# initc3/HoneyBadgerMPC

Measured on AMD Instinct MI355X. Metric: shares reconstructed/sec (batch open, n=64 t=21), higher is better.
Workload: dtype u256 (integer mod p): exact int8 x int8 -> int32 byte-split GEMM on the matrix cores; the high half of every sum folded mod p on the matrix cores too, one-word Barrett quotient

## Files before the change

honeybadgermpc_amd/_capi.py:

```python
import ctypes
import os

import numpy as np

_HERE = os.path.dirname(os.path.abspath(__file__))
LIB_PATH = os.environ.get("HBMPC_HIP_LIB") or os.path.join(_HERE, "lib", "libhbmpc_hip.so")

HB_OK, HB_ERR_SINGULAR, HB_ERR_BAD_ARG, HB_ERR_UNSUPPORTED = 0, 1, 2, 3
HB_ERR_NO_DEVICE, HB_ERR_HIP, HB_ERR_MISMATCH, HB_ERR_RETRY = 4, 5, 6, 7
HB_DEC_COLLECTING, HB_DEC_DONE, HB_DEC_DISAGREE, HB_DEC_UNSUPPORTED, HB_DEC_PENDING = 0, 1, 2, 3, 4
HB_DEC_OPT_DEFER, HB_DEC_OPT_BESIDE = 1, 2
HB_EW_ADD, HB_EW_SUB, HB_EW_MUL, HB_EW_NEG = 0, 1, 2, 3
HB_EW_SELFTEST_BEAVER, HB_EW_SELFTEST_INV, HB_EW_SELFTEST_BROADCAST = 4, 5, 0x100
HB_PM_AUTO, HB_PM_DIRECT, HB_PM_NTT = 0, 1, 2
HB_PM_SELFTEST_SUMS, HB_PM_SELFTEST_POWERS, HB_PM_SELFTEST_TABLES, HB_PM_SELFTEST_MAC, HB_PM_SELFTEST_CONV = 0, 1, 2, 3, 4
HB_BF_SELFTEST_MASK, HB_BF_SELFTEST_SWITCH, HB_BF_SELFTEST_INDEX, HB_BF_SELFTEST_HALVE = 0, 1, 2, 3
HB_MIMC_SUB, HB_MIMC_PAIR = 1, 2
HB_MIMC_SELFTEST_PLAIN, HB_MIMC_SELFTEST_ROUND, HB_MIMC_SELFTEST_FIRST = 0, 1, 2
HB_JJ_SCALAR_BROADCAST, HB_JJ_POINT_BROADCAST = 1, 2
HB_JJ_SELFTEST_SCALAR_MUL, HB_JJ_SELFTEST_DOUBLE_TABLE, HB_JJ_SELFTEST_MASK, HB_JJ_SELFTEST_STAGE1 = 0, 1, 2, 3
HB_JJ_SELFTEST_STAGE2, HB_JJ_SELFTEST_STAGE3, HB_JJ_SELFTEST_SCALE = 4, 5, 6
HB_FXP_MOD, HB_FXP_TRUNC, HB_FXP_NEG_TRUNC = 0, 1, 2
HB_FXP_SELFTEST_MASK, HB_FXP_SELFTEST_TRUNC_PR, HB_FXP_SELFTEST_LEAVES = 0, 1, 2
HB_FXP_SELFTEST_CARRY_MASK, HB_FXP_SELFTEST_CARRY_COMBINE, HB_FXP_SELFTEST_FINISH = 3, 4, 5
# ... 35 lines not shown
_vp, _i, _i64, _sz = ctypes.c_void_p, ctypes.c_int, ctypes.c_int64, ctypes.c_size_t
_pp = ctypes.POINTER(ctypes.c_void_p)
SYMBOLS = {
    "hb_version": (_i, []),
    "hb_device_count": (_i, []),
    "hb_ctx_create": (_i, [_pp, _vp, _i, _i]),
    "hb_ctx_destroy": (None, [_vp]),
    "hb_last_error": (ctypes.c_char_p, [_vp]),
    "hb_ctx_cache_clear": (_i, [_vp]),
    "hb_ctx_cache_entries": (_i, [_vp]),
    "hb_elem_bytes": (_i, [_vp]),
    "hb_malloc": (_i, [_vp, _pp, _sz]),
    "hb_free": (_i, [_vp, _vp]),
    "hb_memcpy_h2d": (_i, [_vp, _vp, _vp, _sz, _vp]),
    "hb_memcpy_d2h": (_i, [_vp, _vp, _vp, _sz, _vp]),
    "hb_stream_sync": (_i, [_vp, _vp]),
    "hb_vand_matrix_create": (_i, [_vp, _vp, _i, _i, _pp, _vp]),
    "hb_vand_inverse_create": (_i, [_vp, _vp, _i, _pp, _vp]),
    "hb_matrix_from_host": (_i, [_vp, _vp, _i, _i, _pp, _vp]),
    "hb_matrix_to_host": (_i, [_vp, _vp, _vp, _vp]),
    "hb_matrix_destroy": (None, [_vp]),
    "hb_reduce": (_i, [_vp, _vp, _vp, _i64, _vp, _vp]),
    "hb_ew_op": (_i, [_vp, _i, _vp, _vp, _i, _vp, _i64, _vp]),
    "hb_ew_beaver": (_i, [_vp, _vp, _vp, _vp, _vp, _vp, _vp, _i64, _vp]),
    "hb_ew_inv": (_i, [_vp, _vp, _vp, _i64, _vp, _vp]),
    "hb_pm_power_sums": (_i, [_vp, _vp, _vp, _i64, _i, _i, _vp, _i, _vp, _vp]),
    "hb_pm_powers": (_i, [_vp, _vp, _vp, _i64, _i, _vp, _vp]),
    "hb_rf_newton": (_i, [_vp, _vp, _i, _vp, _vp]),
    "hb_rf_roots": (_i, [_vp, _vp, _i, ctypes.c_uint64, _vp, _vp, _vp]),
    "hb_bf_mask": (_i, [_vp, _vp, _vp, _vp, _vp, _i64, _i, _vp, _vp]),
    "hb_bf_switch": (_i, [_vp, _vp, _vp, _vp, _vp, _vp, _vp, _i64, _i, _vp, _vp]),
    "hb_mimc_plain": (_i, [_vp, _vp, _vp, _vp, _i, _vp, _i, _i, _vp, _i64, _vp]),
    "hb_mimc_first": (_i, [_vp, _vp, _vp, _vp, _i, _vp, _vp, _i64, _vp]),
    "hb_mimc_round": (_i, [_vp, _vp, _vp, _vp, _vp, _vp, _i, _i64, _vp, _vp, _i64, _vp]),
    "hb_jj_scalar_mul": (_i, [_vp, _vp, _i, _vp, _vp, _i, _vp, _vp, _vp, _vp, _i64, _vp]),
    "hb_jj_double_table": (_i, [_vp, _vp, _vp, _vp, _i, _vp, _vp, _vp, _i64, _vp, _vp]),
    "hb_jj_add_mask": (_i, [_vp, _vp, _vp, _vp, _vp, _vp, _vp, _i64, _vp, _i64, _vp]),
    "hb_jj_add_stage1": (_i, [_vp, _vp, _vp, _vp, _vp, _i64, _vp, _vp, _vp, _i64, _vp]),
    "hb_jj_add_stage2": (_i, [_vp, _vp, _vp, _vp, _vp, _i64, _vp, _vp, _vp, _vp, _vp, _i64, _vp]),
    "hb_jj_add_stage3": (_i, [_vp, _vp, _vp, _vp, _vp, _i64, _vp, _i64, _vp]),
    "hb_jj_add_finish": (_i, [_vp, _vp, _vp, _vp, _vp, _vp, _i64, _vp, _vp]),
    "hb_fxp_mask": (_i, [_vp, _vp, _vp, _i, _i, _i, _vp, _vp, _i64, _vp]),
    "hb_fxp_trunc_pr": (_i, [_vp, _vp, _vp, _vp, _i, _vp, _vp, _i64, _vp]),
    "hb_fxp_ltl_leaves": (_i, [_vp, _vp, _vp, _i, _vp, _vp, _i64, _vp]),
    "hb_fxp_carry_mask": (_i, [_vp, _vp, _vp, _i, _i, _vp, _vp, _vp, _i64, _vp]),
    "hb_fxp_carry_combine": (_i, [_vp, _vp, _vp, _vp, _i, _i, _vp, _vp, _vp, _vp, _vp, _i64, _vp]),
    "hb_fxp_div2m_finish": (_i, [_vp, _vp, _vp, _vp, _vp, _i, _vp, _i, _vp, _i64, _vp]),
    "hb_bd_leaves": (_i, [_vp, _vp, _vp, _i, _vp, _vp, _i64, _vp]),
    "hb_bd_prefix_mask": (_i, [_vp, _vp, _vp, _i, _i, _vp, _vp, _vp, _i64, _vp]),
    "hb_bd_prefix_combine": (_i, [_vp, _vp, _vp, _vp, _i, _i, _vp, _vp, _vp, _i64, _vp]),
    "hb_bd_sum_mask": (_i, [_vp, _vp, _vp, _vp, _i, _vp, _vp, _vp, _i64, _vp]),
    "hb_bd_sum_combine": (_i, [_vp, _vp, _vp, _vp, _vp, _i, _vp, _vp, _vp, _vp, _i64, _vp]),
    "hb_div_pair_mask": (_i, [_vp, _vp, _vp, _vp, _vp, _vp, _i64, _vp]),
    "hb_div_or_mask": (_i, [_vp, _vp, _i, _i, _i, _vp, _vp, _vp, _i64, _vp]),
    "hb_div_or_combine": (_i, [_vp, _vp, _vp, _i, _i, _i, _vp, _vp, _vp, _i64, _vp]),
    "hb_div_norm_mask": (_i, [_vp, _vp, _vp, _i, _vp, _vp, _vp, _vp, _vp, _i64, _vp]),
    "hb_div_product_step": (_i, [_vp, _i, _i, _vp, _vp, _vp, _vp, _vp, _vp, _vp, _vp, _vp, _i, _i, _i, _vp, _vp, _i64, _vp]),
    "hb_div_trunc_step": (_i, [_vp, _i, _i, _i, _vp, _vp, _i, _vp, _vp, _vp, _vp, _vp, _vp, _vp, _vp, _i64, _vp]),
    "hb_legendre": (_i, [_vp, _vp, _vp, _i64, _vp]),
    "hb_eq_mask1": (_i, [_vp, _vp, _vp, _vp, _vp, _vp, _vp, _vp, _vp, _vp, _i, _i64, _vp]),
    "hb_eq_mid": (_i, [_vp, _vp, _vp, _vp, _vp, _vp, _vp, _vp, _vp, _vp, _vp, _vp, _vp, _vp, _i, _i64, _vp]),
    "hb_eq_cshare": (_i, [_vp, _vp, _vp, _vp, _vp, _vp, _vp, _i, _i64, _vp]),
    "hb_eq_finish": (_i, [_vp, _vp, _vp, _i, _vp, _vp, _vp, _i, _i64, _vp]),
    "hb_lt_mask": (_i, [_vp, _vp, _vp, _vp, _vp, _i64, _vp]),
    "hb_lt_leaves": (_i, [_vp, _vp, _vp, _i, _i, _vp, _vp, _i64, _vp]),
    "hb_lt_xor_mask": (_i, [_vp, _vp, _vp, _vp, _vp, _vp, _vp, _vp, _i64, _vp]),
    "hb_lt_dmask": (_i, [_vp, _vp, _vp, _vp, _vp, _vp, _i, _vp, _vp, _vp, _vp, _vp, _vp, _i64, _vp]),
    "hb_lt_mid": (_i, [_vp, _vp, _vp, _vp, _i, _vp, _vp, _vp, _vp, _vp, _vp, _vp, _vp, _vp, _vp, _vp, _i64, _vp]),
    "hb_lt_xor_finish": (_i, [_vp, _vp, _vp, _vp, _vp, _vp, _vp, _vp, _i64, _vp]),
    "hb_off_mul_add": (_i, [_vp, _vp, _vp, _vp, _vp, _i64, _vp]),
    "hb_off_invsqrt_scale": (_i, [_vp, _vp, _vp, _i, _vp, _i64, _vp, _vp]),
    "hb_off_degree_check": (_i, [_vp, _vp, _i, _i64, _i, _vp, _vp]),
    "hb_mat_mul": (_i, [_vp, _vp, _vp, _vp, _i, _vp, _i64, _i, _i, _i, _vp]),
    "hb_mat_constants": (_i, [_i, _vp]),
    "hb_quick_interp_check": (_i, [_vp, _vp, _i, _vp, _i, _vp, _i, _vp, _i64, _i64, _i64, _vp, _vp, _vp]),
    "hb_quick_interp_check_map": (_i, [_vp, _vp, _i, _vp, _i, _vp, _i, _vp, _i64, _i64, _i64, _vp, _vp, _vp, _vp]),
    "hb_quick_dec_create": (_i, [_vp, _vp, _i, _pp, _vp]),
    "hb_quick_dec_arrivals": (_i, [_vp, _vp, _i, _i, _i, _vp]),
    "hb_quick_dec_decide": (_i, [_vp, _vp, _i, _vp, _i64, _i64, _i64, _vp, _vp, _vp, _vp]),
    "hb_quick_dec_launch": (_i, [_vp, _vp, _i, _vp, _i64, _i64, _i64, _vp, _vp]),
    "hb_quick_dec_verdict": (_i, [_vp, _vp, _vp]),
    "hb_quick_dec_beside": (_i, [_vp, _i]),
    "hb_quick_dec_destroy": (None, [_vp]),
    "hb_dec_create": (_i, [_vp, _vp, _i, _i, _i, _pp, _vp]),
    "hb_dec_begin": (_i, [_vp, _vp, _i64, _i, _vp, _vp, _i, _vp]),
    "hb_dec_arrived1": (_i, [_vp, _i]),
    "hb_dec_options": (_i, [_vp, _i]),
    "hb_dec_settle": (_i, [_vp]),
    "hb_dec_arrived": (_i, [_vp, _vp, _i, _vp, _vp]),
    "hb_dec_verdict": (_i, [_vp, _vp, _vp]),
    "hb_dec_arrivals_list": (_i, [_vp, _vp, _i, _vp]),
    "hb_dec_destroy": (None, [_vp]),
    "hb_wait_create": (_i, [_vp, _i, _pp]),
    "hb_wait_begin": (_i, [_vp, _vp, _i64, _i64, _i, _i, _i, _i, _vp, _vp, _vp]),
    "hb_wait_arrived1": (_i, [_vp, _i, _i]),
    "hb_wait_result": (_i, [_vp, _i, _vp, _vp, _i, _vp]),
    "hb_wait_destroy": (None, [_vp]),
    "hb_symbols_fetch": (_i, [_vp, _vp, _i, _i64, _i64, _vp, _i, _vp, _vp]),
    "hb_candidate_check": (_i, [_vp, _vp, _i, _vp, _i, _vp, _i64, _i64, _vp, _vp, _vp]),
    "hb_stream_after": (_i, [_vp, _vp, _vp]),
    "hb_side_stream": (_i, [_vp, _pp]),
    "hb_probe_create": (_i, [_vp, _vp, _i, _i, _pp, _vp]),
    "hb_probe_feed": (_i, [_vp, _vp, _i, _vp, _i64, _i64, _i, _vp, _vp, _vp]),
    "hb_probe_reset": (_i, [_vp]),
    "hb_probe_workgroups": (_i, [_vp, _i]),
    "hb_probe_points_fed": (_i, [_vp]),
    "hb_probe_destroy": (None, [_vp]),
    "hb_matvec": (_i, [_vp, _vp, _vp, HbView, _vp, _vp, HbView, _i64, _vp]),
    "hb_matvec_check": (_i, [_vp, _vp, _vp, HbView, _vp, _vp, HbView, _vp, _i, _vp, _i64, _vp]),
    "hb_vandermonde_batch_evaluate": (_i, [_vp, _vp, _i, _vp, _i64, _i, _vp, _vp]),
    "hb_vandermonde_batch_interpolate": (_i, [_vp, _vp, _i, _vp, _i64, _vp, _vp]),
    "hb_fft_batch_evaluate": (_i, [_vp, _vp, _i, _vp, _i64, _i, _i, _vp, _vp]),
    "hb_fft_batch_interpolate": (_i, [_vp, _vp, _i, _vp, _i, _vp, _i64, _vp, _vp]),
    "hb_gao_decode": (_i, [_vp, _vp, _i, _i, _vp, _i64, _vp, _vp, _vp, _vp, _vp]),
    "hb_wb_decode": (_i, [_vp, _vp, _i, _i, _vp, _vp, _i64, _vp, _vp, _vp, _vp]),
    "hb_sqrt_mod": (_i, [_vp, _vp, _i64, _vp, _vp, _vp]),
    "hb_open_plan_create": (_i, [_vp, _i, _i, _i, _vp, _vp, _i, _vp, _vp, _i, _i64, _pp, _vp]),
    "hb_open_r1_encode": (_i, [_vp, _vp, _i64, _vp, _vp]),
    "hb_open_r1_decode": (_i, [_vp, _vp, _i64, _vp, _vp]),
    "hb_open_r2_decode": (_i, [_vp, _vp, _i64, _vp, _vp]),
    "hb_open_status": (_i, [_vp, _vp]),
    "hb_open_plan_set_option": (_i, [_vp, _i, _i]),
    "hb_open_plan_get_option": (_i, [_vp, _i, _vp]),
    "hb_open_plan_destroy": (None, [_vp]),
    "hb_selftest_mulmod": (_i, [_vp, _i, _vp, _vp, _vp]),
    "hb_selftest_ew": (_i, [_vp, _i, _i, _vp, _vp, _i64]),
    "hb_selftest_pm": (_i, [_vp, _i, _i, _vp, _vp, _i64, _i, _i64, _vp]),
    "hb_selftest_bf": (_i, [_vp, _i, _i, _vp, _i64, _i, _vp]),
    "hb_selftest_mimc": (_i, [_vp, _i, _i, _vp, _vp, _i, _i, _i64, _vp, _i64]),
    "hb_selftest_jj": (_i, [_vp, _i, _i, _vp, _vp, _vp, _i, _i64, _vp, _i64]),
    "hb_selftest_fxp": (_i, [_vp, _i, _i, _vp, _vp, _vp, _i64]),
    "hb_selftest_bd": (_i, [_vp, _i, _i, _vp, _vp, _vp, _i64]),
    "hb_selftest_div": (_i, [_vp, _i, _i, _vp, _vp, _vp, _i64]),
    "hb_selftest_eq": (_i, [_vp, _i, _i, _vp, _vp, _vp, _i64]),
    "hb_selftest_lt": (_i, [_vp, _i, _i, _vp, _vp, _vp, _i64]),
    "hb_selftest_off": (_i, [_vp, _i, _i, _vp, _vp, _i64]),
    "hb_selftest_rf": (_i, [_vp, _i, _i, _vp, _vp, _vp]),
    "hb_selftest_mat": (_i, [_vp, _i, _i, _vp, _vp, _vp]),
}
DEBUG_SYMBOLS = {
    "hb_debug_mm8_create": (_i, [_vp, _vp, _i, _i, _pp]),
    "hb_debug_mm8_apply": (_i, [_vp, _vp, _vp, _i64, _i64, _i64, _vp, _i64, _i64, _i64, _i64, _vp, _vp]),
    "hb_debug_occupancy": (_i, [_i, _i, _vp, _vp]),
    "hb_debug_reload_env": (None, []),
    "hb_debug_pm_slab_bytes": (None, [_i64]),
    "hb_debug_rf_stats": (None, [_vp]),
    "hb_debug_rf_profile": (None, [_i]),
    "hb_debug_mat_split": (None, [_i]),
    "hb_debug_matvec_route": (_i, [_vp, _vp, _i64, _vp]),
    "hb_debug_fs_pack_rows": (_i, [_i, _i, _i, _vp, _vp]),
    "hb_debug_fs_pack_points": (_i, [_vp, _i, _i, _i, _vp, _vp]),
    "hb_debug_fs_slot": (_i, [_i, _i, _vp, _i, _i, _vp]),
    "hb_debug_fs_last_pack": (_i, []),
}

_lib = None


def load_library():
    global _lib
    if _lib is not None:
        return _lib
    import torch

    if torch.cuda.is_available():
        torch.cuda.init()
    if not os.path.exists(LIB_PATH):
        raise HbmpcBackendError(
            f"{LIB_PATH} not found: build it with honeybadgermpc_amd/csrc/build.sh "
            "(or __graft_entry__.build()).  There is no CPU fallback."
        )
    try:
        lib = ctypes.CDLL(LIB_PATH)
    except OSError as e:
        raise HbmpcBackendError(f"cannot load {LIB_PATH}: {e}") from e
    for name, (restype, argtypes) in list(SYMBOLS.items()) + list(DEBUG_SYMBOLS.items()):
        fn = getattr(lib, name)
        fn.restype = restype
        fn.argtypes = argtypes
    _lib = lib
    if _marshal is not None and hasattr(_marshal, "bind_dec"):
        _marshal.bind_dec(ctypes.cast(lib.hb_dec_arrived1, ctypes.c_void_p).value)
        if hasattr(_marshal, "bind_wait"):
            _marshal.bind_wait(ctypes.cast(lib.hb_wait_arrived1, ctypes.c_void_p).value)
    return lib


def _load_marshal():
    try:
        import importlib.util

        path = os.path.join(_HERE, "lib", "_hbmarshal.so")
        spec = importlib.util.spec_from_file_location("_hbmarshal", path)
        mod = importlib.util.module_from_spec(spec)
        spec.loader.exec_module(mod)
        return mod
    except Exception:
        return None


_marshal = _load_marshal()


def ints_to_limbs(values, modulus, nbytes=32):
    if _marshal is not None:
        raw = _marshal.pack(values, modulus, nbytes)
        return np.frombuffer(bytearray(raw), dtype=np.uint64).reshape(len(values), nbytes // 8)
    buf = bytearray(len(values) * nbytes)
    off = 0
    for v in values:
        if v < 0:
            raise OverflowError("can't convert negative int to unsigned")
        if v >= modulus:
            v %= modulus
        buf[off : off + nbytes] = v.to_bytes(nbytes, "little")
        off += nbytes
    return np.frombuffer(buf, dtype=np.uint64).reshape(len(values), nbytes // 8)


def limbs_to_ints(arr, nbytes=32):
    if _marshal is not None:
        return _marshal.unpack(np.ascontiguousarray(arr), nbytes)
    b = np.ascontiguousarray(arr).tobytes()
    return [int.from_bytes(b[i : i + nbytes], "little") for i in range(0, len(b), nbytes)]


def np_ptr(a):
    return a.ctypes.data_as(ctypes.c_void_p)


class Context:

    _cache = {}
    _seen = {}

    @classmethod
    def get(cls, modulus, device=None, n_limbs=None):
        ctx = cls._seen.get((modulus, device, n_limbs)) if device is not None else None
        if ctx is not None:
            return ctx
        import torch

        if not torch.cuda.is_available():
            raise HbmpcBackendError(
                "honeybadgermpc_amd needs an MI355X (gfx950) GPU: torch.cuda.is_available() is False "
                "and there is no CPU fallback."
            )
        asked = (modulus, device, n_limbs) if device is not None else None
        if device is None:
            device = torch.cuda.current_device()
        if n_limbs is None:
            n_limbs = 1 if int(modulus) < (1 << 64) else 4
        key = (int(modulus), int(device), int(n_limbs))
        ctx = cls._cache.get(key)
        if ctx is None:
            ctx = cls(modulus, device, n_limbs)
            cls._cache[key] = ctx
        if asked is not None and isinstance(device, int) and len(cls._seen) < 64:
            cls._seen[asked] = ctx
        return ctx

    def __init__(self, modulus, device, n_limbs=4):
        import torch

        self.torch = torch
        self.lib = load_library()
        self.modulus = int(modulus)
        self.device = int(device)
        if self.modulus >= 1 << 256:
            raise ValueError("modulus must be below 2**256")
        if self.modulus % 2 == 0 or self.modulus < 3:
            raise ValueError("modulus must be an odd prime")
        if n_limbs not in (1, 4) or (n_limbs == 1 and self.modulus >= 1 << 64):
            raise ValueError("n_limbs must be 4, or 1 for a modulus below 2**64")
        self.n_limbs = int(n_limbs)
        self.nbytes = 8 * self.n_limbs
        p = ints_to_limbs([self.modulus], self.modulus + 1, self.nbytes)
        h = ctypes.c_void_p()
        rc = self.lib.hb_ctx_create(ctypes.byref(h), np_ptr(p), self.n_limbs, self.device)
        if rc != HB_OK:
            raise HbmpcBackendError(f"hb_ctx_create failed: {_STATUS_NAMES.get(rc, rc)}")
        self.h = h
        self.tdev = torch.device("cuda", self.device)
        self._raw_stream = getattr(torch._C, "_cuda_getCurrentRawStream", None)

    def stream(self):
        raw = self._raw_stream
        if raw is not None:
            return ctypes.c_void_p(raw(self.device))
        return ctypes.c_void_p(self.torch.cuda.current_stream(self.tdev).cuda_stream)

    def check(self, rc, what):
        if rc == HB_OK:
            return
        msg = self.lib.hb_last_error(self.h)
        raise HbmpcBackendError(f"{what}: {_STATUS_NAMES.get(rc, rc)}: {msg.decode() if msg else ''}")

    def empty(self, count):
        return self.torch.empty((max(int(count), 0), self.n_limbs), dtype=self.torch.int64, device=self.tdev)

    def to_device(self, limbs):
        t = self.torch.from_numpy(np.ascontiguousarray(limbs).view(np.int64))
        return t.to(self.tdev)

    def upload_ints(self, values):
        return self.to_device(ints_to_limbs(values, self.modulus, self.nbytes))
# ... 37 lines not shown
```

honeybadgermpc_amd/csrc/hb_common.hpp:

```cpp
#pragma once
#include <hip/hip_runtime.h>
#include <stdint.h>
#include <stdio.h>
#include <string.h>

#include <functional>
#include <map>
#include <mutex>
#include <string>
#include <vector>

#include "../../include/hbmpc_hip.h"
#include "fp29.hpp"

namespace hb {
struct FastMatrix;
struct Mm8Matrix;
struct Mm8wMatrix;
}
namespace hb {

struct Wide { static constexpr int NL = 9, NW = 8; };
struct Narrow { static constexpr int NL = 3, NW = 2; };

constexpr int OT = 4;

template <int NL, int NW>
__device__ __forceinline__ void eval_at_point_128(uint32_t (&r)[NL], const uint32_t *__restrict__ x_packed, const uint32_t *__restrict__ poly, int d,
                                                  const FpParams<NL> &P, uint32_t (*red)[NL]) {
    const int tid = threadIdx.x;
    uint32_t xd[NL], xm[NL], acc[NL];
    load_digits<NL, NW>(xd, x_packed);
    to_mont(xm, xd, P);
#pragma unroll
    for (int q = 0; q < NL; q++) acc[q] = 0;
    for (int l = tid; l < d; l += 128) {
        uint32_t pw[NL], cd[NL], m[NL];
        fp_pow_u32(pw, xm, (uint32_t)l, P);
        load_digits<NL, NW>(cd, poly + (size_t)l * NW);
        mont_mul(m, cd, pw, P);
        fp_add(acc, acc, m, P);
    }
#pragma unroll
    for (int q = 0; q < NL; q++) red[tid][q] = acc[q];
    __syncthreads();
    for (int w = 64; w >= 1; w >>= 1) {
        if (tid < w) {
            uint32_t a[NL], b[NL], t[NL];
#pragma unroll
            for (int q = 0; q < NL; q++) { a[q] = red[tid][q]; b[q] = red[tid + w][q]; }
            fp_add(t, a, b, P);
#pragma unroll
            for (int q = 0; q < NL; q++) red[tid][q] = t[q];
        }
        __syncthreads();
    }
#pragma unroll
    for (int q = 0; q < NL; q++) r[q] = red[0][q];
}

__host__ __device__ inline size_t m_index(int i, int l, int n_in, int nl, int q) {
    return (((size_t)((i / OT) * n_in + l) * (size_t)nl + (size_t)q) * OT) + (size_t)(i % OT);
}
inline int m_tiles(int n_out) { return (n_out + OT - 1) / OT; }

}

struct hb_matrix {
    hb_ctx *ctx;
    int n_out, n_in;
    uint32_t *dev;
    size_t words;
    bool cached;
    int refs;
    hb::Mm8wMatrix *wide;
    bool wide_tried;
};

namespace hb {
struct TlsError {
    static std::string &slot() { static thread_local std::string s; return s; }
    TlsError &operator=(const std::string &m) { slot() = m; return *this; }
    TlsError &operator=(const char *m) { slot() = m ? m : ""; return *this; }
    const char *c_str() const { return slot().c_str(); }
    void clear() { slot().clear(); }
    bool empty() const { return slot().empty(); }
};
struct PrescaleParams {
    uint32_t pbar[9];
    uint32_t pneg[8];
    uint32_t m0, m1;
};
}
namespace hb {
enum EnvHook {
    ENV_CACHE_CAP,
    ENV_GAO_PAIR,
    ENV_MM8W_FLAT,
    ENV_MM8W_RQ,
    ENV_MM8W_TILE16,
    ENV_MM8_NO_SKIP,
    ENV_NO_EVAL_FEW,
    ENV_NO_FUSED_PACK,
    ENV_NO_FUSED_SMALL,
    ENV_NO_FUSED_VALIDATE,
    ENV_NO_MFMA,
    ENV_NO_MFMA_DECODE,
    ENV_NO_MFMA_WIDE,
    ENV_NO_NARROW_FAST,
    ENV_NO_QUICK,
    ENV_NO_QUICK_PLAN,
    ENV_NTT_STAGE_LOOP,
    ENV_PROBE_WGS,
    ENV_QUICK_NO_CAND,
    ENV_UPLOAD_MODE,
    ENV_WB_NO_GAO,
    ENV_WB_NO_UNIFORM,
    ENV_COUNT
};
const char *env_hook(EnvHook h);
void env_reload();
}
struct hb_ctx {
    int device;
    int n_limbs;
    hb::FpParams<9> pw;
    hb::FpParams<3> pn;
    uint64_t p_limbs[4];
    std::recursive_mutex mu;
    int api_depth = 0;
    hb::TlsError err;
    std::map<std::string, hb_matrix *> mcache;
    std::map<std::vector<int32_t>, int32_t *> icache;
    std::map<std::string, void *> dcache;
    std::map<std::string, hb::FastMatrix *> fcache;
    std::map<std::string, hb::Mm8Matrix *> m8cache;
    struct CacheSlot { uint64_t tick; bool pinned; std::function<void()> drop; };
    std::map<std::string, CacheSlot> lru;
    uint64_t lru_clock = 0;
    size_t cache_cap = 192;
    int32_t *flag_dev;
    hb::PrescaleParams psc;
    int psc_state = 0;
    std::map<std::string, void *> ptcache;
    struct QuickSlot { void *buf = nullptr; size_t cap = 0; void *ev = nullptr; };
    std::vector<QuickSlot> qslots;
    unsigned qnext = 0;
    std::vector<void *> probe_pool, probe_host_pool;
    void *side_stream = nullptr;
    std::map<std::string, std::pair<void *, size_t>> scratch;
    void *fetch_host = nullptr, *fetch_dev = nullptr;
    int fetch_seq = 0;
    void *cand_host = nullptr, *cand_dev = nullptr;
    int32_t *cand_ticket = nullptr;
    int cand_seq = 0;
    void *after_event = nullptr;
    std::map<int, void *> wide_shared;
    std::map<std::string, std::vector<int>> wide_shapes;
    void *mm8_shared = nullptr;
    int elem_words() const { return n_limbs == 4 ? 8 : 2; }
    int nl() const { return n_limbs == 4 ? 9 : 3; }
};

struct hb_api_guard {
    hb_ctx *c;
    explicit hb_api_guard(hb_ctx *ctx) : c(ctx) { if (c) { c->mu.lock(); c->api_depth++; } }
    ~hb_api_guard() { if (c) { c->api_depth--; c->mu.unlock(); } }
    hb_api_guard(const hb_api_guard &) = delete;
    hb_api_guard &operator=(const hb_api_guard &) = delete;
};
#define HB_API_GUARD(ctxexpr) hb_api_guard hb_api_guard__(ctxexpr)

inline int ctx_scratch(hb_ctx *ctx, const char *slot, size_t bytes, void **out) {
    auto &e = ctx->scratch[slot];
    if (e.second < bytes || !e.first) {
        if (e.first) { (void)hipFree(e.first); e.first = nullptr; e.second = 0; }
        const size_t want = bytes ? bytes : 4;
        const hipError_t err = hipMalloc(&e.first, want);
        if (err != hipSuccess) { e.first = nullptr; ctx->err = std::string("scratch ") + slot + ": " + hipGetErrorString(err); return HB_ERR_HIP; }
        e.second = want;
    }
    *out = e.first;
    return HB_OK;
}
inline void ctx_scratch_free(hb_ctx *ctx) {
    for (auto &kv : ctx->scratch) if (kv.second.first) (void)hipFree(kv.second.first);
    ctx->scratch.clear();
}

#define HB_HIP(ctx, call)                                                                         \
    do {                                                                                          \
        hipError_t e__ = (call);                                                                  \
        if (e__ != hipSuccess) {                                                                  \
            (ctx)->err = std::string(#call) + ": " + hipGetErrorString(e__);                      \
            return HB_ERR_HIP;                                                                    \
        }                                                                                         \
    } while (0)

#define HB_LAUNCH_CHECK(ctx)                                                                      \
    do {                                                                                          \
        hipError_t e__ = hipGetLastError();                                                       \
        if (e__ != hipSuccess) {                                                                  \
            (ctx)->err = std::string("kernel launch: ") + hipGetErrorString(e__);                 \
            return HB_ERR_HIP;                                                                    \
        }                                                                                         \
    } while (0)

namespace hb {

inline int fail(hb_ctx *ctx, int code, const char *msg) {
    if (ctx) ctx->err = msg;
    return code;
}
inline int nsub_for(int d, int nl, int nw) {
    int shift = 29 * nl - 32 * nw;
    long per = 1L << shift;
    long n = (d + per - 1) / per;
    return n < 1 ? 1 : (int)n;
}
void fp_params_from_limbs(FpParams<9> &P, const uint64_t *p_limbs);
void fp_params_from_limbs(FpParams<3> &P, const uint64_t *p_limbs);
int get_int_array(hb_ctx *ctx, const int32_t *host, int n, int32_t **dev, hipStream_t s);
int own_int_array(hb_ctx *ctx, const int32_t *host, int n, int32_t **dev, hipStream_t s);
void cache_note(hb_ctx *ctx, const std::string &rk, std::function<void()> drop, bool pinned = false);
void cache_touch(hb_ctx *ctx, const std::string &rk);
void cache_trim(hb_ctx *ctx);
void matrix_unref(hb_matrix *m);
int alloc_matrix(hb_ctx *ctx, int n_out, int n_in, hb_matrix **out);
int upload_elems(hb_ctx *ctx, const uint64_t *host, size_t count, uint32_t **dev, hipStream_t s);
int upload_table(hb_ctx *ctx, void *dst_dev, const void *src_host, size_t bytes, hipStream_t s);
std::string table_key(const char *kind, hb_ctx *ctx, const uint64_t *x, int n, int d);
int pow_points_dev(hb_ctx *ctx, const uint64_t *base_host, const int32_t *exps_dev, int count, uint32_t **out_dev, hipStream_t s);
int vand_matrix_from_dev(hb_ctx *ctx, const std::string &key, const uint32_t *x_dev, int n, int d, hb_matrix **out, hipStream_t s);
int vinv_from_dev(hb_ctx *ctx, const std::string &key, const uint32_t *x_dev, int k, hb_matrix **out, hipStream_t s);
int gao_decode(hb_ctx *ctx, const uint64_t *x_host, int npts, int k, const uint64_t *ys_dev, int64_t C,
               uint64_t *coeffs_dev, uint64_t *errloc_dev, int32_t *errloc_len_dev, uint8_t *ok_dev, void *stream, int ys_stride = 0, const int32_t *sel_host = nullptr);
int launch_matvec(hb_ctx *ctx, const hb_matrix *m, const uint32_t *in, hb_view iv, const int32_t *in_rows_dev, int64_t in_count,
                  uint32_t *out, hb_view ov, int64_t out_count, const int32_t *check_mask_dev, int32_t *mismatch_dev,
                  int64_t C, hipStream_t s);
int launch_copy_view(hb_ctx *ctx, const uint32_t *src, hb_view sv, uint32_t *dst, hb_view dv, int64_t C, int L, int64_t dst_count, hipStream_t s);

int get_twiddles(hb_ctx *ctx, const uint64_t *omega_host, int n, uint32_t **tw, hipStream_t s);
int launch_ntt_lds(hb_ctx *ctx, const uint32_t *tw, int n, const uint32_t *in, hb_view iv, int64_t in_count, int d, int k,
                   uint32_t *out, hb_view ov, int64_t out_count, const int32_t *check_mask_dev, int32_t *mismatch_dev,
                   int64_t C, hipStream_t s, uint32_t *copy_dst = nullptr, hb_view cpv = hb_view{0, 0}, int64_t copy_count = 0, int copy_rows = 0);

struct FastMatrix {
    int n_out, n_in;
    int ot;
    uint32_t *M;
    int32_t *nd;
    int32_t *negrow;
    uint32_t *K;
    uint32_t *K2;
    uint32_t *K1;
    uint32_t *KT;
};
__host__ __device__ inline size_t mf_index(int i, int l, int n_in, int nl, int q, int ot) {
    return (((size_t)((i / ot) * n_in + l) * (size_t)nl + (size_t)q) * ot) + (size_t)(i % ot);
}
void fast_matrix_free(FastMatrix *m);
int fast_vand_create(hb_ctx *ctx, const uint32_t *x_dev, int n, int d, FastMatrix **out, hipStream_t s);
int fast_vinv_create(hb_ctx *ctx, const uint32_t *x_dev, int k, FastMatrix **out, hipStream_t s);
int launch_prescale(hb_ctx *ctx, const FastMatrix *m, const uint32_t *in, hb_view iv, const int32_t *rows_dev, int64_t in_count,
                    uint32_t *out_dg, int64_t C, hipStream_t s);
int launch_prescale_pk(hb_ctx *ctx, const FastMatrix *m, const uint32_t *in, hb_view iv, const int32_t *rows_dev, int64_t in_count,
                       uint32_t *out_pk, int64_t C, hipStream_t s);
int launch_matvec2(hb_ctx *ctx, const FastMatrix *m, const uint32_t *in_dg,
                   const uint32_t *in_pk, hb_view iv, const int32_t *in_rows_dev, int64_t in_count, uint32_t *scratch_dg,
                   uint32_t *out_pk, hb_view ov, int64_t out_count,
                   int pk_rows, int pk_from_mont, uint32_t *out_dg, const int32_t *check_mask_dev, int32_t *mismatch_dev,
                   int64_t C, hipStream_t s, int check_skip = 0, const uint32_t *K_override = nullptr);

int launch_decode_check(hb_ctx *ctx, const FastMatrix *dec, const FastMatrix *enc, const uint32_t *cols, hb_view cv,
                        const int32_t *z_dev, uint32_t *pk_dst, hb_view pv, int64_t pk_count, int pk_rows, uint32_t *coef_dg,
                        const int32_t *mask_dev, int32_t *mismatch_dev, int64_t C, hipStream_t s, int check_skip);

bool prescale_params(hb_ctx *ctx);
int mm8_from_fast(hb_ctx *ctx, const FastMatrix *f, Mm8Matrix **out, hipStream_t s, const int32_t *rows = nullptr, int n_rows = 0);
void mm8_free(Mm8Matrix *m);
int launch_mm8(hb_ctx *ctx, const Mm8Matrix *m, const uint32_t *in, hb_view iv, const int32_t *in_rows_dev, int64_t in_count,
               uint32_t *out, hb_view ov, int64_t out_count, const int32_t *check_mask_dev, int32_t *mismatch_dev,
               int64_t C, hipStream_t s, uint32_t *copy_dst = nullptr, hb_view cpv = hb_view{0, 0}, int64_t copy_count = 0,
               int copy_rows = 0, const int32_t *check_rows_dev = nullptr);

int mm8w_from_host(hb_ctx *ctx, const uint64_t *m_host, int n_out, int n_in, Mm8wMatrix **out, hipStream_t s);
void mm8w_free(Mm8wMatrix *m);
int mm8w_route(hb_ctx *ctx, const Mm8wMatrix *m, int64_t C, int32_t *out);
int launch_mm8w(hb_ctx *ctx, const Mm8wMatrix *m, const uint32_t *in, hb_view iv, const int32_t *in_rows_dev, int64_t in_count,
                uint32_t *out, hb_view ov, int64_t out_count, const int32_t *check_mask_dev, int32_t *mismatch_dev,
                int64_t C, hipStream_t s, const uint32_t *cmp = nullptr, hb_view cv = hb_view{0, 0}, int n_store = 0);
bool fold_tables(hb_ctx *ctx, int n_bytes, uint8_t *fold, uint32_t *top8, uint32_t *mu, uint32_t *shift8);
struct FsVerdict { unsigned long long word; unsigned long long pad; };
struct FsDone { int32_t *counter; FsVerdict *host; int32_t seq; };
constexpr int32_t FS_VERDICT_NONE = 0x3fffffff;
#ifdef __HIPCC__
__device__ __forceinline__ void fs_publish_verdict(int32_t *mismatch, int32_t *first_bad, int32_t *counter, FsVerdict *host, int32_t seq) {
    const int32_t fl = mismatch ? __hip_atomic_load(mismatch, __ATOMIC_RELAXED, __HIP_MEMORY_SCOPE_AGENT) : 0;
    const int32_t fb = first_bad ? __hip_atomic_load(first_bad, __ATOMIC_RELAXED, __HIP_MEMORY_SCOPE_AGENT) : INT32_MAX;
    const uint32_t low = ((fl & 1) ? 0x80000000u : 0u) | ((fl & 0x40000000) ? 0x40000000u : 0u) | (uint32_t)((fb < 0 || fb > FS_VERDICT_NONE) ? FS_VERDICT_NONE : fb);
    __hip_atomic_store(&host->word, ((unsigned long long)(uint32_t)seq << 32) | low, __ATOMIC_RELAXED, __HIP_MEMORY_SCOPE_SYSTEM);
    if (mismatch) __hip_atomic_store(mismatch, 0, __ATOMIC_RELAXED, __HIP_MEMORY_SCOPE_AGENT);
    if (first_bad) __hip_atomic_store(first_bad, INT32_MAX, __ATOMIC_RELAXED, __HIP_MEMORY_SCOPE_AGENT);
    if (counter) __hip_atomic_store(counter, 0, __ATOMIC_RELAXED, __HIP_MEMORY_SCOPE_AGENT);
}
__device__ __forceinline__ void fs_workgroup_done(const FsDone &done, int32_t *mismatch, int32_t *first_bad) {
    if (!done.counter) return;
    asm volatile("s_waitcnt vmcnt(0)" ::: "memory");
    __syncthreads();
    if (threadIdx.x == 0 && atomicAdd(done.counter, 1) == (int)gridDim.x - 1) fs_publish_verdict(mismatch, first_bad, done.counter, done.host, done.seq);
}
#endif
inline bool fs_verdict_is(const FsVerdict *host, int32_t seq) { return (int32_t)(*reinterpret_cast<const volatile unsigned long long *>(&host->word) >> 32) == seq; }
inline void fs_verdict_read(const FsVerdict *host, int32_t *flag, int32_t *first) {
    const uint32_t low = (uint32_t)*reinterpret_cast<const volatile unsigned long long *>(&host->word);
    *flag = ((low >> 31) ? 1 : 0) | ((low & 0x40000000u) ? 0x40000000 : 0);
    const int32_t f = (int32_t)(low & 0x3fffffffu);
    *first = f == FS_VERDICT_NONE ? INT32_MAX : f;
}
struct Mm8wShared { uint32_t bias; uint32_t c80r[9], biasmod[9]; void *wp; uint32_t *zero; };
int mm8w_geometry(int n_out, int d, int *tile_rows, int *n_rt, int *nkb, size_t *a8_bytes, size_t *crow_words);
int mm8w_shared(hb_ctx *ctx, int d, const Mm8wShared **out, hipStream_t s);
void mm8w_shared_free(hb_ctx *ctx);
int launch_mm8w_raw(hb_ctx *ctx, int n_out, int d, int tile_rows, const void *a8, const uint32_t *crow, const Mm8wShared *sh,
                    const uint32_t *in, hb_view iv, const int32_t *in_rows_dev, int64_t in_count, uint32_t *out, hb_view ov, int64_t out_count,
                    const int32_t *check_mask_dev, int32_t *mismatch_dev, int64_t C, hipStream_t s, const uint32_t *cmp, hb_view cv, int n_store,
                    int32_t *first_bad_dev, uint32_t *bad_map_dev = nullptr, const FsDone *done = nullptr);
void point_tables_free(hb_ctx *ctx);
void mm8_shared_free(hb_ctx *ctx);
struct PointTable {
    int n, S;
    uint32_t *xm, *inv, *pw;
    bool usable;
    int refs;
    bool small;
    std::vector<uint16_t> xs;
    uint16_t *xs_dev;
};
int point_table(hb_ctx *ctx, const uint64_t *x_host, int n, PointTable **out, hipStream_t s);
struct QuickLayout {
    int n, d, nc, n_coef, n_out, tile_rows, nkb;
    size_t o_a8, o_crow, o_wj, o_full, o_nraw, o_mcan, o_z, o_map, o_sync, need;
    size_t o_cand, o_cand_crow;
};
int quick_layout(hb_ctx *ctx, int n, int d, int nc, int n_coef, QuickLayout *L);
int quick_build(hb_ctx *ctx, const uint64_t *x_host, const int32_t *z, const int32_t *zc, const QuickLayout &L, uint8_t *base, const Mm8wShared **shared, hipStream_t s,
                int flags = 3 );
int quick_layout_cand(hb_ctx *ctx, QuickLayout *L);
int quick_launch(hb_ctx *ctx, const QuickLayout &L, const uint8_t *base, const Mm8wShared *sh, const uint32_t *cols, hb_view cv, uint32_t *out, hb_view ov,
                 int64_t out_count, int n_store, int32_t *mismatch_dev, int32_t *first_bad_dev, int64_t C, hipStream_t s, uint32_t *bad_map_dev = nullptr,
                 const FsDone *done = nullptr);
struct FsLayout {
    int n, d, nc, n_coef, n_out, n_rt, nkb;
    size_t o_a8, o_crow, o_kt, o_mode, o_z, o_cand, o_cand_crow, need;
    int pk_nm, pk_ns;
    uint8_t pk_single[8];
};
constexpr int FS_BUILD_Z = 1, FS_BUILD_ZC = 2;
int fs_layout(hb_ctx *ctx, const PointTable *pt, int d, int nc, int n_coef, FsLayout *L);
int fs_build(hb_ctx *ctx, const PointTable *pt, const int32_t *z, const int32_t *zc, const FsLayout &L, uint8_t *base, int flags, int32_t *status_dev, hipStream_t s);
bool fs_pack(const PointTable *pt, const int32_t *z, FsLayout *L);
int fs_launch(hb_ctx *ctx, const FsLayout &L, const uint8_t *base, const uint32_t *cols, hb_view cv, uint32_t *out, hb_view ov, int64_t out_count,
              int32_t *mismatch_dev, int32_t *first_bad_dev, uint32_t *bad_map_dev, int64_t C, hipStream_t s, const FsDone *done = nullptr,
              const int32_t *pick_zc = nullptr);
int fs_build_cand(hb_ctx *ctx, PointTable *pt, const int32_t *z, const FsLayout &L, uint8_t *base, int32_t *status_dev, hipStream_t s, bool with_z = false);
struct Mv64Matrix;
int points_on_device(hb_ctx *ctx, const uint64_t *x_host, int n, uint32_t **out, hipStream_t s);
bool mv64_applies(const hb_ctx *ctx, int d);
bool mv64_matrix_cores(const hb_ctx *ctx, int d);
int mv64_from_host(hb_ctx *ctx, const uint64_t *m_host, int n_out, int d, const int32_t *mode_host, Mv64Matrix **out, hipStream_t s);
void mv64_free(Mv64Matrix *m);
int launch_mv64(hb_ctx *ctx, const Mv64Matrix *m, const uint64_t *in, hb_view iv, const int32_t *in_rows_dev, int64_t in_count, uint64_t *out, hb_view ov,
                int64_t out_count, int32_t *mismatch_dev, int32_t *first_bad_dev, int64_t C, hipStream_t s);
int mv64_plan_tables(hb_ctx *ctx, const uint64_t *x, int n, int d, const int32_t *z, const int32_t *zc, int nc, std::vector<uint64_t> &V, std::vector<uint64_t> &Vinv,
                     std::vector<uint64_t> &P);
int quick_dec_supported(hb_quick_dec *qd, int d, int nc, int n_coef);
const Mm8wMatrix *matrix_wide(hb_ctx *ctx, const hb_matrix *m, hipStream_t s);

#define HB_DISPATCH(ctx, EXPR_W, EXPR_N)                                                          \
    do {                                                                                          \
        if ((ctx)->n_limbs == 4) { EXPR_W; } else { EXPR_N; }                                     \
    } while (0)

}
```

honeybadgermpc_amd/csrc/hb_core.hip:

```cpp
#include <algorithm>

#include <mutex>
#include <string>

#include "hb_common.hpp"

using namespace hb;

namespace {

struct U320 { uint64_t l[5]; };
inline bool ge(const U320 &a, const U320 &b) {
    for (int i = 4; i >= 0; i--) if (a.l[i] != b.l[i]) return a.l[i] > b.l[i];
    return true;
}
inline void sub(U320 &a, const U320 &b) {
    unsigned __int128 br = 0;
    for (int i = 0; i < 5; i++) {
        unsigned __int128 d = (unsigned __int128)a.l[i] - b.l[i] - (uint64_t)br;
        a.l[i] = (uint64_t)d; br = (d >> 64) & 1;
    }
}
inline void dbl_mod(U320 &a, const U320 &p) {
    for (int i = 4; i > 0; i--) a.l[i] = (a.l[i] << 1) | (a.l[i - 1] >> 63);
// ... 272 lines not shown
    pack<NL, NW>(o, d);
    bool diff = false;
#pragma unroll
    for (int q = 0; q < NW; q++) diff |= o[q] != w[q];
    if (diff) {
        store_words<NW>(dst + i * NW, o);
        if (changed) atomicAdd(changed, 1);
    } else if (dst != src) {
        store_words<NW>(dst + i * NW, w);
    }
}

namespace hb {

void cache_note(hb_ctx *ctx, const std::string &rk, std::function<void()> drop, bool pinned) {
    ctx->lru[rk] = hb_ctx::CacheSlot{++ctx->lru_clock, pinned, std::move(drop)};
}
void cache_touch(hb_ctx *ctx, const std::string &rk) {
    auto it = ctx->lru.find(rk);
    if (it != ctx->lru.end()) it->second.tick = ++ctx->lru_clock;
}
static void cache_drop_down_to(hb_ctx *ctx, size_t keep) {
    std::vector<std::pair<uint64_t, std::string>> order;
    for (auto &kv : ctx->lru) if (!kv.second.pinned) order.emplace_back(kv.second.tick, kv.first);
    if (order.size() <= keep) return;
    std::sort(order.begin(), order.end());
    (void)hipDeviceSynchronize();
    for (size_t i = 0; i + keep < order.size(); i++) {
        auto it = ctx->lru.find(order[i].second);
        if (it == ctx->lru.end()) continue;
        auto drop = std::move(it->second.drop);
        ctx->lru.erase(it);
        drop();
    }
}
void cache_trim(hb_ctx *ctx) {
    if (ctx->api_depth > 1) return;
    size_t unpinned = 0;
    for (auto &kv : ctx->lru) if (!kv.second.pinned) unpinned++;
    if (unpinned > ctx->cache_cap) cache_drop_down_to(ctx, ctx->cache_cap / 2);
}
void matrix_unref(hb_matrix *m) {
    if (!m) return;
    if (--m->refs > 0) return;
    (void)hipFree(m->dev);
    mm8w_free(m->wide);
    delete m;
}

static std::string int_key(const int32_t *host, int n) {
    return std::string("i|") + std::string(reinterpret_cast<const char *>(host), (size_t)(n > 0 ? n : 0) * 4);
}
int own_int_array(hb_ctx *ctx, const int32_t *host, int n, int32_t **dev, hipStream_t s) {
    int32_t *d = nullptr;
    HB_HIP(ctx, hipMalloc(&d, sizeof(int32_t) * (size_t)(n > 0 ? n : 1)));
    const int rc = upload_table(ctx, d, host, sizeof(int32_t) * (size_t)(n > 0 ? n : 0), s);
    if (rc) { (void)hipFree(d); return rc; }
    *dev = d;
    return HB_OK;
}
int get_int_array(hb_ctx *ctx, const int32_t *host, int n, int32_t **dev, hipStream_t s) {
    std::vector<int32_t> key(host, host + n);
    const std::string rk = int_key(host, n);
    auto it = ctx->icache.find(key);
    if (it != ctx->icache.end()) { cache_touch(ctx, rk); *dev = it->second; return HB_OK; }
    int32_t *d = nullptr;
    int rc = own_int_array(ctx, host, n, &d, s); if (rc) return rc;
    ctx->icache[key] = d;
    cache_note(ctx, rk, [ctx, key]() { auto f = ctx->icache.find(key); if (f != ctx->icache.end()) { (void)hipFree(f->second); ctx->icache.erase(f); } });
    *dev = d;
    return HB_OK;
}

int alloc_matrix(hb_ctx *ctx, int n_out, int n_in, hb_matrix **out) {
    hb_matrix *m = new hb_matrix();
    m->ctx = ctx; m->n_out = n_out; m->n_in = n_in; m->cached = false; m->refs = 1; m->wide = nullptr; m->wide_tried = false;
    m->words = (size_t)m_tiles(n_out) * (size_t)n_in * OT * (size_t)ctx->nl();
    if (m->words == 0) m->words = 1;
    hipError_t e = hipMalloc(&m->dev, m->words * sizeof(uint32_t));
    if (e != hipSuccess) { delete m; ctx->err = std::string("hipMalloc: ") + hipGetErrorString(e); return HB_ERR_HIP; }
    *out = m;
    return HB_OK;
}

__global__ void k_upload_copy(const uint4 *__restrict__ src, uint4 *__restrict__ dst, size_t n16) {
    const size_t i = (size_t)blockIdx.x * blockDim.x + threadIdx.x;
    if (i < n16) dst[i] = src[i];
}
int upload_table(hb_ctx *ctx, void *dst_dev, const void *src_host, size_t bytes, hipStream_t s) {
    if (bytes == 0) return HB_OK;
    static const int legacy = [] { const char *e = env_hook(ENV_UPLOAD_MODE); return e && !strcmp(e, "memcpy") ? 1 : 0; }();
    if (legacy) {
        hipError_t e = hipMemcpyAsync(dst_dev, src_host, bytes, hipMemcpyHostToDevice, s);
        if (e == hipSuccess) e = hipStreamSynchronize(s);
        if (e != hipSuccess) { ctx->err = std::string("table upload: ") + hipGetErrorString(e); return HB_ERR_HIP; }
        return HB_OK;
    }
    const size_t n16 = (bytes + 15) / 16;
    void *stage = nullptr;
    HB_HIP(ctx, hipMalloc(&stage, n16 * 16));
    hipError_t e = hipMemcpy(stage, src_host, bytes, hipMemcpyHostToDevice);
    if (e == hipSuccess) {
        if (bytes % 16 == 0) k_upload_copy<<<(unsigned)((n16 + 255) / 256), 256, 0, s>>>((const uint4 *)stage, (uint4 *)dst_dev, n16);
        else e = hipMemcpyAsync(dst_dev, stage, bytes, hipMemcpyDeviceToDevice, s);
    }
    if (e == hipSuccess) e = hipGetLastError();
    if (e == hipSuccess) e = hipStreamSynchronize(s);
    (void)hipFree(stage);
    if (e != hipSuccess) { ctx->err = std::string("table upload: ") + hipGetErrorString(e); return HB_ERR_HIP; }
    return HB_OK;
}

int upload_elems(hb_ctx *ctx, const uint64_t *host, size_t count, uint32_t **dev, hipStream_t s) {
    size_t bytes = count * (size_t)ctx->elem_words() * 4;
    HB_HIP(ctx, hipMalloc(dev, bytes ? bytes : 4));
    const int rc = upload_table(ctx, *dev, host, bytes, s);
    if (rc) { (void)hipFree(*dev); *dev = nullptr; }
    return rc;
}

int points_on_device(hb_ctx *ctx, const uint64_t *x_host, int n, uint32_t **out, hipStream_t s) {
    std::string key = table_key("xs", ctx, x_host, n, 0);
    auto it = ctx->dcache.find(key);
    if (it != ctx->dcache.end()) { *out = (uint32_t *)it->second; cache_touch(ctx, "d|" + key); return HB_OK; }
    uint32_t *xd = nullptr;
    const int rc = upload_elems(ctx, x_host, (size_t)n, &xd, s); if (rc) return rc;
    ctx->dcache[key] = xd;
    cache_note(ctx, "d|" + key, [ctx, key]() { auto f = ctx->dcache.find(key); if (f != ctx->dcache.end()) { (void)hipFree(f->second); ctx->dcache.erase(f); } });
    *out = xd;
    return HB_OK;
}

std::string table_key(const char *kind, hb_ctx *ctx, const uint64_t *x, int n, int d) {
    std::string k(kind);
    k += ":" + std::to_string(n) + ":" + std::to_string(d) + ":";
    k.append(reinterpret_cast<const char *>(x), (size_t)n * ctx->n_limbs * 8);
    return k;
}

}

template <int NL, int NW>
__global__ void __launch_bounds__(128) k_eval_few(const FpParams<NL> P, const uint32_t *__restrict__ x, int n, const uint32_t *__restrict__ polys, int d,
                                                  uint32_t *__restrict__ out) {
    __shared__ uint32_t red[128][NL];
    const int c = blockIdx.x / n, i = blockIdx.x - c * n;
    uint32_t r[NL];
    eval_at_point_128<NL, NW>(r, x + (size_t)i * NW, polys + (size_t)c * d * NW, d, P, red);
    if (threadIdx.x == 0) store_digits<NL, NW>(out + ((size_t)c * n + i) * NW, r);
}


namespace hb {
static const char *const ENV_NAMES[ENV_COUNT] = {"HB_CACHE_CAP", "HB_GAO_PAIR", "HB_MM8W_FLAT", "HB_MM8W_RQ", "HB_MM8W_TILE16", "HB_MM8_NO_SKIP", "HB_NO_EVAL_FEW", "HB_NO_FUSED_PACK", "HB_NO_FUSED_SMALL", "HB_NO_FUSED_VALIDATE", "HB_NO_MFMA", "HB_NO_MFMA_DECODE", "HB_NO_MFMA_WIDE", "HB_NO_NARROW_FAST", "HB_NO_QUICK", "HB_NO_QUICK_PLAN", "HB_NTT_STAGE_LOOP", "HB_PROBE_WGS", "HB_QUICK_NO_CAND", "HB_UPLOAD_MODE", "HB_WB_NO_GAO", "HB_WB_NO_UNIFORM"};
static std::string g_env_val[ENV_COUNT];
static bool g_env_set[ENV_COUNT];
static std::once_flag g_env_once;
static std::mutex g_env_mu;
static void env_read() {
    for (int i = 0; i < ENV_COUNT; i++) {
        const char *e = ::getenv(ENV_NAMES[i]);
        g_env_set[i] = e != nullptr;
        g_env_val[i] = e ? e : "";
    }
}
const char *env_hook(EnvHook h) {
    std::call_once(g_env_once, env_read);
    return g_env_set[h] ? g_env_val[h].c_str() : nullptr;
}
void env_reload() {
    std::call_once(g_env_once, env_read);
    std::lock_guard<std::mutex> lk(g_env_mu);
    env_read();
}
}
extern "C" void hb_debug_reload_env() { hb::env_reload(); }

extern "C" {

int hb_version(void) { return 100; }

int hb_device_count(void) {
    int n = 0;
    if (hipGetDeviceCount(&n) != hipSuccess) return 0;
    return n;
}

int hb_ctx_create(hb_ctx **out, const uint64_t *p_limbs, int n_limbs, int device) {
    if (!out || !p_limbs) return HB_ERR_BAD_ARG;
    *out = nullptr;
    if (n_limbs != 1 && n_limbs != 4) return HB_ERR_BAD_ARG;
    if ((p_limbs[0] & 1) == 0) return HB_ERR_UNSUPPORTED;
    bool small = true; for (int i = 1; i < n_limbs; i++) if (p_limbs[i]) small = false;
    if (small && p_limbs[0] < 3) return HB_ERR_UNSUPPORTED;
    int ndev = 0;
    if (hipGetDeviceCount(&ndev) != hipSuccess || ndev == 0) return HB_ERR_NO_DEVICE;
    if (device < 0 || device >= ndev) return HB_ERR_NO_DEVICE;
    if (hipSetDevice(device) != hipSuccess) return HB_ERR_NO_DEVICE;
    hb_ctx *ctx = new hb_ctx();
    ctx->device = device; ctx->n_limbs = n_limbs;
    memset(ctx->p_limbs, 0, sizeof ctx->p_limbs);
    memcpy(ctx->p_limbs, p_limbs, (size_t)n_limbs * 8);
    if (n_limbs == 4) make_params<9>(ctx->pw, p_limbs, 4); else make_params<3>(ctx->pn, p_limbs, 1);
    if (const char *e = env_hook(ENV_CACHE_CAP)) { long v = atol(e); if (v >= 1) ctx->cache_cap = (size_t)v; }
    ctx->flag_dev = nullptr;
    if (hipMalloc(&ctx->flag_dev, 64 * sizeof(int32_t)) != hipSuccess) { delete ctx; return HB_ERR_HIP; }
    (void)hipMemset(ctx->flag_dev, 0, 64 * sizeof(int32_t));
    *out = ctx;
    return HB_OK;
}

void hb_ctx_destroy(hb_ctx *ctx) {
    if (!ctx) return;
    (void)hipSetDevice(ctx->device);
    ctx->lru.clear();
    for (auto &kv : ctx->mcache) matrix_unref(kv.second);
    for (auto &kv : ctx->icache) (void)hipFree(kv.second);
    for (auto &kv : ctx->dcache) (void)hipFree(kv.second);
    for (auto &kv : ctx->fcache) fast_matrix_free(kv.second);
    for (auto &kv : ctx->m8cache) mm8_free(kv.second);
    if (ctx->flag_dev) (void)hipFree(ctx->flag_dev);
    if (ctx->side_stream) (void)hipStreamDestroy((hipStream_t)ctx->side_stream);
    point_tables_free(ctx);
    mm8w_shared_free(ctx);
    mm8_shared_free(ctx);
    ctx_scratch_free(ctx);
    delete ctx;
}

const char *hb_last_error(const hb_ctx *ctx) { return ctx ? ctx->err.c_str() : "no context"; }
int hb_elem_bytes(const hb_ctx *ctx) { return ctx ? ctx->n_limbs * 8 : 0; }

int hb_malloc(hb_ctx *ctx, void **dptr, size_t bytes) { HB_API_GUARD(ctx); HB_HIP(ctx, hipMalloc(dptr, bytes ? bytes : 4)); return HB_OK; }
int hb_free(hb_ctx *ctx, void *dptr) { HB_API_GUARD(ctx); HB_HIP(ctx, hipFree(dptr)); return HB_OK; }
int hb_memcpy_h2d(hb_ctx *ctx, void *dst, const void *src, size_t bytes, void *stream) { HB_API_GUARD(ctx);
    HB_HIP(ctx, hipMemcpyAsync(dst, src, bytes, hipMemcpyHostToDevice, (hipStream_t)stream)); return HB_OK;
}
int hb_memcpy_d2h(hb_ctx *ctx, void *dst, const void *src, size_t bytes, void *stream) { HB_API_GUARD(ctx);
    HB_HIP(ctx, hipMemcpyAsync(dst, src, bytes, hipMemcpyDeviceToHost, (hipStream_t)stream));
    HB_HIP(ctx, hipStreamSynchronize((hipStream_t)stream)); return HB_OK;
}
int hb_stream_sync(hb_ctx *ctx, void *stream) { HB_API_GUARD(ctx); HB_HIP(ctx, hipStreamSynchronize((hipStream_t)stream)); return HB_OK; }

}

namespace hb {

template <int NL, int NW>
__global__ void k_pow_points(const FpParams<NL> P, const uint32_t *__restrict__ base, const int32_t *__restrict__ exps, int count,
                             uint32_t *__restrict__ out) {
    int i = blockIdx.x * blockDim.x + threadIdx.x;
    if (i >= count) return;
    uint32_t bd[NL], bm[NL], r[NL], c[NL];
    load_digits<NL, NW>(bd, base);
    to_mont(bm, bd, P);
    fp_pow_u32(r, bm, (uint32_t)(exps ? exps[i] : i), P);
    from_mont(c, r, P);
    store_digits<NL, NW>(out + (size_t)i * NW, c);
}

int pow_points_dev(hb_ctx *ctx, const uint64_t *base_host, const int32_t *exps_dev, int count, uint32_t **out_dev, hipStream_t s) {
    uint32_t *bd = nullptr;
    int rc = upload_elems(ctx, base_host, 1, &bd, s); if (rc) return rc;
    HB_HIP(ctx, hipMalloc(out_dev, (size_t)(count > 0 ? count : 1) * ctx->elem_words() * 4));
    if (count > 0) {
        HB_DISPATCH(ctx,
            (k_pow_points<9, 8><<<(count + 63) / 64, 64, 0, s>>>(ctx->pw, bd, exps_dev, count, *out_dev)),
            (k_pow_points<3, 2><<<(count + 63) / 64, 64, 0, s>>>(ctx->pn, bd, exps_dev, count, *out_dev)));
        HB_LAUNCH_CHECK(ctx);
    }
    HB_HIP(ctx, hipStreamSynchronize(s));
    HB_HIP(ctx, hipFree(bd));
    return HB_OK;
}

int vand_matrix_from_dev(hb_ctx *ctx, const std::string &key, const uint32_t *x_dev, int n, int d, hb_matrix **out, hipStream_t s) {
    hb_matrix *m = nullptr;
    int rc = alloc_matrix(ctx, n, d, &m); if (rc) return rc;
    HB_HIP(ctx, hipMemsetAsync(m->dev, 0, m->words * 4, s));
    if (n > 0 && d > 0) {
        HB_DISPATCH(ctx,
            (k_vand_table<9, 8><<<(n + 63) / 64, 64, 0, s>>>(ctx->pw, x_dev, n, d, m->dev)),
            (k_vand_table<3, 2><<<(n + 63) / 64, 64, 0, s>>>(ctx->pn, x_dev, n, d, m->dev)));
        HB_LAUNCH_CHECK(ctx);
        HB_HIP(ctx, hipStreamSynchronize(s));
    }
    m->cached = true; ctx->mcache[key] = m; *out = m;
    cache_note(ctx, "m|" + key, [ctx, key]() { auto f = ctx->mcache.find(key); if (f != ctx->mcache.end()) { hb_matrix *mm = f->second; ctx->mcache.erase(f); matrix_unref(mm); } });
    return HB_OK;
}

int vinv_from_dev(hb_ctx *ctx, const std::string &key, const uint32_t *x_dev, int k, hb_matrix **out, hipStream_t s) {
    if (k > 1023) return fail(ctx, HB_ERR_UNSUPPORTED, "vandermonde inverse: k > 1023");
    hb_matrix *m = nullptr;
    int rc = alloc_matrix(ctx, k, k, &m); if (rc) return rc;
    HB_HIP(ctx, hipMemsetAsync(m->dev, 0, m->words * 4, s));
    int singular = 0;
    if (k > 0) {
        HB_HIP(ctx, hipMemsetAsync(ctx->flag_dev, 0, sizeof(int32_t), s));
        int threads = ((k + 1 + 63) / 64) * 64;
        size_t lds = (size_t)(k + 2 * (k + 1)) * ctx->nl() * 4;
        if (ctx->n_limbs == 4) {
            HB_HIP(ctx, hipFuncSetAttribute(reinterpret_cast<const void *>(k_vinv_table<9, 8>), hipFuncAttributeMaxDynamicSharedMemorySize, (int)lds));
            k_vinv_table<9, 8><<<1, threads, lds, s>>>(ctx->pw, x_dev, k, m->dev, ctx->flag_dev);
        } else {
            HB_HIP(ctx, hipFuncSetAttribute(reinterpret_cast<const void *>(k_vinv_table<3, 2>), hipFuncAttributeMaxDynamicSharedMemorySize, (int)lds));
            k_vinv_table<3, 2><<<1, threads, lds, s>>>(ctx->pn, x_dev, k, m->dev, ctx->flag_dev);
// ... 369 lines not shown
```

honeybadgermpc_amd/csrc/hb_mfma.hip:

```cpp
#include <atomic>

#include "hb_mm8.hpp"

namespace hb {

#include "hb_mm8_body.inc"

#ifdef HB_MM8_TIMING
__device__ unsigned long long g_mm8_t[2048 * 8];
#define MM8_T(k) do { const unsigned long long tn_ = __builtin_amdgcn_s_memtime(); tacc[k] += tn_ - tlast; tlast = tn_; } while (0)
#else
#define MM8_T(k) do { } while (0)
#endif
template <int NKB, bool CHECK, bool RAGGED, bool SKIP>
__global__ __launch_bounds__(256, 2) void k_mm8(const int4 *__restrict__ a8, const uint32_t *__restrict__ crowd,
                                                const uint32_t *__restrict__ zero_src,
                                                const uint32_t *__restrict__ in_pk, int64_t in_sc, int64_t in_sl,
                                                const int32_t *__restrict__ in_rows, int64_t in_count, int d,
                                                uint32_t *__restrict__ out_pk, int64_t out_sc, int64_t out_sl, int64_t out_count,
                                                const int32_t *__restrict__ check_mask, const int32_t *__restrict__ check_rows, int32_t *__restrict__ mismatch,
                                                uint32_t *__restrict__ copy_dst, int64_t copy_sc, int64_t copy_sl, int64_t copy_count, int copy_rows,
                                                int n_out, int n_rt, int tpw, int64_t n_chunks, int64_t n_units, BarrettParams bp) {
    extern __shared__ uint4 mm8_lds[];
    const int lane = threadIdx.x & 63, wave = __builtin_amdgcn_readfirstlane(threadIdx.x >> 6);
// ... 264 lines not shown
namespace {

constexpr size_t MM8_LDS_LIMIT = 78 * 1024;
size_t mm8_lds_bytes(int n_rt, int nkb, int tpw);
int mm8_tpw(int n_rt, int nkb) {
    int tpw = (n_rt == 1) ? 4 : (n_rt == 2) ? 2 : 1;
    return tpw;
}
size_t mm8_lds_bytes(int n_rt, int nkb, int tpw) {
    return ((size_t)n_rt * 64 + (size_t)n_rt * nkb * 2 * 64 + (size_t)2 * tpw * nkb * 4 * 64 + MM8_FOLD_Q) * 16 + 96 * 4 + (size_t)n_rt * 16 * 4;
}

int mm8_num_cus() {
    static int n = 0;
    if (!n) {
        int dev = 0;
        (void)hipGetDevice(&dev);
        if (hipDeviceGetAttribute(&n, hipDeviceAttributeMultiprocessorCount, dev) != hipSuccess || n <= 0) n = 256;
    }
    return n;
}

typedef std::vector<uint32_t> Big;
Big big_mul(const Big &a, const Big &b) {
    Big r(a.size() + b.size(), 0);
    for (size_t i = 0; i < a.size(); i++) {
        uint64_t cy = 0;
        for (size_t j = 0; j < b.size(); j++) {
            uint64_t t = (uint64_t)a[i] * b[j] + r[i + j] + cy;
            r[i + j] = (uint32_t)t; cy = t >> 32;
        }
        r[i + b.size()] = (uint32_t)cy;
    }
    return r;
}
bool big_ge(const Big &a, const Big &b) {
    for (size_t i = a.size(); i-- > 0;) if (a[i] != b[i]) return a[i] > b[i];
    return true;
}
void big_sub(Big &a, const Big &b) {
    int64_t br = 0;
    for (size_t i = 0; i < a.size(); i++) {
        int64_t t = (int64_t)a[i] - (i < b.size() ? b[i] : 0) + br;
        a[i] = (uint32_t)t; br = t >> 32;
    }
}
void big_add(Big &a, const Big &b) {
    uint64_t cy = 0;
    for (size_t i = 0; i < a.size(); i++) {
        uint64_t t = (uint64_t)a[i] + (i < b.size() ? b[i] : 0) + cy;
        a[i] = (uint32_t)t; cy = t >> 32;
    }
}
Big big_divmod(const Big &x, const Big &p, Big *q) {
    Big r(p.size() + 1, 0), pp(p); pp.push_back(0);
    if (q) q->assign(x.size(), 0);
    for (int bit = (int)x.size() * 32 - 1; bit >= 0; bit--) {
        uint32_t in = (x[bit >> 5] >> (bit & 31)) & 1u;
        for (size_t i = r.size(); i-- > 0;) r[i] = (r[i] << 1) | (i ? r[i - 1] >> 31 : in);
        if (big_ge(r, pp)) { big_sub(r, pp); if (q) (*q)[bit >> 5] |= 1u << (bit & 31); }
    }
    r.pop_back();
    return r;
}
Big big_shl(const Big &a, int bits, size_t words) {
    Big r(words, 0);
    for (size_t i = 0; i < a.size(); i++) {
        const size_t w = i + bits / 32; const int s = bits % 32;
        if (w < words) r[w] |= a[i] << s;
        if (s && w + 1 < words) r[w + 1] |= a[i] >> (32 - s);
    }
    return r;
}

}

namespace hb {

bool prescale_params(hb_ctx *ctx) {
    if (ctx->psc_state) return ctx->psc_state > 0;
    ctx->psc_state = -1;
    if (ctx->n_limbs != 4 || (ctx->p_limbs[3] >> 62) == 0) return false;
    Big p(8);
    for (int i = 0; i < 4; i++) { p[2 * i] = (uint32_t)ctx->p_limbs[i]; p[2 * i + 1] = (uint32_t)(ctx->p_limbs[i] >> 32); }
    Big pw9(p); pw9.push_back(0);
    Big pb(9, 0); pb[8] = 1u << 5;
    big_sub(pb, pw9);
    for (int k = 0; k < 9; k++) {
        const int bit = 29 * k, j = bit >> 5, sft = bit & 31;
        const uint64_t v = pb[j] | ((uint64_t)(j + 1 < 9 ? pb[j + 1] : 0) << 32);
        ctx->psc.pbar[k] = (uint32_t)(v >> sft) & DMASK;
    }
    Big pn(9, 0); pn[8] = 1;
    big_sub(pn, pw9);
    for (int k = 0; k < 8; k++) ctx->psc.pneg[k] = pn[k];
    Big two290(10, 0); two290[9] = 1u << 2;
    Big mu; big_divmod(two290, p, &mu);
    const uint64_t muv = mu[0] | ((uint64_t)mu[1] << 32);
    ctx->psc.m0 = (uint32_t)muv & DMASK;
    ctx->psc.m1 = (uint32_t)(muv >> LB);
    ctx->psc_state = 1;
    return true;
}

void mm8_free(Mm8Matrix *m) {
    if (!m) return;
    (void)hipFree(m->a8); (void)hipFree(m->crow); (void)hipFree(m->zero);
    delete m;
}

int mm8_shared(hb_ctx *ctx, const Mm8Shared **out, hipStream_t s) {
    if (ctx->mm8_shared) { *out = static_cast<const Mm8Shared *>(ctx->mm8_shared); return HB_OK; }
    if (ctx->n_limbs != 4 || (ctx->p_limbs[3] >> 62) == 0 || !prescale_params(ctx)) return fail(ctx, HB_ERR_UNSUPPORTED, "mm8: modulus");
    Mm8Shared *sh = new Mm8Shared();
    memset(sh, 0, sizeof *sh);
    Big p(8);
    for (int k = 0; k < 4; k++) { p[2 * k] = (uint32_t)ctx->p_limbs[k]; p[2 * k + 1] = (uint32_t)(ctx->p_limbs[k] >> 32); }
    uint32_t shift8[8];
    if (!fold_tables(ctx, 16, sh->fold_host, sh->bp.c384, &sh->bp.mu, shift8)) { delete sh; return fail(ctx, HB_ERR_UNSUPPORTED, "mm8: fold table"); }
    {
        Big pn(9, 0); pn[8] = 1;
        Big pw9(p); pw9.push_back(0);
        big_sub(pn, pw9);
        for (int k = 0; k < 8; k++) sh->bp.pneg[k] = pn[k];
    }
    auto digits9 = [](const Big &v, uint32_t *dg) {
        for (int k = 0; k < 9; k++) {
            const int bit = 29 * k, j = bit >> 5, sft = bit & 31;
            const uint64_t w = (uint64_t)(j < (int)v.size() ? v[j] : 0) | ((uint64_t)(j + 1 < (int)v.size() ? v[j + 1] : 0) << 32);
            dg[k] = (uint32_t)(w >> sft) & DMASK;
        }
    };
    Big biasmod;
    { Big bt(14, 0); for (int c = 0; c < MM8_NC; c++) { Big t(1, (uint32_t)MM8_BIAS); big_add(bt, big_shl(t, 8 * c, 14)); } biasmod = big_divmod(bt, p, nullptr); }
    { Big sft(shift8, shift8 + 8); if (!big_ge(biasmod, sft)) big_add(biasmod, p); big_sub(biasmod, sft); }
    digits9(biasmod, sh->biasmod);
    for (int merged = 0; merged < 2; merged++) {
        Big bt(14, 0);
        for (int c = 0; c < MM8_NCP; c++) {
            Big t(1, (uint32_t)MM8_BIAS_PACK);
            big_add(bt, big_shl(t, 8 * c, 14));
            if (merged) big_add(bt, big_shl(t, 8 * (c + 8), 14));
        }
        Big bm = big_divmod(bt, p, nullptr);
        Big sft(shift8, shift8 + 8);
        if (!big_ge(bm, sft)) big_add(bm, p);
        big_sub(bm, sft);
        digits9(bm, merged ? sh->biasmod_pm : sh->biasmod_ps);
    }
    {
        Big c80(8, 0x80808080u);
        Big r261(9, 0); r261[8] = 1u << 5;
        digits9(big_divmod(big_mul(c80, r261), p, nullptr), sh->c80r);
    }
    if (hipMalloc(&sh->fold_dev, sizeof sh->fold_host) != hipSuccess) { delete sh; return fail(ctx, HB_ERR_HIP, "mm8: hipMalloc(fold table)"); }
    if (int rc = upload_table(ctx, sh->fold_dev, sh->fold_host, sizeof sh->fold_host, s)) { (void)hipFree(sh->fold_dev); delete sh; return rc; }
    ctx->mm8_shared = sh;
    *out = sh;
    return HB_OK;
}

void mm8_shared_free(hb_ctx *ctx) {
    Mm8Shared *sh = static_cast<Mm8Shared *>(ctx->mm8_shared);
    if (!sh) return;
    (void)hipFree(sh->fold_dev);
    delete sh;
    ctx->mm8_shared = nullptr;
}

int mm8_from_fast(hb_ctx *ctx, const FastMatrix *f, Mm8Matrix **out, hipStream_t s, const int32_t *rows, int n_rows) {
    *out = nullptr;
    if (env_hook(ENV_NO_MFMA)) return HB_ERR_UNSUPPORTED;
    if (ctx->n_limbs != 4 || f->n_in < 1 || f->n_in > 32 || f->n_out < 1) return HB_ERR_UNSUPPORTED;
    if ((ctx->p_limbs[3] >> 62) == 0) return HB_ERR_UNSUPPORTED;
    const int n_out = rows ? n_rows : f->n_out, d = f->n_in, nkb = (d + 7) / 8, n_rt = (n_out + 15) / 16;
    if (n_out < 1) return HB_ERR_UNSUPPORTED;
    if (mm8_lds_bytes(n_rt, nkb, (n_rt == 1) ? 4 : (n_rt == 2) ? 2 : 1) > MM8_LDS_LIMIT) return HB_ERR_UNSUPPORTED;
    const int tiles = (f->n_out + f->ot - 1) / f->ot;
    std::vector<uint32_t> Mh((size_t)tiles * d * f->ot * 9);
    std::vector<int32_t> neg((size_t)f->n_out, 0);
    HB_HIP(ctx, hipMemcpyAsync(Mh.data(), f->M, Mh.size() * 4, hipMemcpyDeviceToHost, s));
    if (f->negrow) HB_HIP(ctx, hipMemcpyAsync(neg.data(), f->negrow, neg.size() * 4, hipMemcpyDeviceToHost, s));
    HB_HIP(ctx, hipStreamSynchronize(s));

    Big p(8);
    for (int k = 0; k < 4; k++) { p[2 * k] = (uint32_t)ctx->p_limbs[k]; p[2 * k + 1] = (uint32_t)(ctx->p_limbs[k] >> 32); }
    Big c80(8, 0x80808080u);
    c80 = big_divmod(c80, p, nullptr);
    Big biasmod;
    { Big bt(14, 0); for (int c = 0; c < MM8_NC; c++) { Big t(1, (uint32_t)MM8_BIAS); big_add(bt, big_shl(t, 8 * c, 14)); } biasmod = big_divmod(bt, p, nullptr); }
    std::vector<uint8_t> foldtab((size_t)MM8_FOLD_Q * 16, 0);
    BarrettParams bpar;
    {
        uint32_t shift8[8];
        if (!fold_tables(ctx, 16, foldtab.data(), bpar.c384, &bpar.mu, shift8)) return HB_ERR_UNSUPPORTED;
        Big sh(shift8, shift8 + 8);
        if (!big_ge(biasmod, sh)) big_add(biasmod, p);
        big_sub(biasmod, sh);
    }

    std::vector<int8_t> a((size_t)n_rt * nkb * 2 * 64 * 16, 0);
    bool skip01 = nkb >= 2 && !env_hook(ENV_MM8_NO_SKIP);
    std::vector<uint32_t> cr((size_t)n_rt * 16 * 16 + (size_t)MM8_FOLD_Q * 4, 0);
    memcpy(&cr[(size_t)n_rt * 16 * 16], foldtab.data(), foldtab.size());
    for (size_t i = 0; i < (size_t)n_rt * 16; i++) for (int k = 0; k < 8; k++) { cr[i * 16 + 2 * k] = 0x10100000u; cr[i * 16 + 2 * k + 1] = 0x1010u; }
    for (int i = 0; i < n_out; i++) {
        Big pos(5, 0), ngs(5, 0);
        int64_t colsum = 0;
        const int src = rows ? rows[i] : i;
        if (src < 0 || src >= f->n_out) return HB_ERR_BAD_ARG;
        for (int l = 0; l < d; l++) {
            uint32_t dg[9], w8[8];
            for (int q = 0; q < 9; q++) dg[q] = Mh[mf_index(src, l, d, 9, q, f->ot)];
            pack<9, 8>(w8, dg);
            if (w8[4] | w8[5] | w8[6] | w8[7]) return HB_ERR_UNSUPPORTED;
            const int sgn = neg[src] ? -1 : 1;
            int carry = 0;
            const int lane_ = (4 * ((i % 16) % 4) + (i % 16) / 4) + 16 * ((l % 8) / 2), el = l & 1;
            for (int b = 0; b < 16; b++) {
                int t = sgn * (int)((w8[b >> 2] >> (8 * (b & 3))) & 0xffu) + carry;
                if (t > 127) { t -= 256; carry = 1; } else if (t < -128) { t += 256; carry = -1; } else carry = 0;
                const int grp = b >> 3, r7 = 7 - (b & 7), hi = r7 >> 2, bi = r7 & 3;
                a[((((size_t)(i / 16) * nkb + l / 8) * 2 + grp) * 64 + (size_t)lane_) * 16 + 4 * (2 * hi + el) + bi] = (int8_t)t;
                if (t != 0 && grp == 1 && l < 8) skip01 = false;
                colsum += (t < 0) ? -t : t;
            }
            if (carry) return HB_ERR_UNSUPPORTED;
            Big e(w8, w8 + 4);
            big_add(neg[src] ? ngs : pos, e);
        }
        if (colsum * 128 > MM8_BIAS) return HB_ERR_UNSUPPORTED;
        Big cp = big_divmod(big_mul(c80, pos), p, nullptr), cn = big_divmod(big_mul(c80, ngs), p, nullptr);
        if (!big_ge(cp, cn)) big_add(cp, p);
        big_sub(cp, cn);
        if (!big_ge(cp, biasmod)) big_add(cp, p);
        big_sub(cp, biasmod);
        for (int k = 0; k < 8; k++) {
            const uint64_t pair = (uint64_t)cp[k] + ((0x1010ull << 32) | 0x10100000ull);
            cr[(size_t)i * 16 + 2 * k] = (uint32_t)pair;
            cr[(size_t)i * 16 + 2 * k + 1] = (uint32_t)(pair >> 32);
        }
    }
    Mm8Matrix *m = new Mm8Matrix();
    m->n_out = n_out; m->d = d; m->nkb = nkb; m->n_rt = n_rt; m->skip01 = skip01; m->a8 = nullptr; m->crow = nullptr; m->zero = nullptr;
    m->bp = bpar;
    {
        Big pn(9, 0); pn[8] = 1;
        Big pw9(p); pw9.push_back(0);
        big_sub(pn, pw9);
        for (int k = 0; k < 8; k++) m->bp.pneg[k] = pn[k];
    }
    HB_HIP(ctx, hipMalloc(&m->a8, a.size()));
    HB_HIP(ctx, hipMalloc(&m->crow, cr.size() * 4));
    HB_HIP(ctx, hipMalloc(&m->zero, 64));
    {
        std::vector<uint8_t> zero64(64, 0);
        int rc = upload_table(ctx, m->a8, a.data(), a.size(), s);
        if (!rc) rc = upload_table(ctx, m->crow, cr.data(), cr.size() * 4, s);
        if (!rc) rc = upload_table(ctx, m->zero, zero64.data(), 64, s);
        if (rc) { mm8_free(m); return rc; }
    }
    *out = m;
    return HB_OK;
}

int launch_mm8(hb_ctx *ctx, const Mm8Matrix *m, const uint32_t *in, hb_view iv, const int32_t *in_rows_dev, int64_t in_count,
               uint32_t *out, hb_view ov, int64_t out_count, const int32_t *check_mask_dev, int32_t *mismatch_dev,
               int64_t C, hipStream_t s, uint32_t *copy_dst, hb_view cpv, int64_t copy_count, int copy_rows,
               const int32_t *check_rows_dev) {
    if (C <= 0) return HB_OK;
    const int tpw = mm8_tpw(m->n_rt, m->nkb);
    const int64_t n_tiles = (C + 15) / 16;
    const int64_t n_units = (n_tiles + tpw - 1) / tpw;
    int64_t blocks = 2 * (int64_t)mm8_num_cus();
    if (blocks > n_units) blocks = n_units;
    blocks = mm8_trimmed_grid(n_units, blocks);
    const size_t lds = mm8_lds_bytes(m->n_rt, m->nkb, tpw);
    const bool check = check_mask_dev != nullptr;
    const bool ragged = !check && (m->n_out % 16) >= 1 && (m->n_out % 16) <= 8;
#define MM8_LAUNCH_(NKB, CHK, RG, SK)                                                                                 \
    do {                                                                                                          \
        static std::atomic<unsigned long long> attr_done{0};                                                                               \
        if (!((attr_done.load() >> (ctx->device & 63)) & 1ull)) {                                                                                         \
            HB_HIP(ctx, hipFuncSetAttribute(reinterpret_cast<const void *>(k_mm8<NKB, CHK, RG, SK>), hipFuncAttributeMaxDynamicSharedMemorySize, 80 * 1024)); \
            attr_done.fetch_or(1ull << (ctx->device & 63));                                                                                     \
        }                                                                                                         \
        hipLaunchKernelGGL((k_mm8<NKB, CHK, RG, SK>), dim3((unsigned)blocks), dim3(256), lds, s, m->a8, m->crow, m->zero, in, iv.stride_c, \
                           iv.stride_l, in_rows_dev, in_count, m->d, out, ov.stride_c, ov.stride_l, out_count,   \
                           check_mask_dev, check_rows_dev, mismatch_dev, copy_dst, cpv.stride_c, cpv.stride_l, copy_count, copy_rows,         \
                           m->n_out, m->n_rt, tpw, C, n_units, m->bp);             \
    } while (0)
#define MM8_LAUNCH(NKB) do { if (check) MM8_LAUNCH_(NKB, true, false, false); else if (ragged) MM8_LAUNCH_(NKB, false, true, false); else MM8_LAUNCH_(NKB, false, false, false); } while (0)
#define MM8_LAUNCH_SK(NKB) do { if (check) MM8_LAUNCH_(NKB, true, false, true); else if (ragged) MM8_LAUNCH_(NKB, false, true, false); else MM8_LAUNCH_(NKB, false, false, true); } while (0)
    switch (m->nkb) {
        case 1: MM8_LAUNCH(1); break;
        case 2: if (m->skip01) MM8_LAUNCH_SK(2); else MM8_LAUNCH(2); break;
        case 3: if (m->skip01) MM8_LAUNCH_SK(3); else MM8_LAUNCH(3); break;
        case 4: if (m->skip01) MM8_LAUNCH_SK(4); else MM8_LAUNCH(4); break;
        default: return fail(ctx, HB_ERR_UNSUPPORTED, "mm8: more than 32 terms");
    }
#undef MM8_LAUNCH
#undef MM8_LAUNCH_SK
#undef MM8_LAUNCH_
    HB_LAUNCH_CHECK(ctx);
    return HB_OK;
}
// ... 31 lines not shown
```

honeybadgermpc_amd/csrc/hb_mfma_fused.hip:

```cpp
#include <math.h>

#include <algorithm>
#include <atomic>
#include <type_traits>

#include "hb_mm8.hpp"

namespace hb {

#include "hb_mm8_body.inc"

constexpr int FS_WAVES = 8, FS_TPW = 4;
#ifdef HB_MM8_TIMING
__device__ unsigned long long g_fs_t[256 * 8 * 8];
#define FS_T(k) do { const unsigned long long tn_ = __builtin_amdgcn_s_memtime(); tacc[k] += tn_ - tlast; tlast = tn_; } while (0)
#else
#define FS_T(k) do { } while (0)
#endif
constexpr int FS_MAXD = 24, FS_MAXC = 104;
constexpr size_t FS_LDS_LIMIT = 156 * 1024;

struct FsIdx { uint16_t z[FS_MAXD], xz[FS_MAXD], zc[FS_MAXC], xzc[FS_MAXC]; };
struct FsPick { const uint4 *cand; const uint32_t *cand_crow; int n_coef, nc; uint16_t zc[FS_MAXC]; };
struct FsSplit { uint32_t terms[FS_WAVES]; };
struct FsPack { int nm, ns; uint8_t single[8]; };
__host__ __device__ inline int fs_slot(const FsPack &pk, int i, int n_out, int &kind) {
    kind = 0;
    if (!(pk.nm | pk.ns)) return i;
    const int base = 16 * ((n_out + 15) / 16 - 1);
    int before = 0;
    for (int k = 0; k < pk.ns; k++) {
        if (pk.single[k] == i) { kind = 2; return base + 4 + (k & 3) + 8 * (k >> 2); }
        before += pk.single[k] < i;
    }
    const int pos = i - before;
    if (pos >= base) kind = 1;
    return pos;
}
static bool fs_pack_decide(int d, int n_coef, int nc, const uint8_t *small, FsPack *pk) {
    memset(pk, 0, sizeof *pk);
    const int n_out = n_coef + nc, rem = n_out - 16 * ((n_out + 15) / 16 - 1);
    if ((int64_t)d * 8 * 128 * 128 > MM8_BIAS_PACK) return false;
    if (rem <= 8) { pk->nm = rem; return true; }
    if (rem == 16) return false;
    int ns = 0;
    for (int i = n_coef - 1; i >= 0 && ns < 8; i--)
        if (small[i]) pk->single[ns++] = (uint8_t)i;
    std::reverse(pk->single, pk->single + ns);
    if (rem - ns > 4) { memset(pk, 0, sizeof *pk); return false; }
    pk->nm = rem - ns; pk->ns = ns;
    return true;
}
constexpr int FS_CAND_MAXN = 128;

__host__ __device__ inline size_t fs_lds_bytes(int n_rt, int nkb) {
    return ((size_t)n_rt * 64 + (size_t)n_rt * nkb * 2 * 64 + (size_t)2 * FS_TPW * nkb * 4 * 64 + MM8_FOLD_Q) * 16 + (size_t)(32 + 16 * n_rt) * 4;
}

#define FS_REDUCE(I_, F_, E_, C0_) \
    do { \
        const int i = (I_); \
        const int md = maskl[i]; \
        const bool live = chunk < n_chunks; \
        const bool cmp = live && md > 0, st = live && md < 0; \
        uint32_t ew[8]; \
        load_words<8>(ew, in_pk + (cmp ? (chunk * in_sc + (int64_t)(md - 1) * in_sl) * 8 : 0)); \
        uint64_t pw[8]; \
        { \
            const uint4 *cr = reinterpret_cast<const uint4 *>(crl + (size_t)i * 16); \
        _Pragma("unroll") \
            for (int k = 0; k < 4; k++) { \
                const uint4 c = cr[k]; \
                pw[2 * k] = (uint64_t)c.x | ((uint64_t)c.y << 32); \
                pw[2 * k + 1] = (uint64_t)c.z | ((uint64_t)c.w << 32); \
            } \
        } \
        uint32_t glo[5], ghi[5]; \
        _Pragma("unroll") \
        for (int k = 0; k < 12; k++) { \
            uint64_t gk = (uint64_t)F_(k) * k256 + (k < 7 ? pw[k] : 0ull); \
            if (k < 11) gk += (uint64_t)E_(k) * k16m; \
            if (k < 7) pw[k] = gk; \
            else { glo[k - 7] = (uint32_t)gk; ghi[k - 7] = (uint32_t)(gk >> 32); } \
        } \
        pw[0] += (uint64_t)(C0_) * u1; \
        pw[7] += (uint64_t)glo[0] * u1; \
        uint32_t hw[5]; \
        { \
            unsigned cyw = 0; \
        _Pragma("unroll") \
            for (int k = 0; k < 4; k++) hw[k] = __builtin_addc(glo[k + 1], ghi[k], cyw, &cyw); \
            hw[4] = ghi[4] + cyw; \
        } \
        v4i hb; \
        _Pragma("unroll") \
        for (int k = 0; k < 4; k++) hb[k] = (int)(hw[k] ^ 0x80808080u); \
        v4i dcol[8]; \
        _Pragma("unroll") \
        for (int eb = 0; eb < 8; eb++) \
            dcol[eb] = __builtin_amdgcn_mfma_i32_16x16x64_i8(fold_lane[eb * (MM8_FOLD_ROW / 16)], hb, v4i{0, 0, 0, 0}, 0, 0, 0); \
        _Pragma("unroll") \
        for (int k = 0; k < 8; k++) pw[k] += (uint64_t)hw[4] * bp.c384[k]; \
        _Pragma("unroll") \
        for (int k = 0; k < 8; k++) { \
            int64_t tt = (int64_t)pw[k] + (int64_t)dcol[k][0] * s1; \
            tt += (int64_t)dcol[k][1] * s256; \
            tt += (int64_t)dcol[k][2] * s64k; \
            tt += (int64_t)dcol[k][3] * s16m; \
            pw[k] = (uint64_t)tt; \
        } \
        const uint64_t tq = pw[7] + (pw[6] >> 32); \
        const uint32_t qh = (uint32_t)(((uint64_t)(uint32_t)(tq >> 16) * bp.mu) >> 46); \
        _Pragma("unroll") \
        for (int k = 0; k < 8; k++) pw[k] += (uint64_t)qh * bp.pneg[k]; \
        uint32_t ow[8]; \
        uint32_t top; \
        { \
            unsigned cy = 0; \
            ow[0] = (uint32_t)pw[0]; \
        _Pragma("unroll") \
            for (int k = 1; k < 8; k++) ow[k] = __builtin_addc((uint32_t)pw[k], (uint32_t)(pw[k - 1] >> 32), cy, &cy); \
            top = (uint32_t)(pw[7] >> 32) + cy - qh; \
        } \
        if (__builtin_amdgcn_ballot_w64(top != 0 || ow[7] >= ~bp.pneg[7]) != 0) { \
            uint32_t u[8]; \
            unsigned cy2 = 0; \
        _Pragma("unroll") \
            for (int k = 0; k < 8; k++) u[k] = __builtin_addc(ow[k], bp.pneg[k], cy2, &cy2); \
            const bool take = cy2 || top; \
        _Pragma("unroll") \
            for (int k = 0; k < 8; k++) ow[k] = take ? u[k] : ow[k]; \
        } \
        uint32_t diff = 0; \
        _Pragma("unroll") \
        for (int k = 0; k < 8; k++) diff |= ew[k] ^ ow[k]; \
        asm volatile("" : "+v"(diff), "+v"(ow[0]), "+v"(ow[1]), "+v"(ow[2]), "+v"(ow[3]), "+v"(ow[4]), "+v"(ow[5]), "+v"(ow[6]), "+v"(ow[7])); \
        const unsigned long long bad_lanes = __builtin_amdgcn_ballot_w64(cmp && diff); \
        if (bad_lanes) { \
            const uint32_t bits16 = (uint32_t)((bad_lanes | (bad_lanes >> 16) | (bad_lanes >> 32) | (bad_lanes >> 48)) & 0xffffull); \
            if (lane == 0) { \
                const int64_t tile_base = chunk - n; \
                const int32_t cmin = (int32_t)tile_base + __builtin_ctz(bits16); \
                if (*reinterpret_cast<volatile int32_t *>(mismatch) == 0) atomicOr(mismatch, 1); \
                if (first_bad && *reinterpret_cast<volatile int32_t *>(first_bad) > cmin) atomicMin(first_bad, cmin); \
                if (bad_map) atomicOr(bad_map + (tile_base >> 5), bits16 << (tile_base & 31)); \
            } \
        } \
        const int64_t oidx = chunk * out_sc + (int64_t)(-md - 1) * out_sl; \
        if (st && oidx < out_count) store_words<8>(out_pk + oidx * 8, ow); \
    } while (0)

template <int NKB, int PK>
__global__ __launch_bounds__(64 * FS_WAVES, 2) void k_mm8f(const int4 *__restrict__ a8, const uint32_t *__restrict__ crowd, const v4i *__restrict__ foldg,
                                                          const uint32_t *__restrict__ KT, const PrescaleParams PP,
                                                          const uint32_t *__restrict__ in_pk, int64_t in_sc, int64_t in_sl, const int32_t *__restrict__ in_rows,
                                                          int64_t in_count, int d, const int32_t *__restrict__ rowmode,
                                                          uint32_t *__restrict__ out_pk, int64_t out_sc, int64_t out_sl, int64_t out_count,
                                                          int32_t *__restrict__ mismatch, int32_t *__restrict__ first_bad, uint32_t *__restrict__ bad_map,
                                                          int n_out, int n_rt, int64_t n_chunks, int64_t n_units, BarrettParams bp, const FsDone done, const FsPick pick,
                                                          const FsSplit split) {
    constexpr bool PACKED = PK != 0;
    const int n_slots = PACKED ? 16 * n_rt : n_out;
    constexpr int NT = 64 * FS_WAVES, NL = 9, NW = 8;
    extern __shared__ uint4 fs_lds[];
    const int lane = threadIdx.x & 63, wave = __builtin_amdgcn_readfirstlane(threadIdx.x >> 6);
    const int n = lane & 15, g = lane >> 4;
    uint32_t *crl = reinterpret_cast<uint32_t *>(fs_lds);
    int4 *abuf = reinterpret_cast<int4 *>(fs_lds + n_rt * 64);
    uint4 *xbuf = fs_lds + n_rt * 64 + n_rt * NKB * 2 * 64;
    constexpr int bufsz = FS_TPW * NKB * 4 * 64;
    int32_t *rowl = reinterpret_cast<int32_t *>(xbuf + 2 * bufsz);
    int32_t *maskl = rowl + 32;
    v4i *foldl = reinterpret_cast<v4i *>(maskl + 16 * n_rt);

#ifdef HB_MM8_TIMING
    unsigned long long tacc[8] = {0, 0, 0, 0, 0, 0, 0, 0}, tlast = __builtin_amdgcn_s_memtime();
#endif
    auto unit_chunk = [&](int64_t unit) {
        const int64_t chunk = unit * 64 + lane;
        return chunk >= n_chunks ? n_chunks - 1 : chunk;
    };
    auto fetch_row = [&](int64_t chunk, int row, uint32_t (&w)[NW], bool &okk) {
        const int64_t idx = chunk * in_sc + (int64_t)row * in_sl;
        okk = idx < in_count;
        load_words<NW>(w, in_pk + (okk ? idx : 0) * NW);
    };
    const uint32_t first_terms = (0x01010101u << wave) & (d < 32 ? (1u << d) - 1u : ~0u);
    uint32_t x_first[NW] = {0, 0, 0, 0, 0, 0, 0, 0};
    bool ok_first = false;
    if (first_terms) {
        const int l0 = __builtin_ctz(first_terms);
        fetch_row(unit_chunk(blockIdx.x), in_rows ? in_rows[l0] : l0, x_first, ok_first);
    }
    uint4 pk_piece = make_uint4(0, 0, 0, 0), pk_crow = make_uint4(0, 0, 0, 0);
    const int pk_e = threadIdx.x;
    const bool pk_has_piece = !PACKED && pick.cand && pk_e < pick.nc * NKB * 8, pk_has_crow = !PACKED && pick.cand && pk_e < pick.nc * 4;
    if (pk_has_piece) {
        const int j = pk_e / (NKB * 8), pc = pk_e - j * (NKB * 8);
        pk_piece = pick.cand[(size_t)pick.zc[j] * (NKB * 8) + pc];
    }
    if (pk_has_crow) pk_crow = reinterpret_cast<const uint4 *>(pick.cand_crow)[(size_t)pick.zc[pk_e >> 2] * 4 + (pk_e & 3)];
    {
        const int tid = threadIdx.x, n_mask = n_rt * 16, n_crow = n_rt * 64, n_img = n_rt * NKB * 2 * 64;
        const int lc = tid < d ? tid : d - 1;
        int32_t rw = in_rows ? in_rows[lc] : lc;
        int32_t mk = rowmode[tid < n_slots ? tid : 0];
        v4i cr = reinterpret_cast<const v4i *>(crowd)[tid < n_crow ? tid : 0];
        v4i fo = foldg[tid < MM8_FOLD_Q ? tid : 0];
        v4i img[3];
#pragma unroll
        for (int k = 0; k < 3; k++) img[k] = reinterpret_cast<const v4i *>(a8)[tid + k * NT < n_img ? tid + k * NT : 0];
        asm volatile("" : "+v"(rw), "+v"(mk), "+v"(cr), "+v"(fo), "+v"(img[0]), "+v"(img[1]), "+v"(img[2]));
        if (tid < 32) rowl[tid] = rw;
        if (tid < n_mask) maskl[tid] = tid < n_slots ? mk : 0;
        if (tid < n_crow) reinterpret_cast<v4i *>(fs_lds)[tid] = cr;
        if (tid < MM8_FOLD_Q) foldl[tid] = fo;
#pragma unroll
        for (int k = 0; k < 3; k++)
            if (tid + k * NT < n_img) reinterpret_cast<v4i *>(abuf)[tid + k * NT] = img[k];
        for (int i = tid + NT; i < n_mask; i += NT) maskl[i] = i < n_slots ? rowmode[i] : 0;
        for (int i = tid + NT; i < n_crow; i += NT) fs_lds[i] = reinterpret_cast<const uint4 *>(crowd)[i];
        for (int i = tid + 3 * NT; i < n_img; i += NT) abuf[i] = a8[i];
    }
    for (int i = threadIdx.x; i < (8 * NKB - d) * 256; i += NT) {
        const int l = d + (i >> 8), b = (i >> 7) & 1, t = (i >> 5) & 3, h = (i >> 4) & 1, c = i & 15;
        const int kb = l >> 3, gg = (l & 7) >> 1, e = l & 1;
        xbuf[(size_t)b * bufsz + (size_t)((((t * NKB + kb) * 2 + e) * 2 + h) * 64) + (c + 16 * gg)] = make_uint4(0, 0, 0, 0);
    }
    const int n_pairs = FS_TPW * n_rt;
    const uint32_t my_terms = (uint32_t)__builtin_amdgcn_readfirstlane((int)split.terms[wave]);

    auto scale_unit = [&](auto first, int64_t unit, uint4 *dst, uint32_t terms) {
        constexpr bool FIRST = decltype(first)::value;
        const int64_t chunk = unit_chunk(unit);
        const int t = lane >> 4;
        uint32_t xw[NW];
        bool ok = false;
        auto fetch = [&](int l, uint32_t (&w)[NW], bool &okk) { fetch_row(chunk, FIRST ? (in_rows ? in_rows[l] : l) : rowl[l], w, okk); };
        terms &= d < 32 ? (1u << d) - 1u : ~0u;
        int l = terms ? __builtin_ctz(terms) : d;
        if constexpr (FIRST) {
#pragma unroll
            for (int k = 0; k < NW; k++) xw[k] = x_first[k];
            ok = ok_first;
        } else if (l < d) fetch(l, xw, ok);
        while (l < d) {
            terms &= terms - 1u;
            const int ln = terms ? __builtin_ctz(terms) : d;
            uint32_t xn[NW];
            bool okn = false;
            fetch(ln < d ? ln : l, xn, okn);
            const uint32_t *__restrict__ T = KT + (size_t)l * (NL * NL);
            uint32_t xd[NL];
            unpack<NL, NW>(xd, xw);
            uint64_t col[NL + 1];
#pragma unroll
            for (int j = 0; j <= NL; j++) col[j] = 0;
#pragma unroll
            for (int q = 0; q < NL; q++)
#pragma unroll
                for (int j = 0; j < NL; j++) col[j] += (uint64_t)xd[q] * T[q * NL + j];
            uint32_t v[NL + 1];
#pragma unroll
            for (int k = 0; k < NL; k++) { v[k] = (uint32_t)col[k] & DMASK; col[k + 1] += col[k] >> LB; }
            v[NL] = (uint32_t)col[NL];
            const uint64_t mid = (uint64_t)v[9] * PP.m0 + (uint64_t)v[8] * PP.m1 + (((uint64_t)v[8] * PP.m0) >> LB);
            const uint64_t qh = (uint64_t)v[9] * PP.m1 + (mid >> LB);
            const uint32_t q0 = (uint32_t)qh & DMASK, q1 = (uint32_t)(qh >> LB);
            uint64_t dc[NL];
#pragma unroll
            for (int k = 0; k < NL; k++) {
                dc[k] = v[k] + (uint64_t)q0 * PP.pbar[k];
                if (k > 0) dc[k] += (uint64_t)q1 * PP.pbar[k - 1];
            }
            uint32_t r[NL];
#pragma unroll
            for (int k = 0; k < NL; k++) {
                r[k] = (uint32_t)dc[k] & DMASK;
                if (k < NL - 1) dc[k + 1] += dc[k] >> LB;
            }
            uint32_t w[NW];
            pack<NL, NW>(w, r);
            if (PP.pneg[NW - 1] >> 31) {
#pragma unroll
                for (int k = 0; k < NW; k++) w[k] = ok ? w[k] : 0u;
            } else {
                uint32_t u[NW];
                unsigned cy = 0;
#pragma unroll
                for (int k = 0; k < NW; k++) u[k] = __builtin_addc(w[k], PP.pneg[k], cy, &cy);
                const bool take = cy || (r[NL - 1] >> 24);
#pragma unroll
                for (int k = 0; k < NW; k++) w[k] = ok ? (take ? u[k] : w[k]) : 0u;
            }
            const int kb = l >> 3, gg = (l & 7) >> 1, e = l & 1;
            uint4 *slot = dst + (size_t)(((t * NKB + kb) * 2 + e) * 2) * 64 + (n + 16 * gg);
            slot[0] = make_uint4(w[0], w[1], w[2], w[3]);
            slot[64] = make_uint4(w[4], w[5], w[6], w[7]);
#pragma unroll
            for (int k = 0; k < NW; k++) xw[k] = xn[k];
            ok = okn;
            l = ln;
        }
    };

    scale_unit(std::true_type{}, blockIdx.x, xbuf, first_terms);
    if (!PACKED && pick.cand) {
        __syncthreads();
        auto put = [&](int e, const uint4 &v) {
            const int j = e / (NKB * 8), pc = e - j * (NKB * 8);
            const int ri = pick.n_coef + j, rt = ri >> 4, r16 = ri & 15, r = 4 * (r16 & 3) + (r16 >> 2);
            const int kb = pc >> 3, grp = (pc >> 2) & 1, gg = pc & 3;
            reinterpret_cast<uint4 *>(abuf)[((rt * NKB + kb) * 2 + grp) * 64 + r + 16 * gg] = v;
        };
        if (pk_has_piece) put(pk_e, pk_piece);
        for (int e = pk_e + NT; e < pick.nc * NKB * 8; e += NT) {
            const int j = e / (NKB * 8), pc = e - j * (NKB * 8);
            put(e, pick.cand[(size_t)pick.zc[j] * (NKB * 8) + pc]);
        }
        if (pk_has_crow) fs_lds[(pick.n_coef + (pk_e >> 2)) * 4 + (pk_e & 3)] = pk_crow;
        for (int j = threadIdx.x; j < pick.nc; j += NT) maskl[pick.n_coef + j] = (int32_t)pick.zc[j] + 1;
    }

    const v4i biasv = v4i{MM8_BIAS, MM8_BIAS, MM8_BIAS, MM8_BIAS};
    uint32_t k256 = 256u, k16m = 1u << 24;
    int32_t s1 = 1, s256 = 256, s64k = 1 << 16, s16m = 1 << 24;
    uint32_t u1 = 1u;
    asm volatile("" : "+s"(k256), "+s"(k16m), "+s"(s1), "+s"(s256), "+s"(s64k), "+s"(s16m), "+s"(u1));
    const v4i *fold_lane = reinterpret_cast<const v4i *>(reinterpret_cast<const char *>(foldl) + (g == (n >> 2) ? 16 * n : 256));

    int buf = 0;
    int64_t unit = blockIdx.x;
    FS_T(0);
    for (; unit < n_units; unit += gridDim.x, buf ^= 1) {
        asm volatile("s_waitcnt lgkmcnt(0)" ::: "memory");
        FS_T(7);
        __builtin_amdgcn_s_barrier();
        FS_T(1);
        if (my_terms && unit + gridDim.x < n_units) scale_unit(std::false_type{}, unit + gridDim.x, xbuf + (size_t)(buf ^ 1) * bufsz, my_terms);
        FS_T(2);
        for (int pidx = wave; pidx < n_pairs; pidx += FS_WAVES) {
            const int tl = n_rt == 2 ? (pidx >> 1) : pidx / n_rt;
            const int rt = n_rt == 2 ? ((pidx ^ (pidx >> 2)) & 1) : pidx - tl * n_rt;
            const int64_t chunk = (unit * FS_TPW + tl) * 16 + n;
            const uint4 *xs = xbuf + (size_t)buf * bufsz + (size_t)tl * NKB * 4 * 64 + lane;
            const int4 *as = abuf + (size_t)rt * NKB * 2 * 64 + lane;
            uint32_t eap[4][11], c0p[4];
            const int rows_here = n_out - 16 * rt < 16 ? n_out - 16 * rt : 16;
            const int nreg = PACKED ? 4 : (rows_here + 3) >> 2;
            const uint32_t xs_addr = (uint32_t)(uintptr_t)(__attribute__((address_space(3))) const void *)xs;
            const uint32_t as_addr = (uint32_t)(uintptr_t)(__attribute__((address_space(3))) const void *)as;
            if (PACKED && rt == n_rt - 1) {
                const v4i biaspv = v4i{MM8_BIAS_PACK, MM8_BIAS_PACK, MM8_BIAS_PACK, MM8_BIAS_PACK};
                auto park_merged = [&](auto rc, const v4i (&acc)[20]) __attribute__((always_inline)) {
                    constexpr int r = decltype(rc)::value;
                    c0p[r] = (uint32_t)acc[0][r];
#pragma unroll
                    for (int j = 0; j < 11; j++) {
                        uint32_t lo = 0, hi = 0;
                        if (j < 9) { lo = (uint32_t)acc[1 + 2 * j][r]; hi = (uint32_t)acc[2 + 2 * j][r]; }
                        if (j >= 2) { lo += (uint32_t)acc[2 * j - 3][r + 2]; hi += (uint32_t)acc[2 * j - 2][r + 2]; }
                        if (j == 1) hi += (uint32_t)acc[0][r + 2];
                        eap[r][j] = lo + (hi << 8);
                    }
                };
                auto park_single = [&](auto rc, const v4i (&acc)[20]) __attribute__((always_inline)) {
                    constexpr int r = decltype(rc)::value;
                    c0p[r] = (uint32_t)acc[0][r];
#pragma unroll
                    for (int j = 0; j < 11; j++) eap[r][j] = j < 9 ? (uint32_t)acc[1 + 2 * j][r] + ((uint32_t)acc[2 + 2 * j][r] << 8) : 0u;
                };
                auto keep = [&](auto rc) __attribute__((always_inline)) {
                    constexpr int r = decltype(rc)::value;
                    asm volatile("" ::"v"(c0p[r]), "v"(eap[r][0]), "v"(eap[r][1]), "v"(eap[r][2]), "v"(eap[r][3]), "v"(eap[r][4]), "v"(eap[r][5]),
                                 "v"(eap[r][6]), "v"(eap[r][7]), "v"(eap[r][8]), "v"(eap[r][9]), "v"(eap[r][10]));
                    __builtin_amdgcn_sched_barrier(0);
                };
                {
                    v4i acc[20];
                    asm volatile("" ::: "memory");
                    __builtin_amdgcn_sched_barrier(0);
                    __builtin_amdgcn_s_setprio(0);
                    Mm8PhasePacked<NKB, 0>::run(acc, xs_addr, as_addr, biaspv);
                    __builtin_amdgcn_s_setprio(2);
                    __builtin_amdgcn_sched_barrier(0);
                    FS_T(3);
                    park_merged(std::integral_constant<int, 0>{}, acc);
                    keep(std::integral_constant<int, 0>{});
                    if constexpr (PK == 1) park_merged(std::integral_constant<int, 1>{}, acc);
                    else park_single(std::integral_constant<int, 1>{}, acc);
                    keep(std::integral_constant<int, 1>{});
                    if constexpr (PK == 2) {
                        park_single(std::integral_constant<int, 3>{}, acc);
                        keep(std::integral_constant<int, 3>{});
                    }
                }
                {
                    v4i acc[20];
                    asm volatile("" ::: "memory");
                    __builtin_amdgcn_sched_barrier(0);
                    FS_T(4);
                    __builtin_amdgcn_s_setprio(0);
                    Mm8PhasePacked<NKB, 1>::run(acc, xs_addr, as_addr, biaspv);
                    __builtin_amdgcn_s_setprio(2);
                    __builtin_amdgcn_sched_barrier(0);
                    FS_T(5);
                    auto pair_merged = [&](auto rc, int k) __attribute__((always_inline)) {
                        constexpr int r = decltype(rc)::value;
                        uint32_t lo = 0, hi = 0;
                        if (k < 10) { lo = (uint32_t)acc[2 * k][r]; hi = (uint32_t)acc[2 * k + 1][r]; }
                        if (k >= 2) { lo += (uint32_t)acc[2 * k - 4][r + 2]; hi += (uint32_t)acc[2 * k - 3][r + 2]; }
                        return lo + (hi << 8);
                    };
                    auto pair_single = [&](auto rc, int k) __attribute__((always_inline)) {
                        constexpr int r = decltype(rc)::value;
                        return k < 10 ? (uint32_t)acc[2 * k][r] + ((uint32_t)acc[2 * k + 1][r] << 8) : 0u;
                    };
#define FS_FM0(k) pair_merged(std::integral_constant<int, 0>{}, k)
#define FS_FM1(k) pair_merged(std::integral_constant<int, 1>{}, k)
#define FS_FS1(k) pair_single(std::integral_constant<int, 1>{}, k)
#define FS_FS3(k) pair_single(std::integral_constant<int, 3>{}, k)
#define FS_E0(k) eap[0][k]
#define FS_E1(k) eap[1][k]
#define FS_E3(k) eap[3][k]
                    if constexpr (PK == 2) { FS_REDUCE(16 * rt + 12 + g, FS_FS3, FS_E3, c0p[3]); __builtin_amdgcn_sched_barrier(0); }
                    FS_REDUCE(16 * rt + g, FS_FM0, FS_E0, c0p[0]);
                    if constexpr (PK == 1) FS_REDUCE(16 * rt + 4 + g, FS_FM1, FS_E1, c0p[1]);
                    else FS_REDUCE(16 * rt + 4 + g, FS_FS1, FS_E1, c0p[1]);
#undef FS_FM0
#undef FS_FM1
#undef FS_FS1
#undef FS_FS3
#undef FS_E0
#undef FS_E1
#undef FS_E3
                }
                FS_T(6);
                continue;
            }
            {
                v4i acc[24];
                asm volatile("" ::: "memory");
                __builtin_amdgcn_sched_barrier(0);
                __builtin_amdgcn_s_setprio(0);
                Mm8Phase<NKB, 0, false>::run(acc, xs_addr, as_addr, biasv);
                __builtin_amdgcn_s_setprio(2);
                __builtin_amdgcn_sched_barrier(0);
                FS_T(3);
#pragma unroll
                for (int reg = 0; reg < 4; reg++) {
                    if (reg >= 2 && reg >= nreg) break;
                    c0p[reg] = (uint32_t)acc[0][reg];
#pragma unroll
                    for (int j = 0; j < 11; j++) eap[reg][j] = (uint32_t)acc[1 + 2 * j][reg] + ((uint32_t)acc[2 + 2 * j][reg] << 8);
                    asm volatile("" ::"v"(c0p[reg]), "v"(eap[reg][0]), "v"(eap[reg][1]), "v"(eap[reg][2]), "v"(eap[reg][3]), "v"(eap[reg][4]),
                                 "v"(eap[reg][5]), "v"(eap[reg][6]), "v"(eap[reg][7]), "v"(eap[reg][8]), "v"(eap[reg][9]), "v"(eap[reg][10]));
                    __builtin_amdgcn_sched_barrier(0);
                }
            }
            {
                v4i acc[24];
                asm volatile("" ::: "memory");
                __builtin_amdgcn_sched_barrier(0);
                FS_T(4);
                __builtin_amdgcn_s_setprio(0);
                Mm8Phase<NKB, 1, false>::run(acc, xs_addr, as_addr, biasv);
                __builtin_amdgcn_s_setprio(2);
                __builtin_amdgcn_sched_barrier(0);
                FS_T(5);
#pragma unroll
                for (int reg = 0; reg < 4; reg++) {
                    if (reg >= 2 && reg >= nreg) break;
#define FS_F(k) ((uint32_t)acc[2 * (k)][reg] + ((uint32_t)acc[2 * (k) + 1][reg] << 8))
#define FS_E(k) eap[reg][k]
                    FS_REDUCE(16 * rt + 4 * reg + g, FS_F, FS_E, c0p[reg]);
#undef FS_F
#undef FS_E
                    if (reg & 1) __builtin_amdgcn_sched_barrier(0);
                }
            }
            FS_T(6);
        }
    }
#ifdef HB_MM8_TIMING
    if (lane == 0 && blockIdx.x < 256) for (int k = 0; k < 8; k++) g_fs_t[(blockIdx.x * 8 + wave) * 8 + k] = tacc[k];
#endif
    fs_workgroup_done(done, mismatch, first_bad);
}

typedef __int128 i128;

struct FsConsts { uint32_t c80r[9], biasmod[9], biasmod_pm[9], biasmod_ps[9]; };
constexpr int32_t FS_OVERFLOW = 0x40000000;

__device__ __forceinline__ size_t fs_digit_addr(int i, int l, int b, int nkb) {
    const int lane_ = (4 * ((i % 16) % 4) + (i % 16) / 4) + 16 * ((l % 8) / 2), el = l & 1;
    const int grp = b >> 3, r7 = 7 - (b & 7), hi = r7 >> 2, bi = r7 & 3;
    return ((((size_t)(i / 16) * nkb + l / 8) * 2 + grp) * 64 + (size_t)lane_) * 16 + 4 * (2 * hi + el) + bi;
}

__device__ __forceinline__ void fs_row_constant(const FpParams<9> &P, const FsConsts &cs, const i128 *row, int d, uint32_t *dst16, int kind = 0) {
    constexpr int NL = 9, NW = 8;
    uint32_t s5[5] = {0, 0, 0, 0, 0};
    for (int l = 0; l < d; l++) {
        const i128 v = row[l];
        const uint32_t vw[5] = {(uint32_t)v, (uint32_t)(v >> 32), (uint32_t)(v >> 64), (uint32_t)(v >> 96), (uint32_t)(v >> 127 >> 1)};
        unsigned cy = 0;
#pragma unroll
        for (int k = 0; k < 5; k++) s5[k] = __builtin_addc(s5[k], vw[k], cy, &cy);
    }
    const bool negs = (s5[4] >> 31) != 0;
    if (negs) {
        unsigned cy = 1;
#pragma unroll
        for (int k = 0; k < 5; k++) s5[k] = __builtin_addc(~s5[k], 0u, cy, &cy);
    }
    uint32_t w8[NW] = {s5[0], s5[1], s5[2], s5[3], s5[4], 0, 0, 0}, fe[NL], prod[NL], corr[NL], k80[NL], bm[NL];
    unpack<NL, NW>(fe, w8);
    if (negs) fp_neg(fe, fe, P);
#pragma unroll
    for (int k = 0; k < NL; k++) { k80[k] = cs.c80r[k]; bm[k] = kind == 0 ? cs.biasmod[k] : kind == 1 ? cs.biasmod_pm[k] : cs.biasmod_ps[k]; }
    mont_mul(prod, fe, k80, P);
    fp_sub(corr, prod, bm, P);
    uint32_t cw[NW];
    pack<NL, NW>(cw, corr);
#pragma unroll
    for (int k = 0; k < 8; k++) {
        const uint64_t pair = (uint64_t)cw[k] + ((0x1010ull << 32) | 0x10100000ull);
        dst16[2 * k] = (uint32_t)pair;
        dst16[2 * k + 1] = (uint32_t)(pair >> 32);
    }
}

__device__ __forceinline__ void fs_build_body(uint8_t *fb_lds, const FpParams<9> &P, const uint32_t *__restrict__ inv, int n, const FsIdx &ix, int d, int nc, int n_coef,
                                              int flags, const FsConsts &cs, uint8_t *__restrict__ a8, uint32_t *__restrict__ crow, uint32_t *__restrict__ KT,
                                              int32_t *__restrict__ rowmode, int32_t *__restrict__ z_dev, int32_t *__restrict__ status, const FsPack &pk) {
    constexpr int NL = 9, NW = 8;
    const int n_out = n_coef + nc, nkb = (d + 7) / 8, n_rt = (n_out + 15) / 16;
    i128 *ent = reinterpret_cast<i128 *>(fb_lds);
    i128 *Ac = ent + (size_t)n_out * d;
    uint32_t *wj = reinterpret_cast<uint32_t *>(Ac + (d + 1));
    uint32_t *part = wj + (size_t)d * NL;
    const int tid = threadIdx.x;
    const bool do_z = flags & FS_BUILD_Z, do_zc = flags & FS_BUILD_ZC;
    if (do_z) {
        const size_t img = (size_t)n_rt * nkb * 2 * 64 * 16;
        for (size_t i = tid; i < img / 16; i += 1024) reinterpret_cast<uint4 *>(a8)[i] = make_uint4(0, 0, 0, 0);
        for (int i = tid; i < n_rt * 16 * 8; i += 1024) { crow[2 * i] = 0x10100000u; crow[2 * i + 1] = 0x1010u; }
        for (int i = tid; i < n_rt * 16; i += 1024) rowmode[i] = 0;
        if (tid < d) z_dev[tid] = ix.z[tid];
    }
    if (do_z && tid < 64) {
        if (tid <= d) Ac[tid] = tid == 0 ? 1 : 0;
        __builtin_amdgcn_fence(__ATOMIC_RELEASE, "wavefront");
        __builtin_amdgcn_wave_barrier();
        for (int q = 0; q < d; q++) {
            i128 nv = 0;
            const bool act = tid <= q + 1 && tid <= d;
            if (act) nv = (tid > 0 ? Ac[tid - 1] : (i128)0) - (i128)ix.xz[q] * Ac[tid];
            __builtin_amdgcn_fence(__ATOMIC_ACQ_REL, "wavefront");
            __builtin_amdgcn_wave_barrier();
            if (act) Ac[tid] = nv;
            __builtin_amdgcn_fence(__ATOMIC_ACQ_REL, "wavefront");
            __builtin_amdgcn_wave_barrier();
        }
        if (tid < d) {
            const i128 xj = ix.xz[tid];
            i128 cur = 1;
            for (int m = d - 1; m >= 0; m--) {
                if (m < n_coef) ent[(size_t)m * d + tid] = cur;
                if (m > 0) cur = Ac[m] + xj * cur;
            }
        }
    } else if (do_z && tid < 64 + 4 * FS_MAXD + 32) {
        const int j = (tid - 64) >> 2, pq = (tid - 64) & 3;
        if (j < d) {
            uint32_t w[NL];
            fp_set(w, P.one);
            const uint32_t *row = inv + (size_t)ix.z[j] * n * NL;
            for (int q = pq; q < d; q += 4) {
                if (q == j) continue;
                uint32_t f[NL];
#pragma unroll
                for (int k = 0; k < NL; k++) f[k] = row[(size_t)ix.z[q] * NL + k];
                mont_mul(w, w, f, P);
            }
#pragma unroll
            for (int k = 0; k < NL; k++) part[((size_t)j * 4 + pq) * NL + k] = w[k];
        }
    } else if (do_zc && tid >= 256) {
        for (int e = tid - 256; e < nc * d; e += 1024 - 256) {
            const int i = e / d, j = e - i * d;
            const int64_t xi = ix.xzc[i];
            i128 v = 1;
            for (int q = 0; q < d; q++)
                if (q != j) v *= (i128)(xi - (int64_t)ix.xz[q]);
            ent[(size_t)(n_coef + i) * d + j] = v;
        }
    }
    __syncthreads();
    if (do_z && tid < d) {
        uint32_t a[NL], b[NL], c[NL];
#pragma unroll
        for (int k = 0; k < NL; k++) { a[k] = part[((size_t)tid * 4) * NL + k]; b[k] = part[((size_t)tid * 4 + 1) * NL + k]; }
        mont_mul(c, a, b, P);
#pragma unroll
        for (int k = 0; k < NL; k++) { a[k] = part[((size_t)tid * 4 + 2) * NL + k]; b[k] = part[((size_t)tid * 4 + 3) * NL + k]; }
        mont_mul(a, a, b, P);
        mont_mul(c, c, a, P);
#pragma unroll
        for (int k = 0; k < NL; k++) wj[(size_t)tid * NL + k] = c[k];
    }
    __syncthreads();
    const int row_lo = do_z ? 0 : n_coef, row_hi = do_zc ? n_out : n_coef;
    for (int e = tid + row_lo * d; e < row_hi * d; e += 1024) {
        const int i = e / d, l = e - i * d;
        i128 v = ent[e];
        const bool negv = v < 0;
        int carry = 0, kind;
        const int sl = fs_slot(pk, i, n_out, kind);
        bool lost = false;
#pragma unroll
        for (int b = 0; b < 16; b++) {
            int t = (int)((uint32_t)(v >> (8 * b)) & 0xffu) + carry;
            if (t > 127) { t -= 256; carry = 1; } else carry = 0;
            if (kind == 0) a8[fs_digit_addr(sl, l, b, nkb)] = (uint8_t)(int8_t)t;
            else if (b < 8 || kind == 1) a8[fs_digit_addr(sl + (b < 8 ? 0 : 8), l, b & 7, nkb)] = (uint8_t)(int8_t)t;
            else lost |= t != 0;
        }
        if ((lost || carry != (negv ? 1 : 0)) && status) atomicOr(status, FS_OVERFLOW);
    }
    for (int i = tid + row_lo; i < row_hi; i += 1024) {
        int kind;
        const int sl = fs_slot(pk, i, n_out, kind);
        fs_row_constant(P, cs, ent + (size_t)i * d, d, crow + (size_t)sl * 16, kind);
        rowmode[sl] = i < n_coef ? -(i + 1) : (int32_t)ix.zc[i - n_coef] + 1;
    }
    if (do_z) {
        for (int e = tid; e < d * NL; e += 1024) {
            const int l = e / NL, q = e - l * NL;
            uint32_t w[NL], two[NL], tq[NL];
#pragma unroll
            for (int k = 0; k < NL; k++) { w[k] = wj[(size_t)l * NL + k]; two[k] = (k == q) ? 1u : 0u; }
            mont_mul(tq, w, two, P);
#pragma unroll
            for (int k = 0; k < NL; k++) KT[((size_t)l * NL + q) * NL + k] = tq[k];
        }
    }
}

__device__ __forceinline__ void fs_cand_body(uint8_t *fc_lds, const FpParams<9> &P, int n, const uint16_t *__restrict__ xs, const FsIdx &ix, int d, const FsConsts &cs,
                                             uint8_t *__restrict__ cand, uint32_t *__restrict__ cand_crow, int32_t *__restrict__ status) {
    i128 *ent = reinterpret_cast<i128 *>(fc_lds);
    const int tid = threadIdx.x, nkb = (d + 7) / 8;
    const size_t row_bytes = (size_t)nkb * 8 * 16;
    for (size_t i = tid; i < (size_t)n * row_bytes / 16; i += 1024) reinterpret_cast<uint4 *>(cand)[i] = make_uint4(0, 0, 0, 0);
    for (int e = tid; e < n * d; e += 1024) {
        const int i = e / d, j = e - i * d;
        const int64_t xi = xs[i];
        i128 v = 1;
        for (int q = 0; q < d; q++)
            if (q != j) v *= (i128)(xi - (int64_t)ix.xz[q]);
        ent[e] = v;
    }
    __syncthreads();
    for (int e = tid; e < n * d; e += 1024) {
        const int i = e / d, l = e - i * d;
        const i128 v = ent[e];
        const bool negv = v < 0;
        const int kb = l >> 3, gg = (l & 7) >> 1, el = l & 1;
        int carry = 0;
#pragma unroll
        for (int b = 0; b < 16; b++) {
            int t = (int)((uint32_t)(v >> (8 * b)) & 0xffu) + carry;
            if (t > 127) { t -= 256; carry = 1; } else carry = 0;
            const int grp = b >> 3, r7 = 7 - (b & 7), hi = r7 >> 2, bi = r7 & 3;
            cand[(size_t)i * row_bytes + (size_t)(((kb * 2 + grp) * 4 + gg) * 16) + 4 * (2 * hi + el) + bi] = (uint8_t)(int8_t)t;
        }
        if (carry != (negv ? 1 : 0) && status) atomicOr(status, FS_OVERFLOW);
    }
    for (int i = tid; i < n; i += 1024) fs_row_constant(P, cs, ent + (size_t)i * d, d, cand_crow + (size_t)i * 16);
}

__global__ void __launch_bounds__(1024) k_fs_build(const FpParams<9> P, const uint32_t *__restrict__ inv, int n, const FsIdx ix, int d, int nc, int n_coef,
                                                   int flags, const FsConsts cs, uint8_t *__restrict__ a8, uint32_t *__restrict__ crow, uint32_t *__restrict__ KT,
                                                   int32_t *__restrict__ rowmode, int32_t *__restrict__ z_dev, int32_t *__restrict__ status, const FsPack pk) {
    extern __shared__ __attribute__((aligned(16))) uint8_t fs_b_lds[];
    fs_build_body(fs_b_lds, P, inv, n, ix, d, nc, n_coef, flags, cs, a8, crow, KT, rowmode, z_dev, status, pk);
}

__global__ void __launch_bounds__(1024) k_fs_cand(const FpParams<9> P, int n, const uint16_t *__restrict__ xs, const FsIdx ix, int d, const FsConsts cs,
                                                  uint8_t *__restrict__ cand, uint32_t *__restrict__ cand_crow, int32_t *__restrict__ status) {
    extern __shared__ __attribute__((aligned(16))) uint8_t fs_c_lds[];
    fs_cand_body(fs_c_lds, P, n, xs, ix, d, cs, cand, cand_crow, status);
}

__global__ void __launch_bounds__(1024) k_fs_build_z_cand(const FpParams<9> P, const uint32_t *__restrict__ inv, int n, const uint16_t *__restrict__ xs, const FsIdx ix, int d, int nc,
                                                          int n_coef, const FsConsts cs, uint8_t *__restrict__ a8, uint32_t *__restrict__ crow, uint32_t *__restrict__ KT,
                                                          int32_t *__restrict__ rowmode, int32_t *__restrict__ z_dev, uint8_t *__restrict__ cand, uint32_t *__restrict__ cand_crow,
                                                          int32_t *__restrict__ status) {
    extern __shared__ __attribute__((aligned(16))) uint8_t fs_zc_lds[];
    if (blockIdx.x == 0) fs_build_body(fs_zc_lds, P, inv, n, ix, d, nc, n_coef, FS_BUILD_Z, cs, a8, crow, KT, rowmode, z_dev, status, FsPack{});
    else fs_cand_body(fs_zc_lds, P, n, xs, ix, d, cs, cand, cand_crow, status);
}

static int fs_num_cus() {
    static int n = 0;
    if (!n) {
        int dev = 0;
        (void)hipGetDevice(&dev);
        if (hipDeviceGetAttribute(&n, hipDeviceAttributeMultiprocessorCount, dev) != hipSuccess || n <= 0) n = 256;
    }
    return n;
}

int fs_layout(hb_ctx *ctx, const PointTable *pt, int d, int nc, int n_coef, FsLayout *L) {
    if (ctx->n_limbs != 4 || !pt || !pt->usable || !pt->small) return HB_ERR_UNSUPPORTED;
    if (d < 4 || d > 22 || nc < 0 || nc > FS_MAXC || n_coef < 1 || n_coef > d) return HB_ERR_UNSUPPORTED;
    if (env_hook(ENV_NO_MFMA) || env_hook(ENV_NO_FUSED_SMALL) || env_hook(ENV_NO_QUICK) || !prescale_params(ctx)) return HB_ERR_UNSUPPORTED;
    if ((int64_t)d * 16 * 128 * 128 > MM8_BIAS) return HB_ERR_UNSUPPORTED;
    std::vector<uint16_t> xs(pt->xs);
    std::sort(xs.begin(), xs.end());
    double bits_n = 0.0, bits_p = 0.0;
    for (int k = 0; k < d - 1 && k < (int)xs.size(); k++) bits_n += log2(1.0 + xs[xs.size() - 1 - k]);
    const int R = xs.empty() ? 0 : xs.back() - xs.front();
    for (int k = 0; k < d - 1; k++) { const int dist = R - k / 2; if (dist < 1) break; bits_p += log2((double)dist); }
    if (bits_n > 124.5 || bits_p > 124.5) return HB_ERR_UNSUPPORTED;
    L->n = pt->n; L->d = d; L->nc = nc; L->n_coef = n_coef; L->n_out = n_coef + nc;
    L->nkb = (d + 7) / 8; L->n_rt = (L->n_out + 15) / 16;
    L->pk_nm = L->pk_ns = 0;
    memset(L->pk_single, 0, sizeof L->pk_single);
    if (fs_lds_bytes(L->n_rt, L->nkb) > FS_LDS_LIMIT) return HB_ERR_UNSUPPORTED;
    auto al = [](size_t v) { return (v + 255) & ~(size_t)255; };
    L->o_a8 = 0;
    L->o_crow = al((size_t)L->n_rt * L->nkb * 2 * 64 * 16);
    L->o_kt = L->o_crow + al((size_t)L->n_rt * 16 * 16 * 4);
    L->o_mode = L->o_kt + al((size_t)d * 81 * 4);
    L->o_z = L->o_mode + al((size_t)L->n_rt * 16 * 4);
    L->need = L->o_z + al((size_t)FS_MAXD * 4);
    L->o_cand = L->o_cand_crow = 0;
    if (pt->n <= FS_CAND_MAXN && nc > 0) {
        L->o_cand = L->need;
        L->o_cand_crow = L->o_cand + al((size_t)pt->n * L->nkb * 8 * 16);
        L->need = L->o_cand_crow + al((size_t)pt->n * 16 * 4);
    }
    return HB_OK;
}

static void fs_small_rows(const uint16_t *xz, int d, int n_coef, uint8_t *small) {
    i128 Ac[FS_MAXD + 1];
    for (int k = 0; k <= d; k++) Ac[k] = k == 0 ? 1 : 0;
    for (int q = 0; q < d; q++)
        for (int k = q + 1; k >= 0; k--) Ac[k] = (k > 0 ? Ac[k - 1] : (i128)0) - (i128)xz[q] * Ac[k];
    for (int m = 0; m < n_coef; m++) small[m] = 1;
    const i128 lim = (i128)1 << 62;
    for (int j = 0; j < d; j++) {
        i128 cur = 1;
        for (int m = d - 1; m >= 0; m--) {
            if (m < n_coef && (cur >= lim || cur <= -lim)) small[m] = 0;
            if (m > 0) cur = Ac[m] + (i128)xz[j] * cur;
        }
    }
}

bool fs_pack(const PointTable *pt, const int32_t *z, FsLayout *L) {
    L->pk_nm = L->pk_ns = 0;
    memset(L->pk_single, 0, sizeof L->pk_single);
    if (env_hook(ENV_NO_FUSED_PACK)) return false;
    uint16_t xz[FS_MAXD];
    uint8_t small[FS_MAXD];
    for (int i = 0; i < L->d; i++) { if (z[i] < 0 || z[i] >= L->n) return false; xz[i] = pt->xs[z[i]]; }
    fs_small_rows(xz, L->d, L->n_coef, small);
    FsPack pk;
    if (!fs_pack_decide(L->d, L->n_coef, L->nc, small, &pk)) return false;
    L->pk_nm = pk.nm; L->pk_ns = pk.ns;
    memcpy(L->pk_single, pk.single, sizeof pk.single);
    return true;
}

int fs_build(hb_ctx *ctx, const PointTable *pt, const int32_t *z, const int32_t *zc, const FsLayout &L, uint8_t *base, int flags, int32_t *status_dev, hipStream_t s) {
    const int n = L.n, d = L.d, nc = L.nc;
    FsIdx ix;
    memset(&ix, 0, sizeof ix);
    uint64_t seen[4] = {0, 0, 0, 0};
    std::vector<uint8_t> seen_big;
    if (n > 256) seen_big.assign((size_t)n, 0);
    auto mark = [&](int v) -> bool {
        if (v < 0 || v >= n) return false;
        if (n > 256) { if (seen_big[v]) return false; seen_big[v] = 1; return true; }
        if (seen[v >> 6] >> (v & 63) & 1) return false;
        seen[v >> 6] |= 1ull << (v & 63);
        return true;
    };
    for (int i = 0; i < d; i++) { if (!mark(z[i])) return fail(ctx, HB_ERR_BAD_ARG, "fused decode: arrival indices"); ix.z[i] = (uint16_t)z[i]; ix.xz[i] = pt->xs[z[i]]; }
    if (flags & FS_BUILD_ZC)
        for (int j = 0; j < nc; j++) { if (!mark(zc[j])) return fail(ctx, HB_ERR_BAD_ARG, "fused decode: compared indices"); ix.zc[j] = (uint16_t)zc[j]; ix.xzc[j] = pt->xs[zc[j]]; }
    const Mm8Shared *sh = nullptr;
    int rc = mm8_shared(ctx, &sh, s); if (rc) return rc;
    FsConsts cs;
    memcpy(cs.c80r, sh->c80r, sizeof cs.c80r);
    memcpy(cs.biasmod, sh->biasmod, sizeof cs.biasmod);
    memcpy(cs.biasmod_pm, sh->biasmod_pm, sizeof cs.biasmod_pm);
    memcpy(cs.biasmod_ps, sh->biasmod_ps, sizeof cs.biasmod_ps);
    FsPack pk;
    memset(&pk, 0, sizeof pk);
    if (L.pk_nm) {
        if (flags != (FS_BUILD_Z | FS_BUILD_ZC)) return fail(ctx, HB_ERR_BAD_ARG, "fused decode: a packed image is built in one piece");
        pk.nm = L.pk_nm; pk.ns = L.pk_ns;
        memcpy(pk.single, L.pk_single, sizeof pk.single);
    }
    const size_t lds = ((size_t)L.n_out * d + d + 1) * 16 + ((size_t)d * 9 + (size_t)d * 4 * 9) * 4;
    k_fs_build<<<1, 1024, lds, s>>>(ctx->pw, pt->inv, n, ix, d, nc, L.n_coef, flags, cs, base + L.o_a8, (uint32_t *)(base + L.o_crow), (uint32_t *)(base + L.o_kt),
                                    (int32_t *)(base + L.o_mode), (int32_t *)(base + L.o_z), status_dev, pk);
    HB_LAUNCH_CHECK(ctx);
    return HB_OK;
}

int fs_build_cand(hb_ctx *ctx, PointTable *pt, const int32_t *z, const FsLayout &L, uint8_t *base, int32_t *status_dev, hipStream_t s, bool with_z) {
    if (!L.o_cand) return fail(ctx, HB_ERR_BAD_ARG, "fused decode: no candidate store in this layout");
    if (!pt->xs_dev) {
        HB_HIP(ctx, hipMalloc(&pt->xs_dev, (size_t)pt->n * 2));
        int rc = upload_table(ctx, pt->xs_dev, pt->xs.data(), (size_t)pt->n * 2, s);
        if (rc) { (void)hipFree(pt->xs_dev); pt->xs_dev = nullptr; return rc; }
    }
    FsIdx ix;
    memset(&ix, 0, sizeof ix);
    uint64_t seen[2] = {0, 0};
    for (int i = 0; i < L.d; i++) {
        const int v = z[i];
        if (v < 0 || v >= pt->n || (seen[v >> 6] >> (v & 63) & 1)) return fail(ctx, HB_ERR_BAD_ARG, "fused decode: arrival indices");
        seen[v >> 6] |= 1ull << (v & 63);
        ix.z[i] = (uint16_t)v; ix.xz[i] = pt->xs[v];
    }
    const Mm8Shared *sh = nullptr;
    int rc = mm8_shared(ctx, &sh, s); if (rc) return rc;
    FsConsts cs;
    memcpy(cs.c80r, sh->c80r, sizeof cs.c80r);
    memcpy(cs.biasmod, sh->biasmod, sizeof cs.biasmod);
    memset(cs.biasmod_pm, 0, sizeof cs.biasmod_pm);
    memset(cs.biasmod_ps, 0, sizeof cs.biasmod_ps);
    if (with_z) {
        const size_t lds_b = ((size_t)L.n_out * L.d + L.d + 1) * 16 + ((size_t)L.d * 9 + (size_t)L.d * 4 * 9) * 4, lds_c = (size_t)pt->n * L.d * 16;
        k_fs_build_z_cand<<<2, 1024, std::max(lds_b, lds_c), s>>>(ctx->pw, pt->inv, pt->n, pt->xs_dev, ix, L.d, L.nc, L.n_coef, cs, base + L.o_a8, (uint32_t *)(base + L.o_crow),
                                                                  (uint32_t *)(base + L.o_kt), (int32_t *)(base + L.o_mode), (int32_t *)(base + L.o_z), base + L.o_cand,
                                                                  (uint32_t *)(base + L.o_cand_crow), status_dev);
        HB_LAUNCH_CHECK(ctx);
        return HB_OK;
    }
    k_fs_cand<<<1, 1024, (size_t)pt->n * L.d * 16, s>>>(ctx->pw, pt->n, pt->xs_dev, ix, L.d, cs, base + L.o_cand, (uint32_t *)(base + L.o_cand_crow), status_dev);
    HB_LAUNCH_CHECK(ctx);
    return HB_OK;
}

static std::atomic<int> g_fs_last_pack{-1};

static FsSplit fs_split(int d, int n_rt, int n_out, int pk_nm, int pk_ns) {
    constexpr int PASS = 95, RAGGED = 70, TERM = 36, PACKED2 = 50, PACKED3 = 55;
    const int packed = pk_ns ? PACKED3 : PACKED2;
    FsSplit sp;
    int load[FS_WAVES];
    const int n_pairs = FS_TPW * n_rt;
    const bool ragged = n_out - 16 * (n_rt - 1) <= 8;
    for (int w = 0; w < FS_WAVES; w++) {
        sp.terms[w] = 0;
        load[w] = 0;
        for (int pidx = w; pidx < n_pairs; pidx += FS_WAVES) {
            const int tl = n_rt == 2 ? (pidx >> 1) : pidx / n_rt;
            const int rt = n_rt == 2 ? ((pidx ^ (pidx >> 2)) & 1) : pidx - tl * n_rt;
            load[w] += (pk_nm && rt == n_rt - 1) ? packed : (ragged && rt == n_rt - 1) ? RAGGED : PASS;
        }
    }
    for (int l = 0; l < d; l++) {
        int best = FS_WAVES - 1;
        for (int w = FS_WAVES - 2; w >= 0; w--)
            if (load[w] < load[best]) best = w;
        sp.terms[best] |= 1u << l;
        load[best] += TERM;
    }
    return sp;
}

int fs_launch(hb_ctx *ctx, const FsLayout &L, const uint8_t *base, const uint32_t *cols, hb_view cv, uint32_t *out, hb_view ov, int64_t out_count,
              int32_t *mismatch_dev, int32_t *first_bad_dev, uint32_t *bad_map_dev, int64_t C, hipStream_t s, const FsDone *done_p, const int32_t *pick_zc) {
    FsDone done;
    memset(&done, 0, sizeof done);
    if (done_p) done = *done_p;
    FsPick pick;
    memset(&pick, 0, sizeof pick);
    if (pick_zc) {
        if (L.pk_nm) return fail(ctx, HB_ERR_BAD_ARG, "fused decode: a packed image has no rows to pick");
        if (!L.o_cand) return fail(ctx, HB_ERR_BAD_ARG, "fused decode: no candidate store to pick from");
        pick.cand = (const uint4 *)(base + L.o_cand); pick.cand_crow = (const uint32_t *)(base + L.o_cand_crow);
        pick.n_coef = L.n_coef; pick.nc = L.nc;
        for (int j = 0; j < L.nc; j++) pick.zc[j] = (uint16_t)pick_zc[j];
    }
    if (C <= 0) return HB_OK;
    const Mm8Shared *sh = nullptr;
    int rc = mm8_shared(ctx, &sh, s); if (rc) return rc;
    const int64_t n_units = (C + 63) / 64;
    int64_t blocks = fs_num_cus();
    if (blocks > n_units) blocks = n_units;
    blocks = mm8_trimmed_grid(n_units, blocks);
    const size_t lds = fs_lds_bytes(L.n_rt, L.nkb);
    const FsSplit split = fs_split(L.d, L.n_rt, L.n_out, L.pk_nm, L.pk_ns);
    const int pack = !L.pk_nm ? 0 : L.pk_ns ? 2 : 1;
    g_fs_last_pack.store(pack);
#define FS_LAUNCH(NKB, PK)                                                                                                                   \
    do {                                                                                                                                   \
        static std::atomic<unsigned long long> attr_done{0};                                                                                                        \
        if (!((attr_done.load() >> (ctx->device & 63)) & 1ull)) { HB_HIP(ctx, hipFuncSetAttribute(reinterpret_cast<const void *>(k_mm8f<NKB, PK>), hipFuncAttributeMaxDynamicSharedMemorySize, 160 * 1024)); attr_done.fetch_or(1ull << (ctx->device & 63)); } \
        k_mm8f<NKB, PK><<<dim3((unsigned)blocks), dim3(64 * FS_WAVES), lds, s>>>((const int4 *)(base + L.o_a8), (const uint32_t *)(base + L.o_crow), sh->fold_dev,        \
            (const uint32_t *)(base + L.o_kt), ctx->psc, cols, cv.stride_c, cv.stride_l, (const int32_t *)(base + L.o_z), INT64_MAX, L.d, (const int32_t *)(base + L.o_mode), \
            out, ov.stride_c, ov.stride_l, out_count, mismatch_dev, first_bad_dev, bad_map_dev, L.n_out, L.n_rt, C, n_units, sh->bp, done, pick, split); \
    } while (0)
    switch (L.nkb) {
        case 1: if (pack == 1) FS_LAUNCH(1, 1); else if (pack == 2) FS_LAUNCH(1, 2); else FS_LAUNCH(1, 0); break;
        case 2: if (pack == 1) FS_LAUNCH(2, 1); else if (pack == 2) FS_LAUNCH(2, 2); else FS_LAUNCH(2, 0); break;
        case 3: if (pack == 1) FS_LAUNCH(3, 1); else if (pack == 2) FS_LAUNCH(3, 2); else FS_LAUNCH(3, 0); break;
        default: return fail(ctx, HB_ERR_UNSUPPORTED, "fused decode: more than 24 terms");
    }
#undef FS_LAUNCH
    HB_LAUNCH_CHECK(ctx);
    return HB_OK;
}

}

extern "C" int hb_debug_fs_pack_rows(int d, int n_coef, int nc, const uint8_t *small, int32_t *out) {
    hb::FsPack pk;
    const bool ok = d >= 1 && d <= hb::FS_MAXD && n_coef >= 1 && n_coef <= d && nc >= 0 && nc <= hb::FS_MAXC && hb::fs_pack_decide(d, n_coef, nc, small, &pk);
    if (!ok) memset(&pk, 0, sizeof pk);
    out[0] = pk.nm; out[1] = pk.ns;
    for (int k = 0; k < 8; k++) out[2 + k] = pk.single[k];
    return ok ? 1 : 0;
}
extern "C" int hb_debug_fs_pack_points(const int32_t *xz, int d, int n_coef, int nc, int32_t *out, uint8_t *small_out) {
    if (d < 1 || d > hb::FS_MAXD || n_coef < 1 || n_coef > d) return 0;
    uint16_t x16[hb::FS_MAXD];
    uint8_t small[hb::FS_MAXD];
    for (int i = 0; i < d; i++) x16[i] = (uint16_t)xz[i];
    hb::fs_small_rows(x16, d, n_coef, small);
    if (small_out) memcpy(small_out, small, (size_t)n_coef);
    return hb_debug_fs_pack_rows(d, n_coef, nc, small, out);
}
extern "C" int hb_debug_fs_last_pack(void) { return hb::g_fs_last_pack.load(); }
extern "C" int hb_debug_fs_slot(int nm, int ns, const int32_t *single, int i, int n_out, int32_t *kind) {
    hb::FsPack pk;
    memset(&pk, 0, sizeof pk);
    pk.nm = nm; pk.ns = ns;
    for (int k = 0; k < 8 && k < ns; k++) pk.single[k] = (uint8_t)single[k];
    int kd = 0;
    const int sl = hb::fs_slot(pk, i, n_out, kd);
    *kind = kd;
    return sl;
}

#ifdef HB_MM8_TIMING
extern "C" int hb_debug_fs_timing(unsigned long long *out, int count) {
    return hipMemcpyFromSymbol(out, HIP_SYMBOL(hb::g_fs_t), sizeof(unsigned long long) * (size_t)count) == hipSuccess ? 0 : 1;
}
#endif
```

honeybadgermpc_amd/csrc/hb_mm8.hpp:

```cpp
#pragma once
#include "hb_common.hpp"

namespace hb {

typedef int v4i __attribute__((ext_vector_type(4)));

constexpr int MM8_NC = 47;
constexpr int MM8_CW = 13;
constexpr int MM8_FOLD_ROW = 272;
constexpr int MM8_FOLD_Q = 8 * MM8_FOLD_ROW / 16;
constexpr int MM8_BIAS = 5800000;
constexpr int MM8_NCP = 39;
constexpr int MM8_BIAS_PACK = MM8_BIAS / 2;

struct BarrettParams {
    uint32_t pneg[8];
    uint32_t c384[8];
    uint32_t mu;
};

struct Mm8Matrix {
    int n_out, d, nkb, n_rt;
    bool skip01;
    int4 *a8;
    uint32_t *crow;
    uint32_t *zero;
    BarrettParams bp;
};

struct Mm8Shared {
    BarrettParams bp;
    uint32_t c80r[9], biasmod[9];
    uint32_t biasmod_pm[9], biasmod_ps[9];
    uint8_t fold_host[MM8_FOLD_Q * 16];
    v4i *fold_dev;
};
int mm8_shared(hb_ctx *ctx, const Mm8Shared **out, hipStream_t s);
int64_t mm8_trimmed_grid(int64_t n_units, int64_t blocks);
void mm8_shared_free(hb_ctx *ctx);

}
```

honeybadgermpc_amd/csrc/hb_open.hip:

```cpp
#include "hb_common.hpp"

using namespace hb;

struct hb_open_plan {
    hb_ctx *ctx;
    int n, d, n_check;
    int64_t max_B, max_C;
    FastMatrix *V;
    FastMatrix *Vinv;
    Mm8Matrix *V8;
    Mm8Matrix *Vzc8;
    int32_t *zc_dev, *ones_dev;
    std::vector<int32_t> zc;
    std::vector<int32_t> z;
    std::vector<uint64_t> x;
    Mm8Matrix *Vinv8;
    uint32_t *scaled_pk;
    int use_v8;
    int use_fused;
    int fused_pending;
    int decode_calls;
    int32_t *z_dev;
    int32_t *mask_dev;
    uint32_t *in_dg;
    uint32_t *coef_dg;
    int32_t *mismatch_dev;
    int validate_arrived_only;
    int ntt_order;
    uint32_t *tw;
    uint32_t *coef_pk;
    hb_matrix *Winv;
    const Mm8wMatrix *Winv8;
    hb_matrix *Vw;
    const Mm8wMatrix *Vw8;
    Mm8wMatrix *F1, *F2;
    int32_t *fmap1, *fmap2;
    uint8_t *q1, *q2;
    QuickLayout l1, l2;
    const Mm8wShared *qsh;
    uint8_t *fs1, *fs2;
    FsLayout fl1, fl2;
    Mv64Matrix *nv_enc, *nv_f1, *nv_f2;
};

static void build_quick_wide(hb_open_plan *pl, hipStream_t s) {
    hb_ctx *ctx = pl->ctx;
    if (pl->q1 || env_hook(ENV_NO_QUICK_PLAN)) return;
    QuickLayout a, b;
    const int n = pl->n, d = pl->d, n_check = pl->n_check;
    if (quick_layout(ctx, n, d, n_check, 1, &a) == HB_OK && quick_layout(ctx, n, d, n_check, d, &b) == HB_OK) {
        uint8_t *b1 = nullptr, *b2 = nullptr;
        const Mm8wShared *sh = nullptr;
        int qrc = HB_OK;
        if (hipMalloc(&b1, a.need) != hipSuccess || hipMalloc(&b2, b.need) != hipSuccess) qrc = HB_ERR_HIP;
        const int32_t *zcp = n_check > 0 ? pl->zc.data() : pl->z.data();
        if (!qrc) qrc = quick_build(ctx, pl->x.data(), pl->z.data(), zcp, a, b1, &sh, s);
        if (!qrc) qrc = quick_build(ctx, pl->x.data(), pl->z.data(), zcp, b, b2, &sh, s);
        if (!qrc) { pl->q1 = b1; pl->q2 = b2; pl->l1 = a; pl->l2 = b; pl->qsh = sh; pl->fused_pending = 0; }
        else { if (b1) (void)hipFree(b1); if (b2) (void)hipFree(b2); }
    }
    ctx->err.clear();
}

static void build_fused_small(hb_open_plan *pl, hipStream_t s) {
    hb_ctx *ctx = pl->ctx;
    if (pl->fs1 || env_hook(ENV_NO_QUICK_PLAN) || env_hook(ENV_NO_QUICK)) return;
    PointTable *pt = nullptr;
    FsLayout a, b;
    if (point_table(ctx, pl->x.data(), pl->n, &pt, s) == HB_OK && fs_layout(ctx, pt, pl->d, pl->n_check, 1, &a) == HB_OK &&
        fs_layout(ctx, pt, pl->d, pl->n_check, pl->d, &b) == HB_OK) {
        uint8_t *b1 = nullptr, *b2 = nullptr;
        int qrc = HB_OK;
        if (hipMalloc(&b1, a.need) != hipSuccess || hipMalloc(&b2, b.need) != hipSuccess) qrc = HB_ERR_HIP;
        const int32_t *zcp = pl->n_check > 0 ? pl->zc.data() : pl->z.data();
        if (!qrc) { (void)fs_pack(pt, pl->z.data(), &a); (void)fs_pack(pt, pl->z.data(), &b); }
        if (!qrc) qrc = fs_build(ctx, pt, pl->z.data(), zcp, a, b1, FS_BUILD_Z | FS_BUILD_ZC, pl->mismatch_dev, s);
        if (!qrc) qrc = fs_build(ctx, pt, pl->z.data(), zcp, b, b2, FS_BUILD_Z | FS_BUILD_ZC, pl->mismatch_dev, s);
        if (!qrc) { pl->fs1 = b1; pl->fs2 = b2; pl->fl1 = a; pl->fl2 = b; pl->fused_pending = 0; }
        else { if (b1) (void)hipFree(b1); if (b2) (void)hipFree(b2); }
    }
    ctx->err.clear();
}

static int valu_planes(hb_open_plan *pl) {
    if (pl->in_dg && pl->coef_dg) return HB_OK;
    hb_ctx *ctx = pl->ctx;
    const size_t bytes = (size_t)pl->max_C * pl->d * ctx->nl() * 4;
    if (!pl->in_dg && hipMalloc(&pl->in_dg, bytes) != hipSuccess) return fail(ctx, HB_ERR_HIP, "open plan: hipMalloc(in_dg)");
    if (!pl->coef_dg && hipMalloc(&pl->coef_dg, bytes) != hipSuccess) return fail(ctx, HB_ERR_HIP, "open plan: hipMalloc(coef_dg)");
    return HB_OK;
}

static int build_fused(hb_open_plan *pl, const uint64_t *x_host, hipStream_t s) {
    hb_ctx *ctx = pl->ctx;
    const int d = pl->d, nc = pl->n_check, L = ctx->n_limbs;
    std::vector<uint64_t> W((size_t)d * d * L), P((size_t)nc * d * L);
    int rc = hb_matrix_to_host(ctx, pl->Winv, W.data(), s);
    if (rc) return rc;
    if (nc > 0) {
        std::vector<uint64_t> xzc((size_t)nc * L);
        for (int j = 0; j < nc; j++) memcpy(&xzc[(size_t)j * L], x_host + (size_t)pl->zc[j] * L, (size_t)L * 8);
        hb_matrix *Vzc = nullptr;
        uint32_t *Wd = nullptr, *Pd = nullptr;
        rc = hb_vand_matrix_create(ctx, xzc.data(), nc, d, &Vzc, s);
        if (!rc) rc = upload_elems(ctx, W.data(), (size_t)d * d, &Wd, s);
        if (!rc && hipMalloc(&Pd, P.size() * 8) != hipSuccess) rc = fail(ctx, HB_ERR_HIP, "fused validate: hipMalloc");
        if (!rc) rc = hb_matvec(ctx, Vzc, (const uint64_t *)Wd, hb_view{1, d}, nullptr, (uint64_t *)Pd, hb_view{1, d}, d, s);
        if (!rc && hipMemcpyAsync(P.data(), Pd, P.size() * 8, hipMemcpyDeviceToHost, s) != hipSuccess) rc = fail(ctx, HB_ERR_HIP, "fused validate: copy");
        if (!rc && hipStreamSynchronize(s) != hipSuccess) rc = fail(ctx, HB_ERR_HIP, "fused validate: sync");
        if (Vzc) matrix_unref(Vzc);
        if (Wd) (void)hipFree(Wd);
        if (Pd) (void)hipFree(Pd);
        if (rc) return rc;
    }
    std::vector<uint64_t> m2((size_t)(d + nc) * d * L), m1((size_t)(1 + nc) * d * L);
    memcpy(m2.data(), W.data(), W.size() * 8);
    memcpy(m1.data(), W.data(), (size_t)d * L * 8);
    if (nc > 0) {
        memcpy(&m2[(size_t)d * d * L], P.data(), P.size() * 8);
        memcpy(&m1[(size_t)d * L], P.data(), P.size() * 8);
    }
    std::vector<int32_t> map2((size_t)d + nc + 1, 0), map1((size_t)1 + nc + 1, 0);
    for (int j = 0; j < nc; j++) { map2[(size_t)d + j] = pl->zc[j] + 1; map1[(size_t)1 + j] = pl->zc[j] + 1; }
    rc = mm8w_from_host(ctx, m2.data(), d + nc, d, &pl->F2, s);
    if (!rc) rc = mm8w_from_host(ctx, m1.data(), 1 + nc, d, &pl->F1, s);
    if (!rc) rc = own_int_array(ctx, map2.data(), (int)map2.size(), &pl->fmap2, s);
    if (!rc) rc = own_int_array(ctx, map1.data(), (int)map1.size(), &pl->fmap1, s);
    if (rc) {
        mm8w_free(pl->F1); mm8w_free(pl->F2); pl->F1 = pl->F2 = nullptr;
        if (pl->fmap1) { (void)hipFree(pl->fmap1); pl->fmap1 = nullptr; }
        if (pl->fmap2) { (void)hipFree(pl->fmap2); pl->fmap2 = nullptr; }
        return rc == HB_ERR_UNSUPPORTED ? HB_OK : rc;
    }
    return HB_OK;
}

static int ensure_fused(hb_open_plan *pl, hipStream_t s) {
    pl->fused_pending = 0;
    if (pl->q1 || pl->F1 || pl->d < 4 || pl->n < 4 || env_hook(ENV_NO_MFMA_DECODE)) return HB_OK;
    hb_ctx *ctx = pl->ctx;
    const int L = ctx->n_limbs;
    if (!pl->Winv) {
        std::vector<uint64_t> xz((size_t)pl->d * L);
        for (int i = 0; i < pl->d; i++) memcpy(&xz[(size_t)i * L], &pl->x[(size_t)pl->z[i] * L], (size_t)L * 8);
        int rc = hb_vand_inverse_create(ctx, xz.data(), pl->d, &pl->Winv, (void *)s);
        if (rc) return rc;
        pl->Winv8 = matrix_wide(ctx, pl->Winv, s);
    }
    return pl->Winv8 ? build_fused(pl, pl->x.data(), s) : HB_OK;
}

extern "C" {

int hb_open_plan_create(hb_ctx *ctx, int n, int d, int use_omega_powers, const uint64_t *x_host,
                        const uint64_t *omega_host, int order, const int32_t *z_host, const int32_t *zc_host,
                        int n_check, int64_t max_B, hb_open_plan **out, void *stream) { HB_API_GUARD(ctx);
    if (!ctx || !out || n <= 0 || d <= 0 || d > n || !x_host || !z_host || max_B < 0) return HB_ERR_BAD_ARG;
    if (n_check < 0 || n_check > n || (n_check > 0 && !zc_host)) return HB_ERR_BAD_ARG;
    for (int i = 0; i < d; i++) if (z_host[i] < 0 || z_host[i] >= n) return HB_ERR_BAD_ARG;
    for (int j = 0; j < n_check; j++) if (zc_host[j] < 0 || zc_host[j] >= n) return HB_ERR_BAD_ARG;
    *out = nullptr;
    hipStream_t s = (hipStream_t)stream;
    cache_trim(ctx);
    hb_open_plan *pl = new hb_open_plan();
    pl->ctx = ctx; pl->n = n; pl->d = d; pl->n_check = n_check; pl->max_B = max_B;
    pl->max_C = (max_B + d - 1) / d; if (pl->max_C < 1) pl->max_C = 1;
    pl->use_v8 = 1;
    pl->use_fused = 1;
    const int L = ctx->n_limbs;
    uint32_t *xd = nullptr, *xzd = nullptr;
    int rc = HB_OK;
#define PLAN_HIP(call) do { hipError_t e__ = (call); if (e__ != hipSuccess) { ctx->err = std::string(#call) + ": " + hipGetErrorString(e__); rc = HB_ERR_HIP; goto done; } } while (0)
    {
        std::vector<uint64_t> xz((size_t)d * L);
        for (int i = 0; i < d; i++) memcpy(&xz[(size_t)i * L], x_host + (size_t)z_host[i] * L, (size_t)L * 8);
        rc = upload_elems(ctx, x_host, (size_t)n, &xd, s); if (rc) goto done;
        rc = upload_elems(ctx, xz.data(), (size_t)d, &xzd, s); if (rc) goto done;
        rc = fast_vand_create(ctx, xd, n, d, &pl->V, s);
        if (!rc) rc = fast_vinv_create(ctx, xzd, d, &pl->Vinv, s);
        (void)hipStreamSynchronize(s);
        if (rc) goto done;
    }
    rc = own_int_array(ctx, z_host, d, &pl->z_dev, s); if (rc) goto done;
    pl->z.assign(z_host, z_host + d);
    pl->x.assign(x_host, x_host + (size_t)n * L);
    {
        std::vector<int32_t> mask((size_t)n + 1, 0);
        mask[n] = -1;
        for (int j = 0; j < n_check; j++) { mask[zc_host[j]] = 1; pl->zc.push_back(zc_host[j]); }
        rc = own_int_array(ctx, mask.data(), n + 1, &pl->mask_dev, s); if (rc) goto done;
    }
    if (use_omega_powers && omega_host && order >= n && order > 0 && (order & (order - 1)) == 0) {
        int logn = 0; while ((1 << logn) < order) logn++;
        const double nl2 = (double)ctx->nl() * ctx->nl();
        const double mv = (double)n * d * nl2, ntt = 0.5 * order * logn * (2.0 * nl2 + 4.0 * ctx->nl());
        if (ntt < mv && (size_t)order * ctx->nl() * 4 <= 40 * 1024) {
            rc = get_twiddles(ctx, omega_host, order, &pl->tw, s); if (rc) goto done;
            pl->ntt_order = order;
            PLAN_HIP(hipMalloc(&pl->coef_pk, (size_t)pl->max_C * d * ctx->elem_words() * 4));
        }
    }
    if (!pl->ntt_order) {
        rc = mm8_from_fast(ctx, pl->V, &pl->V8, s);
        if (rc && rc != HB_ERR_UNSUPPORTED) goto done;
        rc = HB_OK;
        if (pl->V8) {
            PLAN_HIP(hipMalloc(&pl->coef_pk, (size_t)pl->max_C * d * ctx->elem_words() * 4));
            rc = env_hook(ENV_NO_MFMA_DECODE) ? HB_ERR_UNSUPPORTED : mm8_from_fast(ctx, pl->Vinv, &pl->Vinv8, s);
            if (rc && rc != HB_ERR_UNSUPPORTED) goto done;
            rc = HB_OK;
            if (pl->Vinv8) PLAN_HIP(hipMalloc(&pl->scaled_pk, (size_t)pl->max_C * d * ctx->elem_words() * 4));
        }
    }
    if (!pl->V8 && d >= 4 && n >= 4 && !env_hook(ENV_NO_MFMA_DECODE)) {
        std::vector<uint64_t> xz((size_t)d * L);
        for (int i = 0; i < d; i++) memcpy(&xz[(size_t)i * L], x_host + (size_t)z_host[i] * L, (size_t)L * 8);
        rc = hb_vand_inverse_create(ctx, xz.data(), d, &pl->Winv, stream); if (rc) goto done;
        pl->Winv8 = matrix_wide(ctx, pl->Winv, s);
        if (!pl->ntt_order) {
            rc = hb_vand_matrix_create(ctx, x_host, n, d, &pl->Vw, stream); if (rc) goto done;
            pl->Vw8 = matrix_wide(ctx, pl->Vw, s);
        }
        if ((pl->Winv8 || pl->Vw8) && !pl->coef_pk) PLAN_HIP(hipMalloc(&pl->coef_pk, (size_t)pl->max_C * d * ctx->elem_words() * 4));
    }
    if (mv64_applies(ctx, d) && (!use_omega_powers || mv64_matrix_cores(ctx, d))) {
        std::vector<uint64_t> Vh, Vi, Ph;
        rc = mv64_plan_tables(ctx, x_host, n, d, z_host, zc_host, n_check, Vh, Vi, Ph);
        if (rc) goto done;
// ... 226 lines not shown
```

honeybadgermpc_amd/csrc/hb_quick.hip:

```cpp
#include <algorithm>
#include <atomic>
#include <chrono>

#include "hb_common.hpp"

using namespace hb;

namespace hb {

constexpr int QUICK_MAX = 128;
constexpr int QUICK_MAXC = 256;
constexpr int PROBE_MAXN = 256;
constexpr int PROBE_NT = 1024;

struct QuickIdx { uint16_t z[QUICK_MAX], zc[QUICK_MAXC]; };
struct ProbeIdx { uint16_t idx[PROBE_MAXN]; };

template <int NL> __device__ __forceinline__ void ldg(uint32_t (&r)[NL], const uint32_t *p) {
#pragma unroll
    for (int i = 0; i < NL; i++) r[i] = p[i];
}
template <int NL> __device__ __forceinline__ void stg(uint32_t *p, const uint32_t (&r)[NL]) {
#pragma unroll
    for (int i = 0; i < NL; i++) p[i] = r[i];
// ... 936 lines not shown
    int wgs;
};

extern "C" {

}

namespace hb {

int quick_layout(hb_ctx *ctx, int n, int d, int nc, int n_coef, QuickLayout *L) {
    if (ctx->n_limbs != 4 || d < 4 || d > QUICK_MAX || nc < 0 || nc > QUICK_MAXC || n > 65535 || n_coef < 1 || n_coef > d) return fail(ctx, HB_ERR_UNSUPPORTED, "quick: shape");
    if (env_hook(ENV_NO_MFMA) || env_hook(ENV_NO_MFMA_WIDE) || env_hook(ENV_NO_QUICK)) return fail(ctx, HB_ERR_UNSUPPORTED, "quick: disabled");
    if (!prescale_params(ctx) || (ctx->p_limbs[3] >> 56) > 0x7e) return fail(ctx, HB_ERR_UNSUPPORTED, "quick: modulus");
    L->n = n; L->d = d; L->nc = nc; L->n_coef = n_coef; L->n_out = n_coef + nc;
    int n_rt = 0;
    size_t a8_bytes = 0, crow_words = 0;
    const int rc = mm8w_geometry(L->n_out, d, &L->tile_rows, &n_rt, &L->nkb, &a8_bytes, &crow_words);
    if (rc) return fail(ctx, rc, "quick: geometry");
    auto al = [](size_t v) { return (v + 255) & ~(size_t)255; };
    L->o_a8 = 0; L->o_crow = L->o_a8 + al(a8_bytes); L->o_wj = L->o_crow + al(crow_words * 4); L->o_full = L->o_wj + al((size_t)d * 36);
    L->o_nraw = L->o_full + al((size_t)(nc ? nc : 1) * 36); L->o_mcan = L->o_nraw + al((size_t)n_coef * d * 36);
    L->o_z = L->o_mcan + al((size_t)L->n_out * d * 32); L->o_map = L->o_z + al((size_t)d * 4); L->o_sync = L->o_map + al((size_t)(L->n_out + 2) * 4);
    L->need = L->o_sync + al((size_t)(d + 1) * 36 + 64);
    L->o_cand = L->o_cand_crow = 0;
    return HB_OK;
}

int quick_layout_cand(hb_ctx *ctx, QuickLayout *L) {
    (void)ctx;
    if (L->nc < 1 || L->n > 1024 || L->d > QF_NT || env_hook(ENV_QUICK_NO_CAND)) return HB_ERR_UNSUPPORTED;
    auto al = [](size_t v) { return (v + 255) & ~(size_t)255; };
    L->o_full = L->need;
    L->o_cand = L->o_full + al((size_t)L->n * 36);
    L->o_cand_crow = L->o_cand + al((size_t)L->n * L->nkb * 16 * 16);
    L->need = L->o_cand_crow + al((size_t)L->n * 16 * 4);
    return HB_OK;
}

int quick_build(hb_ctx *ctx, const uint64_t *x_host, const int32_t *z, const int32_t *zc, const QuickLayout &L, uint8_t *base, const Mm8wShared **shared, hipStream_t s, int flags) {
    const int n = L.n, d = L.d, nc = L.nc;
    const bool do_z = flags & 1, do_zc = flags & 2, cand = (flags & 4) && L.o_cand;
    std::vector<uint8_t> seen((size_t)n, 0);
    for (int i = 0; i < d; i++) { if (z[i] < 0 || z[i] >= n || seen[z[i]]) return fail(ctx, HB_ERR_BAD_ARG, "quick: arrival indices"); seen[z[i]] = 1; }
    if (do_zc)
        for (int j = 0; j < nc; j++) { if (zc[j] < 0 || zc[j] >= n || seen[zc[j]]) return fail(ctx, HB_ERR_BAD_ARG, "quick: compared indices"); seen[zc[j]] = 1; }
    PointTable *pt = nullptr;
    int rc = point_table(ctx, x_host, n, &pt, s); if (rc) return rc;
    if (!pt->usable) return fail(ctx, HB_ERR_UNSUPPORTED, "quick: repeated points");
    const Mm8wShared *sh = nullptr;
    rc = mm8w_shared(ctx, d, &sh, s); if (rc) return rc;
    *shared = sh;
    QuickIdx ix;
    memset(&ix, 0, sizeof ix);
    for (int i = 0; i < d; i++) ix.z[i] = (uint16_t)z[i];
    if (do_zc) for (int j = 0; j < nc; j++) ix.zc[j] = (uint16_t)zc[j];
    uint32_t *wj = (uint32_t *)(base + L.o_wj), *full = (uint32_t *)(base + L.o_full), *nraw = (uint32_t *)(base + L.o_nraw), *mcan = (uint32_t *)(base + L.o_mcan);
    QuickRowConst rcs;
    memcpy(rcs.c80r, sh->c80r, sizeof rcs.c80r);
    memcpy(rcs.biasmod, sh->biasmod, sizeof rcs.biasmod);
    if (cand && do_zc && !do_z) {
        if (nc > 0) {
            k_quick_pick<<<(unsigned)((nc * L.nkb * 16 + 255) / 256), 256, 0, s>>>(ix, nc, L.n_coef, L.tile_rows, L.nkb, (const uint4 *)(base + L.o_cand),
                                                                                 (const uint32_t *)(base + L.o_cand_crow), (uint4 *)(base + L.o_a8), (uint32_t *)(base + L.o_crow),
                                                                                 (int32_t *)(base + L.o_map));
            HB_LAUNCH_CHECK(ctx);
        }
        return HB_OK;
    }
    const int row_lo = do_z ? 0 : L.n_coef, row_hi = do_zc ? L.n_out : L.n_coef;
    const int frows = (cand && do_z) ? n : nc;
    if (do_z || nc > 0) {
        const int nw = (d + QM_FPB - 1) / QM_FPB, nf = std::max(1, (frows + QM_FPB - 1) / QM_FPB);
        const int nh = L.n_coef == 1 ? nw : ((do_z && d > 40) ? 4 : 1);
        const size_t lds = (size_t)std::max((4 + QM_SEG) * d + 1, d + QM_FSEG * QM_FPB) * 36;
        k_quick_matrix<9><<<nh + nw + nf + (do_z ? 1 : 0), QM_NT, lds, s>>>(ctx->pw, pt->xm, pt->inv, n, ix, d, nc, L.n_coef, wj, full, nraw, (int32_t *)(base + L.o_z),
                                                          (int32_t *)(base + L.o_map), (flags & 3) | (cand && do_z ? 4 : 0), (uint4 *)base, (int)(L.o_wj / 16),
                                                          (uint4 *)(base + L.o_cand), (cand && do_z) ? (int)((L.o_cand_crow - L.o_cand) / 16) : 0,
                                                          nh, nw, nf, pt->pw, pt->S);
    }
    HB_LAUNCH_CHECK(ctx);
    if (cand && do_z) {
        k_quick_fill<<<(unsigned)(L.n_coef + n), QF_NT, 0, s>>>(ctx->pw, pt->inv, n, ix, d, L.n_coef, wj, full, nraw, base + L.o_a8, (uint32_t *)(base + L.o_crow),
                                                               L.tile_rows, L.nkb, rcs, base + L.o_cand, (uint32_t *)(base + L.o_cand_crow), 0);
        HB_LAUNCH_CHECK(ctx);
        return HB_OK;
    }
    if (do_z && do_zc && d <= QF_NT) {
        k_quick_fill<<<(unsigned)L.n_out, QF_NT, 0, s>>>(ctx->pw, pt->inv, n, ix, d, L.n_coef, wj, full, nraw, base + L.o_a8, (uint32_t *)(base + L.o_crow),
                                                        L.tile_rows, L.nkb, rcs, nullptr, nullptr, 1);
        HB_LAUNCH_CHECK(ctx);
        return HB_OK;
    }
    if (row_hi > row_lo) {
        k_quick_image<<<(unsigned)(((row_hi - row_lo) * d + 255) / 256), 256, 0, s>>>(ctx->pw, pt->inv, n, ix, d, nc, L.n_coef, wj, full, nraw, mcan, base + L.o_a8, L.tile_rows, L.nkb, row_lo, row_hi);
        HB_LAUNCH_CHECK(ctx);
        k_quick_rows<<<(unsigned)((row_hi - row_lo + 63) / 64), 64, 0, s>>>(ctx->pw, mcan, row_lo, row_hi, d, rcs, (uint32_t *)(base + L.o_crow), L.tile_rows);
        HB_LAUNCH_CHECK(ctx);
    }
    return HB_OK;
}

int quick_launch(hb_ctx *ctx, const QuickLayout &L, const uint8_t *base, const Mm8wShared *sh, const uint32_t *cols, hb_view cv, uint32_t *out, hb_view ov,
                 int64_t out_count, int n_store, int32_t *mismatch_dev, int32_t *first_bad_dev, int64_t C, hipStream_t s, uint32_t *bad_map_dev, const FsDone *done) {
    const int32_t *fmap = (const int32_t *)(base + L.o_map);
    return launch_mm8w_raw(ctx, L.n_out, L.d, L.tile_rows, (const void *)(base + L.o_a8), (const uint32_t *)(base + L.o_crow), sh,
                           cols, cv, (const int32_t *)(base + L.o_z), INT64_MAX, out, ov, out_count,
                           L.nc > 0 ? fmap : nullptr, mismatch_dev, C, s, cols, cv, n_store, L.nc > 0 ? first_bad_dev : nullptr, L.nc > 0 ? bad_map_dev : nullptr,
                           L.nc > 0 ? done : nullptr);
}

}

extern "C" {

int hb_quick_interp_check(hb_ctx *ctx, const uint64_t *x_host, int n, const int32_t *z, int d, const int32_t *zc, int nc,
                          const uint64_t *cols_dev, int64_t C, int64_t chunk_lo, int64_t chunk_hi, uint64_t *coeffs_dev, int32_t *status_dev, void *stream) {
    return hb_quick_interp_check_map(ctx, x_host, n, z, d, zc, nc, cols_dev, C, chunk_lo, chunk_hi, coeffs_dev, status_dev, nullptr, stream);
}

int hb_quick_interp_check_map(hb_ctx *ctx, const uint64_t *x_host, int n, const int32_t *z, int d, const int32_t *zc, int nc,
                              const uint64_t *cols_dev, int64_t C, int64_t chunk_lo, int64_t chunk_hi, uint64_t *coeffs_dev, int32_t *status_dev,
                              uint32_t *bad_map_dev, void *stream) { HB_API_GUARD(ctx);
    if (!ctx || !x_host || !z || n < 1 || d < 1 || d > n || nc < 0 || (nc > 0 && !zc) || C < 0 || chunk_lo < 0 || chunk_hi > C || chunk_lo > chunk_hi) return HB_ERR_BAD_ARG;
    if (chunk_hi == chunk_lo) return HB_OK;
    if (!cols_dev || (nc > 0 && !status_dev)) return HB_ERR_BAD_ARG;
    hipStream_t s = (hipStream_t)stream;
    cache_trim(ctx);
    auto take_slot = [&](size_t need, hb_ctx::QuickSlot **out) -> int {
        if (ctx->qslots.empty()) ctx->qslots.resize(4);
        hb_ctx::QuickSlot &sl = ctx->qslots[ctx->qnext++ % ctx->qslots.size()];
        if (sl.ev) HB_HIP(ctx, hipEventSynchronize((hipEvent_t)sl.ev));
        else { hipEvent_t ev; HB_HIP(ctx, hipEventCreateWithFlags(&ev, hipEventDisableTiming)); sl.ev = ev; }
        if (sl.cap < need) {
            if (sl.buf) HB_HIP(ctx, hipFree(sl.buf));
            sl.buf = nullptr; sl.cap = 0;
            HB_HIP(ctx, hipMalloc(&sl.buf, need));
            sl.cap = need;
        }
        *out = &sl;
        return HB_OK;
    };
    const int64_t cnt = chunk_hi - chunk_lo;
    const uint32_t *in = (const uint32_t *)cols_dev + (size_t)chunk_lo * 8;
    hb_view pm{1, C}, dv{d, 1};
    if (ctx->n_limbs == 4 && !env_hook(ENV_NO_QUICK)) {
        PointTable *pt = nullptr;
        FsLayout F;
        int rc = point_table(ctx, x_host, n, &pt, s); if (rc) return rc;
        if (fs_layout(ctx, pt, d, nc, coeffs_dev ? d : 1, &F) == HB_OK) {
            hb_ctx::QuickSlot *sl = nullptr;
            rc = take_slot(F.need, &sl); if (rc) return rc;
            uint8_t *base = static_cast<uint8_t *>(sl->buf);
            (void)fs_pack(pt, z, &F);
            rc = fs_build(ctx, pt, z, zc, F, base, FS_BUILD_Z | FS_BUILD_ZC, status_dev, s); if (rc) return rc;
            uint32_t *out = coeffs_dev ? (uint32_t *)coeffs_dev + (size_t)chunk_lo * d * 8 : nullptr;
            rc = fs_launch(ctx, F, base, in, pm, out, dv, coeffs_dev ? cnt * (int64_t)d : 0, status_dev, (nc > 0 && status_dev) ? status_dev + 1 : nullptr,
                           nc > 0 ? bad_map_dev : nullptr, cnt, s);
            if (rc) return rc;
            HB_HIP(ctx, hipEventRecord((hipEvent_t)sl->ev, s));
            return HB_OK;
        }
    }
    QuickLayout L;
    int rc = quick_layout(ctx, n, d, nc, coeffs_dev ? d : 1, &L); if (rc) return rc;
    hb_ctx::QuickSlot *slp = nullptr;
    rc = take_slot(L.need, &slp); if (rc) return rc;
    hb_ctx::QuickSlot &sl = *slp;
    uint8_t *base = static_cast<uint8_t *>(sl.buf);
    const Mm8wShared *sh = nullptr;
    rc = quick_build(ctx, x_host, z, zc, L, base, &sh, s); if (rc) return rc;
    uint32_t *out = coeffs_dev ? (uint32_t *)coeffs_dev + (size_t)chunk_lo * d * 8 : (uint32_t *)(base + L.o_mcan);
    rc = quick_launch(ctx, L, base, sh, in, pm, out, dv, coeffs_dev ? cnt * (int64_t)d : 0, coeffs_dev ? d : 0, status_dev, status_dev ? status_dev + 1 : nullptr, cnt, s, bad_map_dev);
    if (rc) return rc;
    HB_HIP(ctx, hipEventRecord((hipEvent_t)sl.ev, s));
    return HB_OK;
}

}

__global__ void k_publish_verdict(int32_t *status, FsVerdict *host, int seq) {
    fs_publish_verdict(status, status + 1, nullptr, host, seq);
}

static hipError_t ctx_side_stream(hb_ctx *ctx, hipStream_t *out) {
    if (!ctx->side_stream) {
        int lo_prio = 0, hi_prio = 0;
        (void)hipDeviceGetStreamPriorityRange(&lo_prio, &hi_prio);
        hipStream_t ss = nullptr;
        const hipError_t e = hipStreamCreateWithPriority(&ss, hipStreamNonBlocking, hi_prio);
        if (e != hipSuccess) return e;
        ctx->side_stream = ss;
    }
    *out = (hipStream_t)ctx->side_stream;
    return hipSuccess;
}
extern "C" int hb_side_stream(hb_ctx *ctx, void **stream) { HB_API_GUARD(ctx);
    if (!ctx || !stream) return HB_ERR_BAD_ARG;
    hipStream_t ss = nullptr;
    HB_HIP(ctx, ctx_side_stream(ctx, &ss));
    *stream = ss;
    return HB_OK;
}

struct hb_quick_dec {
    hb_ctx *ctx;
    int n;
    PointTable *pt;
    bool wide;
    QuickLayout Q;
    const Mm8wShared *qsh;
    std::vector<uint64_t> x;
    FsLayout L;
    uint8_t *buf;
    size_t cap;
    int32_t *status;
    FsVerdict *res_host, *res_dev;
    int seq;
    bool prepared;
    std::vector<int32_t> z;
    hipStream_t bstream;
    hipEvent_t built, launched;
    bool launch_open;
    hipStream_t launch_stream;
    bool beside;
    bool built_beside;
};

namespace hb {
int quick_dec_supported(hb_quick_dec *qd, int d, int nc, int n_coef) { HB_API_GUARD((qd ? qd->ctx : nullptr));
    if (!qd || d < 1 || d > qd->n || nc < 0 || n_coef < 1 || n_coef > d) return HB_ERR_BAD_ARG;
    FsLayout L;
    if (fs_layout(qd->ctx, qd->pt, d, nc, n_coef, &L) == HB_OK) return HB_OK;
    QuickLayout Q;
    return quick_layout(qd->ctx, qd->n, d, nc, n_coef, &Q);
}
}

extern "C" {

int hb_quick_dec_create(hb_ctx *ctx, const uint64_t *x_host, int n, hb_quick_dec **out, void *stream) { HB_API_GUARD(ctx);
    if (!ctx || !x_host || !out || n < 1) return HB_ERR_BAD_ARG;
    *out = nullptr;
    if (ctx->n_limbs != 4 || env_hook(ENV_NO_QUICK)) return fail(ctx, HB_ERR_UNSUPPORTED, "quick decoder: narrow context or disabled");
    hipStream_t s = (hipStream_t)stream;
    cache_trim(ctx);
    PointTable *pt = nullptr;
    int rc = point_table(ctx, x_host, n, &pt, s); if (rc) return rc;
    if (!pt->usable) return fail(ctx, HB_ERR_UNSUPPORTED, "quick decoder: repeated points");
    if (n > 65535) return fail(ctx, HB_ERR_UNSUPPORTED, "quick decoder: more than 65535 points");
    hb_quick_dec *qd = new hb_quick_dec();
    qd->ctx = ctx; qd->n = n; qd->pt = pt; qd->wide = false; qd->qsh = nullptr; qd->x.assign(x_host, x_host + (size_t)n * 4); qd->buf = nullptr; qd->cap = 0; qd->status = nullptr; qd->res_host = qd->res_dev = nullptr; qd->seq = 0; qd->prepared = false;
    const int32_t init[4] = {0, INT32_MAX, 0, 0};
    hipError_t e = hipMalloc(&qd->status, sizeof init);
    if (e == hipSuccess) e = hipMemcpyAsync(qd->status, init, sizeof init, hipMemcpyHostToDevice, s);
    if (e == hipSuccess) e = hipStreamSynchronize(s);
    if (e == hipSuccess) e = hipHostMalloc((void **)&qd->res_host, sizeof(FsVerdict), hipHostMallocMapped);
    if (e == hipSuccess) e = hipHostGetDevicePointer((void **)&qd->res_dev, qd->res_host, 0);
    qd->bstream = nullptr; qd->built = qd->launched = nullptr; qd->launch_open = false; qd->launch_stream = nullptr; qd->beside = qd->built_beside = false;
    if (e == hipSuccess) e = ctx_side_stream(ctx, &qd->bstream);
    if (e == hipSuccess) e = hipEventCreateWithFlags(&qd->built, hipEventDisableTiming);
    if (e == hipSuccess) e = hipEventCreateWithFlags(&qd->launched, hipEventDisableTiming);
    if (e != hipSuccess) {
        if (qd->status) (void)hipFree(qd->status);
        if (qd->res_host) (void)hipHostFree(qd->res_host);
        if (qd->built) (void)hipEventDestroy(qd->built);
        if (qd->launched) (void)hipEventDestroy(qd->launched);
        delete qd;
        ctx->err = std::string("quick decoder: ") + hipGetErrorString(e);
        return HB_ERR_HIP;
    }
    memset(qd->res_host, 0, sizeof(FsVerdict));
    pt->refs++;
    *out = qd;
    return HB_OK;
}

int hb_quick_dec_arrivals(hb_quick_dec *qd, const int32_t *z, int d, int nc, int n_coef, void *stream) { HB_API_GUARD((qd ? qd->ctx : nullptr));
    if (!qd || !z || d < 1 || d > qd->n || nc < 0 || n_coef < 1 || n_coef > d) return HB_ERR_BAD_ARG;
    hb_ctx *ctx = qd->ctx;
    hipStream_t s = (hipStream_t)stream;
    qd->prepared = false;
    hipStream_t bs = qd->beside ? qd->bstream : s;
    qd->built_beside = false;
    if (qd->launch_open && qd->launch_stream != bs) { HB_HIP(ctx, hipStreamWaitEvent(bs, qd->launched, 0)); }
    FsLayout L;
    int rc = fs_layout(ctx, qd->pt, d, nc, n_coef, &L);
    if (rc) {
        QuickLayout Q;
        rc = quick_layout(ctx, qd->n, d, nc, n_coef, &Q);
        if (rc) return rc;
        (void)quick_layout_cand(ctx, &Q);
        if (qd->cap < Q.need) {
            if (qd->buf) { HB_HIP(ctx, hipStreamSynchronize(s)); HB_HIP(ctx, hipStreamSynchronize(qd->bstream)); HB_HIP(ctx, hipFree(qd->buf)); }
            qd->buf = nullptr; qd->cap = 0;
            HB_HIP(ctx, hipMalloc(&qd->buf, Q.need));
            qd->cap = Q.need;
        }
        rc = quick_build(ctx, qd->x.data(), z, nullptr, Q, qd->buf, &qd->qsh, bs, 1 | 4); if (rc) return rc;
        if (bs != s) { HB_HIP(ctx, hipEventRecord(qd->built, bs)); qd->built_beside = true; }
        qd->Q = Q;
        qd->wide = true;
        qd->z.assign(z, z + d);
        qd->prepared = true;
        return HB_OK;
    }
    qd->wide = false;
// ... 357 lines not shown
```

include/hbmpc_hip_debug.h:

```cpp
#ifndef HBMPC_HIP_DEBUG_H
#define HBMPC_HIP_DEBUG_H

#include "hbmpc_hip.h"

#ifdef __cplusplus
extern "C" {
#endif

int hb_debug_mm8_create(hb_ctx *ctx, const uint64_t *x_host, int n, int d, void **out);
int hb_debug_mm8_apply(hb_ctx *ctx, void *mat, const void *in_dev, int64_t in_sc, int64_t in_sl, int64_t in_count,
                       void *out_dev, int64_t out_sc, int64_t out_sl, int64_t out_count, int64_t n_chunks,
                       const int32_t *check_mask_dev, int32_t *mismatch_dev);
int hb_debug_occupancy(int n_in, int nl, int *mv3, int *dc);
void hb_debug_reload_env(void);
void hb_debug_pm_slab_bytes(int64_t bytes);
void hb_debug_rf_stats(int64_t *out);
void hb_debug_rf_profile(int on);
void hb_debug_mat_split(int mode);
int hb_debug_matvec_route(hb_ctx *ctx, const hb_matrix *m, int64_t C, int32_t *out);
int hb_debug_fs_pack_rows(int d, int n_coef, int nc, const uint8_t *small, int32_t *out);
int hb_debug_fs_pack_points(const int32_t *xz, int d, int n_coef, int nc, int32_t *out, uint8_t *small_out);
int hb_debug_fs_slot(int nm, int ns, const int32_t *single, int i, int n_out, int32_t *kind);
int hb_debug_fs_last_pack(void);


#ifdef __cplusplus
}
#endif
#endif
```

Measured before the change: 8.554 billion.

## Move fused-decode input prescale onto int8 matrix cores with one-word Barrett

Replaces the per-share scalar 9-limb prescale multiply (KT table, two-word Barrett quotient) in the fused decode kernel with int8 MFMA products against a byte-split, per-point scale table built in LDS. The partial sums are folded and reduced with a single-word Barrett quotient. The build kernel now emits signed-digit tables plus a bias correction, and the work split gives these terms a lower cost weight. In exchange it adds LDS footprint, extra table preload registers, and a new signed-digit overflow path.

```diff
diff --git a/honeybadgermpc_amd/_capi.py b/honeybadgermpc_amd/_capi.py
--- a/honeybadgermpc_amd/_capi.py
+++ b/honeybadgermpc_amd/_capi.py
@@ -211,6 +211,7 @@
     "hb_debug_fs_pack_points": (_i, [_vp, _i, _i, _i, _vp, _vp]),
     "hb_debug_fs_slot": (_i, [_i, _i, _vp, _i, _i, _vp]),
     "hb_debug_fs_last_pack": (_i, []),
+    "hb_debug_fs_last_mscale": (_i, []),
 }
 
 _lib = None
diff --git a/honeybadgermpc_amd/csrc/hb_common.hpp b/honeybadgermpc_amd/csrc/hb_common.hpp
--- a/honeybadgermpc_amd/csrc/hb_common.hpp
+++ b/honeybadgermpc_amd/csrc/hb_common.hpp
@@ -101,6 +101,7 @@
     ENV_MM8W_TILE16,
     ENV_MM8_NO_SKIP,
     ENV_NO_EVAL_FEW,
+    ENV_NO_FUSED_MSCALE,
     ENV_NO_FUSED_PACK,
     ENV_NO_FUSED_SMALL,
     ENV_NO_FUSED_VALIDATE,
@@ -355,11 +356,14 @@
     size_t o_a8, o_crow, o_kt, o_mode, o_z, o_cand, o_cand_crow, need;
     int pk_nm, pk_ns;
     uint8_t pk_single[8];
+    size_t o_ms;
+    int mscale;
 };
 constexpr int FS_BUILD_Z = 1, FS_BUILD_ZC = 2;
 int fs_layout(hb_ctx *ctx, const PointTable *pt, int d, int nc, int n_coef, FsLayout *L);
 int fs_build(hb_ctx *ctx, const PointTable *pt, const int32_t *z, const int32_t *zc, const FsLayout &L, uint8_t *base, int flags, int32_t *status_dev, hipStream_t s);
 bool fs_pack(const PointTable *pt, const int32_t *z, FsLayout *L);
+bool fs_mscale(FsLayout *L);
 int fs_launch(hb_ctx *ctx, const FsLayout &L, const uint8_t *base, const uint32_t *cols, hb_view cv, uint32_t *out, hb_view ov, int64_t out_count,
               int32_t *mismatch_dev, int32_t *first_bad_dev, uint32_t *bad_map_dev, int64_t C, hipStream_t s, const FsDone *done = nullptr,
               const int32_t *pick_zc = nullptr);
diff --git a/honeybadgermpc_amd/csrc/hb_core.hip b/honeybadgermpc_amd/csrc/hb_core.hip
--- a/honeybadgermpc_amd/csrc/hb_core.hip
+++ b/honeybadgermpc_amd/csrc/hb_core.hip
@@ -448,7 +448,7 @@
 
 
 namespace hb {
-static const char *const ENV_NAMES[ENV_COUNT] = {"HB_CACHE_CAP", "HB_GAO_PAIR", "HB_MM8W_FLAT", "HB_MM8W_RQ", "HB_MM8W_TILE16", "HB_MM8_NO_SKIP", "HB_NO_EVAL_FEW", "HB_NO_FUSED_PACK", "HB_NO_FUSED_SMALL", "HB_NO_FUSED_VALIDATE", "HB_NO_MFMA", "HB_NO_MFMA_DECODE", "HB_NO_MFMA_WIDE", "HB_NO_NARROW_FAST", "HB_NO_QUICK", "HB_NO_QUICK_PLAN", "HB_NTT_STAGE_LOOP", "HB_PROBE_WGS", "HB_QUICK_NO_CAND", "HB_UPLOAD_MODE", "HB_WB_NO_GAO", "HB_WB_NO_UNIFORM"};
+static const char *const ENV_NAMES[ENV_COUNT] = {"HB_CACHE_CAP", "HB_GAO_PAIR", "HB_MM8W_FLAT", "HB_MM8W_RQ", "HB_MM8W_TILE16", "HB_MM8_NO_SKIP", "HB_NO_EVAL_FEW", "HB_NO_FUSED_MSCALE", "HB_NO_FUSED_PACK", "HB_NO_FUSED_SMALL", "HB_NO_FUSED_VALIDATE", "HB_NO_MFMA", "HB_NO_MFMA_DECODE", "HB_NO_MFMA_WIDE", "HB_NO_NARROW_FAST", "HB_NO_QUICK", "HB_NO_QUICK_PLAN", "HB_NTT_STAGE_LOOP", "HB_PROBE_WGS", "HB_QUICK_NO_CAND", "HB_UPLOAD_MODE", "HB_WB_NO_GAO", "HB_WB_NO_UNIFORM"};
 static std::string g_env_val[ENV_COUNT];
 static bool g_env_set[ENV_COUNT];
 static std::once_flag g_env_once;
diff --git a/honeybadgermpc_amd/csrc/hb_mfma.hip b/honeybadgermpc_amd/csrc/hb_mfma.hip
--- a/honeybadgermpc_amd/csrc/hb_mfma.hip
+++ b/honeybadgermpc_amd/csrc/hb_mfma.hip
@@ -440,6 +440,12 @@
         Big c80(8, 0x80808080u);
         Big r261(9, 0); r261[8] = 1u << 5;
         digits9(big_divmod(big_mul(c80, r261), p, nullptr), sh->c80r);
+    }
+    {
+        digits9(big_divmod(Big(8, 0x80808080u), p, nullptr), sh->ms_c80);
+        Big bt(10, 0);
+        for (int c = 0; c < 32; c++) { Big t(1, 1u << 20); big_add(bt, big_shl(t, 8 * c, 10)); }
+        digits9(big_divmod(bt, p, nullptr), sh->ms_bias);
     }
     if (hipMalloc(&sh->fold_dev, sizeof sh->fold_host) != hipSuccess) { delete sh; return fail(ctx, HB_ERR_HIP, "mm8: hipMalloc(fold table)"); }
     if (int rc = upload_table(ctx, sh->fold_dev, sh->fold_host, sizeof sh->fold_host, s)) { (void)hipFree(sh->fold_dev); delete sh; return rc; }
diff --git a/honeybadgermpc_amd/csrc/hb_mfma_fused.hip b/honeybadgermpc_amd/csrc/hb_mfma_fused.hip
--- a/honeybadgermpc_amd/csrc/hb_mfma_fused.hip
+++ b/honeybadgermpc_amd/csrc/hb_mfma_fused.hip
@@ -53,8 +53,10 @@
 }
 constexpr int FS_CAND_MAXN = 128;
 
-__host__ __device__ inline size_t fs_lds_bytes(int n_rt, int nkb) {
-    return ((size_t)n_rt * 64 + (size_t)n_rt * nkb * 2 * 64 + (size_t)2 * FS_TPW * nkb * 4 * 64 + MM8_FOLD_Q) * 16 + (size_t)(32 + 16 * n_rt) * 4;
+__host__ __device__ inline int fs_ms_q(int d) { return (d + 1) * 64 + d * 8; }
+__host__ __device__ inline size_t fs_lds_bytes(int n_rt, int nkb, int ms_d = 0) {
+    return ((size_t)n_rt * 64 + (size_t)n_rt * nkb * 2 * 64 + (size_t)2 * FS_TPW * nkb * 4 * 64 + MM8_FOLD_Q + (ms_d ? fs_ms_q(ms_d) : 0)) * 16 +
+           (size_t)(32 + 16 * n_rt) * 4;
 }
 
 #define FS_REDUCE(I_, F_, E_, C0_) \
@@ -150,7 +152,7 @@
         if (st && oidx < out_count) store_words<8>(out_pk + oidx * 8, ow); \
     } while (0)
 
-template <int NKB, int PK>
+template <int NKB, int PK, bool MSC>
 __global__ __launch_bounds__(64 * FS_WAVES, 2) void k_mm8f(const int4 *__restrict__ a8, const uint32_t *__restrict__ crowd, const v4i *__restrict__ foldg,
                                                           const uint32_t *__restrict__ KT, const PrescaleParams PP,
                                                           const uint32_t *__restrict__ in_pk, int64_t in_sc, int64_t in_sl, const int32_t *__restrict__ in_rows,
@@ -158,7 +160,7 @@
                                                           uint32_t *__restrict__ out_pk, int64_t out_sc, int64_t out_sl, int64_t out_count,
                                                           int32_t *__restrict__ mismatch, int32_t *__restrict__ first_bad, uint32_t *__restrict__ bad_map,
                                                           int n_out, int n_rt, int64_t n_chunks, int64_t n_units, BarrettParams bp, const FsDone done, const FsPick pick,
-                                                          const FsSplit split) {
+                                                          const FsSplit split, const v4i *__restrict__ MS) {
     constexpr bool PACKED = PK != 0;
     const int n_slots = PACKED ? 16 * n_rt : n_out;
     constexpr int NT = 64 * FS_WAVES, NL = 9, NW = 8;
@@ -172,6 +174,7 @@
     int32_t *rowl = reinterpret_cast<int32_t *>(xbuf + 2 * bufsz);
     int32_t *maskl = rowl + 32;
     v4i *foldl = reinterpret_cast<v4i *>(maskl + 16 * n_rt);
+    v4i *msl = foldl + MM8_FOLD_Q;
 
 #ifdef HB_MM8_TIMING
     unsigned long long tacc[8] = {0, 0, 0, 0, 0, 0, 0, 0}, tlast = __builtin_amdgcn_s_memtime();
@@ -210,7 +213,14 @@
         v4i img[3];
 #pragma unroll
         for (int k = 0; k < 3; k++) img[k] = reinterpret_cast<const v4i *>(a8)[tid + k * NT < n_img ? tid + k * NT : 0];
+        const int n_ms = MSC ? fs_ms_q(d) : 0;
+        v4i msv[4];
+        if constexpr (MSC) {
+#pragma unroll
+            for (int k = 0; k < 4; k++) msv[k] = MS[tid + k * NT < n_ms ? tid + k * NT : 0];
+        }
         asm volatile("" : "+v"(rw), "+v"(mk), "+v"(cr), "+v"(fo), "+v"(img[0]), "+v"(img[1]), "+v"(img[2]));
+        if constexpr (MSC) asm volatile("" : "+v"(msv[0]), "+v"(msv[1]), "+v"(msv[2]), "+v"(msv[3]));
         if (tid < 32) rowl[tid] = rw;
         if (tid < n_mask) maskl[tid] = tid < n_slots ? mk : 0;
         if (tid < n_crow) reinterpret_cast<v4i *>(fs_lds)[tid] = cr;
@@ -218,9 +228,16 @@
 #pragma unroll
         for (int k = 0; k < 3; k++)
             if (tid + k * NT < n_img) reinterpret_cast<v4i *>(abuf)[tid + k * NT] = img[k];
+        if constexpr (MSC) {
+#pragma unroll
+            for (int k = 0; k < 4; k++)
+                if (tid + k * NT < n_ms) msl[tid + k * NT] = msv[k];
+        }
         for (int i = tid + NT; i < n_mask; i += NT) maskl[i] = i < n_slots ? rowmode[i] : 0;
         for (int i = tid + NT; i < n_crow; i += NT) fs_lds[i] = reinterpret_cast<const uint4 *>(crowd)[i];
         for (int i = tid + 3 * NT; i < n_img; i += NT) abuf[i] = a8[i];
+        if constexpr (MSC)
+            for (int i = tid + 4 * NT; i < n_ms; i += NT) msl[i] = MS[i];
     }
     for (int i = threadIdx.x; i < (8 * NKB - d) * 256; i += NT) {
         const int l = d + (i >> 8), b = (i >> 7) & 1, t = (i >> 5) & 3, h = (i >> 4) & 1, c = i & 15;
@@ -230,6 +247,8 @@
     const int n_pairs = FS_TPW * n_rt;
     const uint32_t my_terms = (uint32_t)__builtin_amdgcn_readfirstlane((int)split.terms[wave]);
 
+    uint32_t ms64k = 1u << 16;
+    if constexpr (MSC) asm volatile("" : "+s"(ms64k));
     auto scale_unit = [&](auto first, int64_t unit, uint4 *dst, uint32_t terms) {
         constexpr bool FIRST = decltype(first)::value;
         const int64_t chunk = unit_chunk(unit);
@@ -250,46 +269,78 @@
             uint32_t xn[NW];
             bool okn = false;
             fetch(ln < d ? ln : l, xn, okn);
-            const uint32_t *__restrict__ T = KT + (size_t)l * (NL * NL);
-            uint32_t xd[NL];
-            unpack<NL, NW>(xd, xw);
-            uint64_t col[NL + 1];
-#pragma unroll
-            for (int j = 0; j <= NL; j++) col[j] = 0;
-#pragma unroll
-            for (int q = 0; q < NL; q++)
-#pragma unroll
-                for (int j = 0; j < NL; j++) col[j] += (uint64_t)xd[q] * T[q * NL + j];
-            uint32_t v[NL + 1];
-#pragma unroll
-            for (int k = 0; k < NL; k++) { v[k] = (uint32_t)col[k] & DMASK; col[k + 1] += col[k] >> LB; }
-            v[NL] = (uint32_t)col[NL];
-            const uint64_t mid = (uint64_t)v[9] * PP.m0 + (uint64_t)v[8] * PP.m1 + (((uint64_t)v[8] * PP.m0) >> LB);
-            const uint64_t qh = (uint64_t)v[9] * PP.m1 + (mid >> LB);
-            const uint32_t q0 = (uint32_t)qh & DMASK, q1 = (uint32_t)(qh >> LB);
-            uint64_t dc[NL];
-#pragma unroll
-            for (int k = 0; k < NL; k++) {
-                dc[k] = v[k] + (uint64_t)q0 * PP.pbar[k];
-                if (k > 0) dc[k] += (uint64_t)q1 * PP.pbar[k - 1];
+            uint32_t w[NW];
+            bool over;
+            if constexpr (MSC) {
+                const v4i *tab;
+                if constexpr (FIRST) tab = MS; else tab = msl;
+                const v4i *al = tab + (g == (n >> 2) ? l * 64 + (n & 3) : d * 64);
+                const v4i *cl = tab + (d + 1) * 64 + l * 8;
+                const v4i b0 = v4i{(int)(xw[0] ^ 0x80808080u), (int)(xw[1] ^ 0x80808080u), (int)(xw[2] ^ 0x80808080u), (int)(xw[3] ^ 0x80808080u)};
+                const v4i b1 = v4i{(int)(xw[4] ^ 0x80808080u), (int)(xw[5] ^ 0x80808080u), (int)(xw[6] ^ 0x80808080u), (int)(xw[7] ^ 0x80808080u)};
+                v4i mc[8];
+#pragma unroll
+                for (int eb = 0; eb < 8; eb++) mc[eb] = __builtin_amdgcn_mfma_i32_16x16x64_i8(al[eb * 4], b0, cl[eb], 0, 0, 0);
+#pragma unroll
+                for (int eb = 0; eb < 8; eb++) mc[eb] = __builtin_amdgcn_mfma_i32_16x16x64_i8(al[32 + eb * 4], b1, mc[eb], 0, 0, 0);
+                uint64_t mw[8];
+#pragma unroll
+                for (int k = 0; k < 8; k++) {
+                    const uint32_t lo = (uint32_t)mc[k][0] + ((uint32_t)mc[k][1] << 8), hi = (uint32_t)mc[k][2] + ((uint32_t)mc[k][3] << 8);
+                    mw[k] = (uint64_t)hi * ms64k + lo;
+                }
+                const uint64_t tq = mw[7] + (mw[6] >> 32);
+                const uint32_t mq = (uint32_t)(((uint64_t)(uint32_t)(tq >> 16) * bp.mu) >> 46);
+#pragma unroll
+                for (int k = 0; k < 8; k++) mw[k] += (uint64_t)mq * bp.pneg[k];
+                unsigned cyw = 0;
+                w[0] = (uint32_t)mw[0];
+#pragma unroll
+                for (int k = 1; k < 8; k++) w[k] = __builtin_addc((uint32_t)mw[k], (uint32_t)(mw[k - 1] >> 32), cyw, &cyw);
+                over = (uint32_t)(mw[7] >> 32) + cyw != mq;
+            } else {
+                const uint32_t *__restrict__ T = KT + (size_t)l * (NL * NL);
+                uint32_t xd[NL];
+                unpack<NL, NW>(xd, xw);
+                uint64_t col[NL + 1];
+#pragma unroll
+                for (int j = 0; j <= NL; j++) col[j] = 0;
+#pragma unroll
+                for (int q = 0; q < NL; q++)
+#pragma unroll
+                    for (int j = 0; j < NL; j++) col[j] += (uint64_t)xd[q] * T[q * NL + j];
+                uint32_t v[NL + 1];
+#pragma unroll
+                for (int k = 0; k < NL; k++) { v[k] = (uint32_t)col[k] & DMASK; col[k + 1] += col[k] >> LB; }
+                v[NL] = (uint32_t)col[NL];
+                const uint64_t mid = (uint64_t)v[9] * PP.m0 + (uint64_t)v[8] * PP.m1 + (((uint64_t)v[8] * PP.m0) >> LB);
+                const uint64_t qh = (uint64_t)v[9] * PP.m1 + (mid >> LB);
+                const uint32_t q0 = (uint32_t)qh & DMASK, q1 = (uint32_t)(qh >> LB);
+                uint64_t dc[NL];
+#pragma unroll
+                for (int k = 0; k < NL; k++) {
+                    dc[k] = v[k] + (uint64_t)q0 * PP.pbar[k];
+                    if (k > 0) dc[k] += (uint64_t)q1 * PP.pbar[k - 1];
+                }
+                uint32_t r[NL];
+#pragma unroll
+                for (int k = 0; k < NL; k++) {
+                    r[k] = (uint32_t)dc[k] & DMASK;
+                    if (k < NL - 1) dc[k + 1] += dc[k] >> LB;
+                }
+                pack<NL, NW>(w, r);
+                over = (r[NL - 1] >> 24) != 0;
             }
-            uint32_t r[NL];
-#pragma unroll
-            for (int k = 0; k < NL; k++) {
-                r[k] = (uint32_t)dc[k] & DMASK;
-                if (k < NL - 1) dc[k + 1] += dc[k] >> LB;
-            }
-            uint32_t w[NW];
-            pack<NL, NW>(w, r);
-            if (PP.pneg[NW - 1] >> 31) {
+            const uint32_t *pneg = MSC ? bp.pneg : PP.pneg;
+            if (pneg[NW - 1] >> 31) {
 #pragma unroll
                 for (int k = 0; k < NW; k++) w[k] = ok ? w[k] : 0u;
             } else {
                 uint32_t u[NW];
                 unsigned cy = 0;
 #pragma unroll
-                for (int k = 0; k < NW; k++) u[k] = __builtin_addc(w[k], PP.pneg[k], cy, &cy);
-                const bool take = cy || (r[NL - 1] >> 24);
+                for (int k = 0; k < NW; k++) u[k] = __builtin_addc(w[k], pneg[k], cy, &cy);
+                const bool take = cy || over;
 #pragma unroll
                 for (int k = 0; k < NW; k++) w[k] = ok ? (take ? u[k] : w[k]) : 0u;
             }
@@ -490,7 +541,11 @@
 
 typedef __int128 i128;
 
-struct FsConsts { uint32_t c80r[9], biasmod[9], biasmod_pm[9], biasmod_ps[9]; };
+struct FsConsts {
+    uint32_t c80r[9], biasmod[9], biasmod_pm[9], biasmod_ps[9];
+    uint32_t ms_c80[9], ms_bias[9], pneg[8];
+};
+constexpr int FS_MS_BIAS = 1 << 20;
 constexpr int32_t FS_OVERFLOW = 0x40000000;
 
 __device__ __forceinline__ size_t fs_digit_addr(int i, int l, int b, int nkb) {
@@ -534,7 +589,8 @@
 
 __device__ __forceinline__ void fs_build_body(uint8_t *fb_lds, const FpParams<9> &P, const uint32_t *__restrict__ inv, int n, const FsIdx &ix, int d, int nc, int n_coef,
                                               int flags, const FsConsts &cs, uint8_t *__restrict__ a8, uint32_t *__restrict__ crow, uint32_t *__restrict__ KT,
-                                              int32_t *__restrict__ rowmode, int32_t *__restrict__ z_dev, int32_t *__restrict__ status, const FsPack &pk) {
+                                              int32_t *__restrict__ rowmode, int32_t *__restrict__ z_dev, int32_t *__restrict__ status, const FsPack &pk,
+                                              uint8_t *__restrict__ ms = nullptr) {
     constexpr int NL = 9, NW = 8;
     const int n_out = n_coef + nc, nkb = (d + 7) / 8, n_rt = (n_out + 15) / 16;
     i128 *ent = reinterpret_cast<i128 *>(fb_lds);
@@ -647,6 +703,44 @@
             for (int k = 0; k < NL; k++) KT[((size_t)l * NL + q) * NL + k] = tq[k];
         }
     }
+    if (do_z && ms) {
+        for (int i = tid; i < 64; i += 1024) reinterpret_cast<uint4 *>(ms)[d * 64 + i] = make_uint4(0, 0, 0, 0);
+        for (int e = tid; e < d * 32; e += 1024) {
+            const int l = e >> 5, b = e & 31;
+            uint32_t w[NL], two[NL], u[NL], uw[NW];
+#pragma unroll
+            for (int k = 0; k < NL; k++) { w[k] = wj[(size_t)l * NL + k]; two[k] = (k == (8 * b) / LB) ? 1u << ((8 * b) % LB) : 0u; }
+            mont_mul(u, w, two, P);
+            pack<NL, NW>(uw, u);
+            int8_t dg[32];
+            int carry = 0;
+            for (int pass = 0; pass < 2; pass++) {
+                carry = 0;
+                for (int c = 0; c < 32; c++) {
+                    int t = (int)((uw[c >> 2] >> (8 * (c & 3))) & 0xffu) + carry;
+                    if (t > 127) { t -= 256; carry = 1; } else carry = 0;
+                    dg[c] = (int8_t)t;
+                }
+                if (carry == pass) break;
+                if (pass == 0) {
+                    unsigned cy = 0;
+#pragma unroll
+                    for (int k = 0; k < NW; k++) uw[k] = __builtin_addc(uw[k], cs.pneg[k], cy, &cy);
+                } else if (status) atomicOr(status, FS_OVERFLOW);
+            }
+            for (int c = 0; c < 32; c++) ms[(size_t)(((l * 2 + (b >> 4)) * 8 + (c >> 2)) * 4 + (c & 3)) * 16 + (b & 15)] = (uint8_t)dg[c];
+        }
+        for (int l = tid; l < d; l += 1024) {
+            uint32_t w[NL], c80[NL], bm[NL], prod[NL], kk[NL], kw[NW];
+#pragma unroll
+            for (int k = 0; k < NL; k++) { w[k] = wj[(size_t)l * NL + k]; c80[k] = cs.ms_c80[k]; bm[k] = cs.ms_bias[k]; }
+            mont_mul(prod, w, c80, P);
+            fp_sub(kk, prod, bm, P);
+            pack<NL, NW>(kw, kk);
+            int32_t *ci = reinterpret_cast<int32_t *>(ms + (size_t)(d + 1) * 1024) + l * 32;
+            for (int c = 0; c < 32; c++) ci[c] = FS_MS_BIAS + (int32_t)((kw[c >> 2] >> (8 * (c & 3))) & 0xffu);
+        }
+    }
 }
 
 __device__ __forceinline__ void fs_cand_body(uint8_t *fc_lds, const FpParams<9> &P, int n, const uint16_t *__restrict__ xs, const FsIdx &ix, int d, const FsConsts &cs,
@@ -684,9 +778,10 @@
 
 __global__ void __launch_bounds__(1024) k_fs_build(const FpParams<9> P, const uint32_t *__restrict__ inv, int n, const FsIdx ix, int d, int nc, int n_coef,
                                                    int flags, const FsConsts cs, uint8_t *__restrict__ a8, uint32_t *__restrict__ crow, uint32_t *__restrict__ KT,
-                                                   int32_t *__restrict__ rowmode, int32_t *__restrict__ z_dev, int32_t *__restrict__ status, const FsPack pk) {
+                                                   int32_t *__restrict__ rowmode, int32_t *__restrict__ z_dev, int32_t *__restrict__ status, const FsPack pk,
+                                                   uint8_t *__restrict__ ms) {
     extern __shared__ __attribute__((aligned(16))) uint8_t fs_b_lds[];
-    fs_build_body(fs_b_lds, P, inv, n, ix, d, nc, n_coef, flags, cs, a8, crow, KT, rowmode, z_dev, status, pk);
+    fs_build_body(fs_b_lds, P, inv, n, ix, d, nc, n_coef, flags, cs, a8, crow, KT, rowmode, z_dev, status, pk, ms);
 }
 
 __global__ void __launch_bounds__(1024) k_fs_cand(const FpParams<9> P, int n, const uint16_t *__restrict__ xs, const FsIdx ix, int d, const FsConsts cs,
@@ -737,7 +832,9 @@
     L->o_kt = L->o_crow + al((size_t)L->n_rt * 16 * 16 * 4);
     L->o_mode = L->o_kt + al((size_t)d * 81 * 4);
     L->o_z = L->o_mode + al((size_t)L->n_rt * 16 * 4);
-    L->need = L->o_z + al((size_t)FS_MAXD * 4);
+    L->o_ms = L->o_z + al((size_t)FS_MAXD * 4);
+    L->need = L->o_ms + al((size_t)fs_ms_q(d) * 16);
+    L->mscale = 0;
     L->o_cand = L->o_cand_crow = 0;
     if (pt->n <= FS_CAND_MAXN && nc > 0) {
         L->o_cand = L->need;
@@ -776,6 +873,11 @@
     L->pk_nm = pk.nm; L->pk_ns = pk.ns;
     memcpy(L->pk_single, pk.single, sizeof pk.single);
     return true;
+}
+
+bool fs_mscale(FsLayout *L) {
+    L->mscale = !env_hook(ENV_NO_FUSED_MSCALE) && fs_lds_bytes(L->n_rt, L->nkb, L->d) <= FS_LDS_LIMIT;
+    return L->mscale != 0;
 }
 
 int fs_build(hb_ctx *ctx, const PointTable *pt, const int32_t *z, const int32_t *zc, const FsLayout &L, uint8_t *base, int flags, int32_t *status_dev, hipStream_t s) {
@@ -802,6 +904,10 @@
     memcpy(cs.biasmod, sh->biasmod, sizeof cs.biasmod);
     memcpy(cs.biasmod_pm, sh->biasmod_pm, sizeof cs.biasmod_pm);
     memcpy(cs.biasmod_ps, sh->biasmod_ps, sizeof cs.biasmod_ps);
+    memcpy(cs.ms_c80, sh->ms_c80, sizeof cs.ms_c80);
+    memcpy(cs.ms_bias, sh->ms_bias, sizeof cs.ms_bias);
+    memcpy(cs.pneg, sh->bp.pneg, sizeof cs.pneg);
+    if (L.mscale && flags != (FS_BUILD_Z | FS_BUILD_ZC)) return fail(ctx, HB_ERR_BAD_ARG, "fused decode: the matrix-core division's tables are built with the whole image");
     FsPack pk;
     memset(&pk, 0, sizeof pk);
     if (L.pk_nm) {
@@ -811,7 +917,7 @@
     }
     const size_t lds = ((size_t)L.n_out * d + d + 1) * 16 + ((size_t)d * 9 + (size_t)d * 4 * 9) * 4;
     k_fs_build<<<1, 1024, lds, s>>>(ctx->pw, pt->inv, n, ix, d, nc, L.n_coef, flags, cs, base + L.o_a8, (uint32_t *)(base + L.o_crow), (uint32_t *)(base + L.o_kt),
-                                    (int32_t *)(base + L.o_mode), (int32_t *)(base + L.o_z), status_dev, pk);
+                                    (int32_t *)(base + L.o_mode), (int32_t *)(base + L.o_z), status_dev, pk, L.mscale ? base + L.o_ms : nullptr);
     HB_LAUNCH_CHECK(ctx);
     return HB_OK;
 }
@@ -839,6 +945,9 @@
     memcpy(cs.biasmod, sh->biasmod, sizeof cs.biasmod);
     memset(cs.biasmod_pm, 0, sizeof cs.biasmod_pm);
     memset(cs.biasmod_ps, 0, sizeof cs.biasmod_ps);
+    memset(cs.ms_c80, 0, sizeof cs.ms_c80);
+    memset(cs.ms_bias, 0, sizeof cs.ms_bias);
+    memset(cs.pneg, 0, sizeof cs.pneg);
     if (with_z) {
         const size_t lds_b = ((size_t)L.n_out * L.d + L.d + 1) * 16 + ((size_t)L.d * 9 + (size_t)L.d * 4 * 9) * 4, lds_c = (size_t)pt->n * L.d * 16;
         k_fs_build_z_cand<<<2, 1024, std::max(lds_b, lds_c), s>>>(ctx->pw, pt->inv, pt->n, pt->xs_dev, ix, L.d, L.nc, L.n_coef, cs, base + L.o_a8, (uint32_t *)(base + L.o_crow),
@@ -853,9 +962,11 @@
 }
 
 static std::atomic<int> g_fs_last_pack{-1};
-
-static FsSplit fs_split(int d, int n_rt, int n_out, int pk_nm, int pk_ns) {
-    constexpr int PASS = 95, RAGGED = 70, TERM = 36, PACKED2 = 50, PACKED3 = 55;
+static std::atomic<int> g_fs_last_mscale{-1};
+
+static FsSplit fs_split(int d, int n_rt, int n_out, int pk_nm, int pk_ns, bool mscale) {
+    constexpr int PASS = 95, RAGGED = 70, PACKED2 = 50, PACKED3 = 55;
+    const int TERM = mscale ? 24 : 36;
     const int packed = pk_ns ? PACKED3 : PACKED2;
     FsSplit sp;
     int load[FS_WAVES];
@@ -888,7 +999,7 @@
     FsPick pick;
     memset(&pick, 0, sizeof pick);
     if (pick_zc) {
-        if (L.pk_nm) return fail(ctx, HB_ERR_BAD_ARG, "fused decode: a packed image has no rows to pick");
+        if (L.pk_nm || L.mscale) return fail(ctx, HB_ERR_BAD_ARG, "fused decode: an image built in one piece has no rows to pick");
         if (!L.o_cand) return fail(ctx, HB_ERR_BAD_ARG, "fused decode: no candidate store to pick from");
         pick.cand = (const uint4 *)(base + L.o_cand); pick.cand_crow = (const uint32_t *)(base + L.o_cand_crow);
         pick.n_coef = L.n_coef; pick.nc = L.nc;
@@ -901,17 +1012,20 @@
     int64_t blocks = fs_num_cus();
     if (blocks > n_units) blocks = n_units;
     blocks = mm8_trimmed_grid(n_units, blocks);
-    const size_t lds = fs_lds_bytes(L.n_rt, L.nkb);
-    const FsSplit split = fs_split(L.d, L.n_rt, L.n_out, L.pk_nm, L.pk_ns);
+    const size_t lds = fs_lds_bytes(L.n_rt, L.nkb, L.mscale ? L.d : 0);
+    const FsSplit split = fs_split(L.d, L.n_rt, L.n_out, L.pk_nm, L.pk_ns, L.mscale != 0);
     const int pack = !L.pk_nm ? 0 : L.pk_ns ? 2 : 1;
     g_fs_last_pack.store(pack);
-#define FS_LAUNCH(NKB, PK)                                                                                                                   \
+    g_fs_last_mscale.store(L.mscale ? 1 : 0);
+#define FS_LAUNCH(NKB, PK) do { if (L.mscale) FS_LAUNCH_(NKB, PK, true); else FS_LAUNCH_(NKB, PK, false); } while (0)
+#define FS_LAUNCH_(NKB, PK, MSC)                                                                                                                   \
     do {                                                                                                                                   \
         static std::atomic<unsigned long long> attr_done{0};                                                                                                        \
-        if (!((attr_done.load() >> (ctx->device & 63)) & 1ull)) { HB_HIP(ctx, hipFuncSetAttribute(reinterpret_cast<const void *>(k_mm8f<NKB, PK>), hipFuncAttributeMaxDynamicSharedMemorySize, 160 * 1024)); attr_done.fetch_or(1ull << (ctx->device & 63)); } \
-        k_mm8f<NKB, PK><<<dim3((unsigned)blocks), dim3(64 * FS_WAVES), lds, s>>>((const int4 *)(base + L.o_a8), (const uint32_t *)(base + L.o_crow), sh->fold_dev,        \
+        if (!((attr_done.load() >> (ctx->device & 63)) & 1ull)) { HB_HIP(ctx, hipFuncSetAttribute(reinterpret_cast<const void *>(k_mm8f<NKB, PK, MSC>), hipFuncAttributeMaxDynamicSharedMemorySize, 160 * 1024)); attr_done.fetch_or(1ull << (ctx->device & 63)); } \
+        k_mm8f<NKB, PK, MSC><<<dim3((unsigned)blocks), dim3(64 * FS_WAVES), lds, s>>>((const int4 *)(base + L.o_a8), (const uint32_t *)(base + L.o_crow), sh->fold_dev,        \
             (const uint32_t *)(base + L.o_kt), ctx->psc, cols, cv.stride_c, cv.stride_l, (const int32_t *)(base + L.o_z), INT64_MAX, L.d, (const int32_t *)(base + L.o_mode), \
-            out, ov.stride_c, ov.stride_l, out_count, mismatch_dev, first_bad_dev, bad_map_dev, L.n_out, L.n_rt, C, n_units, sh->bp, done, pick, split); \
+            out, ov.stride_c, ov.stride_l, out_count, mismatch_dev, first_bad_dev, bad_map_dev, L.n_out, L.n_rt, C, n_units, sh->bp, done, pick, split, \
+            L.mscale ? (const v4i *)(base + L.o_ms) : nullptr); \
     } while (0)
     switch (L.nkb) {
         case 1: if (pack == 1) FS_LAUNCH(1, 1); else if (pack == 2) FS_LAUNCH(1, 2); else FS_LAUNCH(1, 0); break;
@@ -920,6 +1034,7 @@
         default: return fail(ctx, HB_ERR_UNSUPPORTED, "fused decode: more than 24 terms");
     }
 #undef FS_LAUNCH
+#undef FS_LAUNCH_
     HB_LAUNCH_CHECK(ctx);
     return HB_OK;
 }
@@ -944,6 +1059,7 @@
     return hb_debug_fs_pack_rows(d, n_coef, nc, small, out);
 }
 extern "C" int hb_debug_fs_last_pack(void) { return hb::g_fs_last_pack.load(); }
+extern "C" int hb_debug_fs_last_mscale(void) { return hb::g_fs_last_mscale.load(); }
 extern "C" int hb_debug_fs_slot(int nm, int ns, const int32_t *single, int i, int n_out, int32_t *kind) {
     hb::FsPack pk;
     memset(&pk, 0, sizeof pk);
diff --git a/honeybadgermpc_amd/csrc/hb_mm8.hpp b/honeybadgermpc_amd/csrc/hb_mm8.hpp
--- a/honeybadgermpc_amd/csrc/hb_mm8.hpp
+++ b/honeybadgermpc_amd/csrc/hb_mm8.hpp
@@ -32,6 +32,7 @@
     BarrettParams bp;
     uint32_t c80r[9], biasmod[9];
     uint32_t biasmod_pm[9], biasmod_ps[9];
+    uint32_t ms_c80[9], ms_bias[9];
     uint8_t fold_host[MM8_FOLD_Q * 16];
     v4i *fold_dev;
 };
diff --git a/honeybadgermpc_amd/csrc/hb_open.hip b/honeybadgermpc_amd/csrc/hb_open.hip
--- a/honeybadgermpc_amd/csrc/hb_open.hip
+++ b/honeybadgermpc_amd/csrc/hb_open.hip
@@ -73,7 +73,7 @@
         int qrc = HB_OK;
         if (hipMalloc(&b1, a.need) != hipSuccess || hipMalloc(&b2, b.need) != hipSuccess) qrc = HB_ERR_HIP;
         const int32_t *zcp = pl->n_check > 0 ? pl->zc.data() : pl->z.data();
-        if (!qrc) { (void)fs_pack(pt, pl->z.data(), &a); (void)fs_pack(pt, pl->z.data(), &b); }
+        if (!qrc) { (void)fs_pack(pt, pl->z.data(), &a); (void)fs_pack(pt, pl->z.data(), &b); (void)fs_mscale(&a); (void)fs_mscale(&b); }
         if (!qrc) qrc = fs_build(ctx, pt, pl->z.data(), zcp, a, b1, FS_BUILD_Z | FS_BUILD_ZC, pl->mismatch_dev, s);
         if (!qrc) qrc = fs_build(ctx, pt, pl->z.data(), zcp, b, b2, FS_BUILD_Z | FS_BUILD_ZC, pl->mismatch_dev, s);
         if (!qrc) { pl->fs1 = b1; pl->fs2 = b2; pl->fl1 = a; pl->fl2 = b; pl->fused_pending = 0; }
diff --git a/honeybadgermpc_amd/csrc/hb_quick.hip b/honeybadgermpc_amd/csrc/hb_quick.hip
--- a/honeybadgermpc_amd/csrc/hb_quick.hip
+++ b/honeybadgermpc_amd/csrc/hb_quick.hip
@@ -1112,6 +1112,7 @@
             rc = take_slot(F.need, &sl); if (rc) return rc;
             uint8_t *base = static_cast<uint8_t *>(sl->buf);
             (void)fs_pack(pt, z, &F);
+            (void)fs_mscale(&F);
             rc = fs_build(ctx, pt, z, zc, F, base, FS_BUILD_Z | FS_BUILD_ZC, status_dev, s); if (rc) return rc;
             uint32_t *out = coeffs_dev ? (uint32_t *)coeffs_dev + (size_t)chunk_lo * d * 8 : nullptr;
             rc = fs_launch(ctx, F, base, in, pm, out, dv, coeffs_dev ? cnt * (int64_t)d : 0, status_dev, (nc > 0 && status_dev) ? status_dev + 1 : nullptr,
diff --git a/include/hbmpc_hip_debug.h b/include/hbmpc_hip_debug.h
--- a/include/hbmpc_hip_debug.h
+++ b/include/hbmpc_hip_debug.h
@@ -22,6 +22,7 @@
 int hb_debug_fs_pack_points(const int32_t *xz, int d, int n_coef, int nc, int32_t *out, uint8_t *small_out);
 int hb_debug_fs_slot(int nm, int ns, const int32_t *single, int i, int n_out, int32_t *kind);
 int hb_debug_fs_last_pack(void);
+int hb_debug_fs_last_mscale(void);
 
 
 #ifdef __cplusplus
```

Result: faster. 9.003 billion (median of 6 runs) (+5.2%).
